# angeris/cfmm-routing-code

Measured on AMD Instinct MI355X. Metric: pool-subproblems/sec to 1e-6 rel-gap; 1e6 pools / 1k tokens; 1/2/4/8 GPU, higher is better.
Workload: dtype f64; 1 GPU; C3: 1000000 pools per GPU (cp2=700000, w2=200000, gn3-8=100000) / 1000 tokens, linear-utility arbitrage, cold-start solve to gap,infeas <= 1e-06; pools_per_gpu=1000000, pools_total=1000000, seed=0, parallelism=single GPU, rccl_ranks=1

## Files before the change

### cfmm-routing-code_amd/csrc/cfmm_hip.hip

```cpp
#include <hip/hip_runtime.h>
#include <dlfcn.h>
#include <algorithm>
#include <cmath>
#include <atomic>
#include <chrono>
#include <condition_variable>
#include <cstdarg>
#include <cstdio>
#include <cstdlib>
#include <cstring>
#include <map>
#include <memory>
#include <set>
#include <mutex>
#include <functional>
#include <limits>
#include <string>
#include <thread>
#include <type_traits>
#include <vector>

#include "../../include/cfmm.h"
#include "kernels.hpp"
#include "iterate.hpp"
// ... 96 lines not shown
    bool have_nu = false;
    bool hsol_valid = false;
    double mu_last = 0.0;
    bool slo_active = false;
    std::vector<double> tr_ovr;
    bool tr_ovr_valid = false;
};

struct cfmm_ctx {
    int device = 0, n = 0, ng = 0;
    int cus = 256;
    hipStream_t stream = nullptr;
    std::string err;
    std::string backend;

    std::shared_ptr<PoolStore> pools = std::make_shared<PoolStore>();
    int *flags2 = nullptr;
    bool is_clone = false;
    unsigned long long pool_gen = 0;
    hipEvent_t ev_pool = nullptr;
    char *upd_dev = nullptr; size_t upd_cap = 0;
    unsigned long long *upd_host = nullptr;
    int *flagsG[CFMM_MAX_POOL_SIZE + 1] = {};
    double *trade_buf = nullptr;
    size_t trade_cap = 0;

    double *c = nullptr, *h = nullptr, *off = nullptr, *glo = nullptr, *ghi = nullptr;
    int *ctype = nullptr, *grp = nullptr;
    int *gptr = nullptr, *gmem = nullptr;
    double *tie_tmp = nullptr;
    double *nu = nullptr, *nu_acc = nullptr, *psi_acc = nullptr, *psi_t = nullptr, *nu0 = nullptr;
    double *s = nullptr, *s_t = nullptr, *Gs = nullptr, *Gs_t = nullptr, *d = nullptr, *Ds = nullptr;
    double *S = nullptr, *Y = nullptr, *rho = nullptr;
    double *acc = nullptr;
    DevState *st = nullptr;
    long long *ts = nullptr;
    char *dev_arena = nullptr, *host_arena = nullptr;
    double *pin = nullptr; size_t pin_cap = 0;
    double *pin_dev = nullptr;
    unsigned long long io_seq = 0;
    bool h_clean = false;
    bool lean_io = true;
    char *util_h = nullptr;
    size_t util_span = 0;
    DevState *hst = nullptr;
    double *hsol = nullptr;
    double *hnu0 = nullptr;
    double *hnu0_d = nullptr, *hsol_d = nullptr;
    DevState *hst_d = nullptr;
    bool nu0_deferred = false;
    Point pt;
    hipEvent_t ev[2] = {nullptr, nullptr}, ev_t0 = nullptr, ev_t1 = nullptr;
    int walk_parity[2] = {0, 0};
    int nslices = 2;
    int eval_grid_mult = 1;
    int eval_blocks_per_cu = 1;
    int upd_grid = 1;
    bool no_graph = false;
    bool multi_graph = false;
    int upd_variant = 0;
    bool upd_generic = false;
    bool general_utility = false;
    bool have_utility = false;
    std::vector<double> hc, hh, hoff;
    std::vector<int> hctype, hgrp;

    bool fused = true;
    bool tile_dma = true;
    bool tiny_path = true;
    bool plain = false;
    bool det = false;
    unsigned long long *acc_l = nullptr;
    double max_reserve = 0.0, min_fee = 1.0;
    double g_max_reserve = 0.0;
    double nu_max = 1.0;
    double det_ref_reserve = 0.0, det_ref_fee = 0.0;
    double *acc3 = nullptr, *xs3 = nullptr;
    DevState *st3 = nullptr;
    DevState *hst3 = nullptr;
    int iter_blocks_per_cu = 1;
    volatile unsigned long long *hstat_h = nullptr;
    unsigned long long *hstat_d = nullptr;
    int run_ahead = 3;
    std::vector<char> listed;
    bool listed_valid = false;
    UpdArgs *upd_batch_d = nullptr, *upd_batch_h = nullptr;
    double *batch_ws[7] = {};
    long long batch_ws_m[7] = {};
    const double *batch_ws_of[7] = {};

    hipGraphExec_t gexec = nullptr;
    int g_iters = 0, g_memory = 0;
    cfmm_opts g_opts = {};
    bool g_valid = false;

    ncclComm_t comm = nullptr;
    int n_ranks = 1, rank = 0;
    int64_t g_total = 0, g_stable = 0, g_table = 0;
    bool g_counts_valid = false;

    unsigned long long *os_mail = nullptr;
    size_t os_cap = 0;
    unsigned long long *os_peers[ONESHOT_MAX_RANKS] = {};
    std::vector<void *> os_opened;
    bool os_ready = false;

    double *sm_out = nullptr, *sm_vec = nullptr, *H = nullptr, *Dinv = nullptr;
    double *Winv = nullptr, *Rinv = nullptr;
    double *chord_y = nullptr;
    bool chol_pairs = true;
    bool inverse_factor = true;
    double *sm_ws[CFMM_POOL_KINDS2] = {};
    long long sm_ws_m[CFMM_POOL_KINDS2] = {};
    double *sm_slo = nullptr;
    int *sm_mask = nullptr, *sm_info = nullptr;
    hipStream_t probe_stream = nullptr;
    long long *probe_ring = nullptr, *probe_ring_d = nullptr;
    bool probe_running = false;
};

namespace {

int fail(cfmm_ctx *ctx, int code, const char *fmt, ...);

int trade_scratch(cfmm_ctx *ctx, size_t count, double **delta, double **lambda)
{
    if (2 * count > ctx->trade_cap) {
        if (ctx->trade_buf) (void)hipFree(ctx->trade_buf);
        ctx->trade_buf = nullptr; ctx->trade_cap = 0;
        hipError_t e = hipMalloc((void **)&ctx->trade_buf, 2 * count * sizeof(double));
        if (e != hipSuccess) return fail(ctx, CFMM_E_HIP, "trade scratch: hipMalloc(%zu) -> %s", 2 * count * sizeof(double), hipGetErrorString(e));
        ctx->trade_cap = 2 * count;
    }
    *delta = ctx->trade_buf; *lambda = ctx->trade_buf + count;
    return CFMM_OK;
}

int fail(cfmm_ctx *ctx, int code, const char *fmt, ...)
{
    char buf[512];
    va_list ap; va_start(ap, fmt); vsnprintf(buf, sizeof buf, fmt, ap); va_end(ap);
    if (ctx) ctx->err = buf; else g_create_error = buf;
    return code;
}

#define HIP_TRY(ctx, call)                                                                        \
    do {                                                                                          \
        hipError_t e_ = (call);                                                                   \
        if (e_ != hipSuccess) return fail(ctx, CFMM_E_HIP, "%s -> %s (%s:%d)", #call, hipGetErrorString(e_), __FILE__, __LINE__); \
    } while (0)

inline bool sharded(const cfmm_ctx *ctx) { return ctx->comm != nullptr || ctx->os_ready; }
inline bool rccl_unfolded(const cfmm_ctx *ctx)
{
    static const bool off = getenv("CFMM_RCCL_FOLD") && atoi(getenv("CFMM_RCCL_FOLD")) != 0;
    return ctx->comm != nullptr && !ctx->det && !off && !(ctx->os_ready && (size_t)acc_arb(ctx->n) + 1 <= ctx->os_cap);
}

int all_reduce(cfmm_ctx *ctx, void *buf, size_t count, int dtype, int op, const DevState *stop = nullptr, int fold_slices = 1)
{
    if (fold_slices > 1 && !(ctx->os_ready && count <= ctx->os_cap))
        hipLaunchKernelGGL(fold_kernel, dim3(((int)count + 255) / 256), dim3(256), 0, ctx->stream, (double *)buf, ctx->n, fold_slices,
                           count > (size_t)acc_arb(ctx->n) + 1 ? 1 : 0, stop);
    if (ctx->os_ready && count <= ctx->os_cap) {
        OneShotArgs a = {};
        for (int r = 0; r < ctx->n_ranks; ++r) a.mail[r] = ctx->os_peers[r];
        a.buf = (unsigned long long *)buf;
        a.epoch_word = ctx->os_mail + oneshot_bytes(ctx->os_cap) / 8;
        a.stop = stop ? &stop->status : nullptr;
        a.nslices = fold_slices; a.stride = acc_stride(ctx->n);
        a.n_ranks = ctx->n_ranks; a.rank = ctx->rank; a.count = (int)count; a.cap = ctx->os_cap;
        a.op = dtype == NCCL_INT64 ? ONESHOT_SUM_I64 : (op == NCCL_MAX ? ONESHOT_MAX_F64 : ONESHOT_SUM_F64);
        hipLaunchKernelGGL(oneshot_allreduce_kernel, dim3(1), dim3(ONESHOT_THREADS), 0, ctx->stream, a);
        return CFMM_OK;
    }
    if (!ctx->comm) return fail(ctx, CFMM_E_UNSUPPORTED, "all-reduce of %zu elements: beyond the one-shot mailbox and no RCCL communicator", count);
    const int rc = g_rccl.AllReduce(buf, buf, count, dtype, op, ctx->comm, ctx->stream);
    if (rc != 0) return fail(ctx, CFMM_E_RCCL, "ncclAllReduce -> %s", g_rccl.GetErrorString ? g_rccl.GetErrorString(rc) : "error");
    return CFMM_OK;
}

template <class T>
int dev_upload(cfmm_ctx *ctx, T **dst, const T *src, size_t count, std::vector<void *> *track)
{
    T *p = nullptr;
    HIP_TRY(ctx, hipMalloc((void **)&p, count * sizeof(T) + 16));
    if (src) HIP_TRY(ctx, hipMemcpyAsync(p, src, count * sizeof(T), hipMemcpyHostToDevice, ctx->stream));
    else HIP_TRY(ctx, hipMemsetAsync(p, 0, count * sizeof(T), ctx->stream));
    if (track) track->push_back(p);
    *dst = p;
    return CFMM_OK;
}

constexpr size_t STAGE_BYTES = 4u << 20;
constexpr int STAGE_SLOTS = 4;
struct StageRing {
    std::mutex mu;
    char *buf = nullptr;
    hipEvent_t ev[STAGE_SLOTS] = {};
    bool used[STAGE_SLOTS] = {};
    hipStream_t last[STAGE_SLOTS] = {};
    int next = 0;
};
StageRing g_stage;
void stage_ring_drain(hipStream_t stream)
{
    std::lock_guard<std::mutex> lock(g_stage.mu);
    for (int q = 0; q < STAGE_SLOTS; ++q)
        if (g_stage.used[q] && g_stage.last[q] == stream) { (void)hipEventSynchronize(g_stage.ev[q]); g_stage.used[q] = false; }
}
hipError_t stage_slot_wait(int slot)
{
    hipError_t e = hipEventSynchronize(g_stage.ev[slot]);
    if (e != hipSuccess) { (void)hipGetLastError(); e = hipDeviceSynchronize(); }
    return e;
}
std::mutex g_stream_mu;
std::vector<hipStream_t> g_free_streams[64];

class HostPool {
public:
    static HostPool &get() { static HostPool *p = new HostPool(); return *p; }
    int threads() const { return nthreads_ + 1; }
    void run(int n, const std::function<void(int)> &f)
    {
        if (n <= 0) return;
        if (n == 1 || nthreads_ == 0) { for (int i = 0; i < n; ++i) f(i); return; }
        std::unique_lock<std::mutex> own(run_mu_);
        {
            std::lock_guard<std::mutex> g(mu_);
            job_ = &f; njobs_ = n; next_.store(0, std::memory_order_relaxed); left_.store(n, std::memory_order_relaxed);
            gen_.fetch_add(1, std::memory_order_release);
        }
// ... 1087 lines not shown
}
int listed_tokens(cfmm_ctx *ctx)
{
    if (ctx->listed_valid) return CFMM_OK;
    const int n = ctx->n;
    double *mark = ctx->sm_vec;
    HIP_TRY(ctx, hipMemsetAsync(mark, 0, (size_t)n * sizeof(double), ctx->stream));
    auto pass = [&](const int *ids, long long count) {
        if (!ids || count <= 0) return;
        const unsigned grid = (unsigned)std::min<long long>((count + 255) / 256, 4ll * ctx->cus);
        hipLaunchKernelGGL(mark_tokens_kernel, dim3(grid), dim3(256), 0, ctx->stream, ids, count, mark);
    };
    const PoolStore &ps = *ctx->pools;
    for (int k = 0; k < CFMM_POOL_KINDS2; ++k) { pass(ps.r2[k].b.ia, ps.r2[k].b.m); pass(ps.r2[k].b.ib, ps.r2[k].b.m); }
    for (int k = 3; k <= CFMM_MAX_POOL_SIZE; ++k) pass(ps.rn[k].b.idx, (long long)k * ps.rn[k].b.m);
    for (auto &row : ps.rg) for (int k = 2; k <= CFMM_MAX_POOL_SIZE; ++k) pass(row[k].b.idx, (long long)k * row[k].b.m);
    HIP_TRY(ctx, hipGetLastError());
    if (sharded(ctx)) { int rc = all_reduce(ctx, mark, (size_t)n, NCCL_FLOAT64, NCCL_SUM); if (rc) return rc; }
    std::vector<double> h(n);
    HIP_TRY(ctx, hipMemcpyAsync(h.data(), mark, (size_t)n * sizeof(double), hipMemcpyDeviceToHost, ctx->stream));
    HIP_TRY(ctx, hipStreamSynchronize(ctx->stream));
    ctx->listed.assign(n, 0);
    for (int j = 0; j < n; ++j) ctx->listed[j] = h[j] != 0.0;
    ctx->listed_valid = true;
    return CFMM_OK;
}

struct SmoothEval { std::vector<double> psi; double value = 0.0, trade = 0.0; };

int smooth_eval_host(cfmm_ctx *ctx, const std::vector<double> &nu, double mu, bool hess, SmoothEval &e, bool warm = true,
                     const std::vector<double> *slo = nullptr)
{
    const int n = ctx->n;
    int rc = smooth_buffers(ctx, hess); if (rc) return rc;
    double *pin = pin_scratch(ctx, 8 * (size_t)n + 64);
    if (!pin) return fail(ctx, CFMM_E_HIP, "pinned staging (%d tokens)", n);
    double *pin_nu = pin, *pin_slo = pin + n, *pin_out = pin + 2 * n;
    std::memcpy(pin_nu, nu.data(), n * sizeof(double));
    if (slo) std::memcpy(pin_slo, slo->data(), n * sizeof(double));
    if (ctx->lean_io) {
        IoList l;
        l.copy(ctx->nu, pin_device(ctx, pin_nu), n * sizeof(double));
        if (slo) l.copy(ctx->sm_slo, pin_device(ctx, pin_slo), n * sizeof(double));
        l.zero(ctx->sm_out, (size_t)(n + 2) * sizeof(double));
        if (hess && !ctx->h_clean) l.zero(ctx->H, (size_t)hess_ld(n) * hess_nr(n) * sizeof(double));
        if (hess) ctx->h_clean = false;
        if ((rc = launch_io(ctx, l, false))) return rc;
        if ((rc = launch_smooth(ctx, mu, hess, warm, slo != nullptr, true))) return rc;
        IoList p;
        p.copy(pin_device(ctx, pin_out), ctx->sm_out, (size_t)(n + 2) * sizeof(double));
        if ((rc = launch_io(ctx, p, true))) return rc;
        if ((rc = wait_io(ctx))) return rc;
    } else {
        HIP_TRY(ctx, hipMemcpyAsync(ctx->nu, pin_nu, n * sizeof(double), hipMemcpyHostToDevice, ctx->stream));
        if (slo) HIP_TRY(ctx, hipMemcpyAsync(ctx->sm_slo, pin_slo, n * sizeof(double), hipMemcpyHostToDevice, ctx->stream));
        if ((rc = launch_smooth(ctx, mu, hess, warm, slo != nullptr))) return rc;
        HIP_TRY(ctx, hipMemcpyAsync(pin_out, ctx->sm_out, (size_t)(n + 2) * sizeof(double), hipMemcpyDeviceToHost, ctx->stream));
        HIP_TRY(ctx, hipStreamSynchronize(ctx->stream));
    }
    e.psi.assign(pin_out, pin_out + n);
    e.value = pin_out[n]; e.trade = pin_out[n + 1];
    return CFMM_OK;
}

struct HostUtilityTerm { double pstar, ubar, uval, viol, d2; };
static HostUtilityTerm host_utility_term(int ctype, double c, double h, double nu, double psi)
{
    HostUtilityTerm t;
    if (ctype == CFMM_ULOG) {
        t.pstar = c / nu - h; t.ubar = c * std::log(c / nu) - c + nu * h;
        t.viol = std::max(-(psi + h), 0.0); t.uval = c * std::log(std::max(psi + h, 1e-300)); t.d2 = c;
    } else {
        t.pstar = h * (c - nu); t.ubar = 0.5 * h * (c - nu) * (c - nu);
        t.viol = 0.0; t.uval = c * psi - 0.5 * psi * psi / h; t.d2 = h * nu * nu;
    }
    return t;
}

int solve_newton(cfmm_ctx *ctx, const cfmm_opts &o, cfmm_stats *out, int evals_before, double warm_mu)
{
    const char *why = "";
    if (!newton_supported(ctx, &why)) return fail(ctx, CFMM_E_UNSUPPORTED, "solve: the second-order method cannot take this problem: %s", why);
    const int n = ctx->n;
    int rc = smooth_buffers(ctx, true); if (rc) return rc;
    const std::vector<double> &c = ctx->hc, &h = ctx->hh;
    const std::vector<int> &ct = ctx->hctype;

    HIP_TRY(ctx, hipStreamSynchronize(ctx->stream));
    const auto t0 = std::chrono::steady_clock::now();
    HIP_TRY(ctx, hipEventRecord(ctx->ev_t0, ctx->stream));

    std::vector<double> s(n), nu(n), d(n), G(n), Hd(n), rhs(n), s2(n), nu2(n), psi_x(n);
    std::vector<int> mask(n), pin(n);
    std::vector<double> lob(n);
    if (!pin_scratch(ctx, 8 * (size_t)n + 64 + n + (size_t)acc_stride(n))) return fail(ctx, CFMM_E_HIP, "pinned staging (%d tokens)", n);
    if (ctx->lean_io) {
        IoList z;
        for (int k = 0; k < CFMM_POOL_KINDS2; ++k) if (ctx->sm_ws[k]) z.zero(ctx->sm_ws[k], 2 * (size_t)ctx->pools->r2[k].b.m * sizeof(double));
        if (z.a.njobs && (rc = launch_io(ctx, z, false))) return rc;
        IoList p;
        p.copy(pin_device(ctx, ctx->pin), ctx->nu_acc, n * sizeof(double));
        if ((rc = launch_io(ctx, p, true)) || (rc = wait_io(ctx))) return rc;
        std::memcpy(nu.data(), ctx->pin, n * sizeof(double));
    } else {
        HIP_TRY(ctx, hipMemcpyAsync(nu.data(), ctx->nu_acc, n * sizeof(double), hipMemcpyDeviceToHost, ctx->stream));
        HIP_TRY(ctx, hipStreamSynchronize(ctx->stream));
    }
    if ((rc = listed_tokens(ctx))) return rc;
    std::vector<char> listed(n);
    for (int j = 0; j < n; ++j) listed[j] = !(ct[j] < CFMM_ULOG && !ctx->listed[j] && h[j] == 0.0);
    long long nbar = 0;
    for (int k = 0; k < CFMM_POOL_KINDS2; ++k) nbar += 2 * ctx->pools->r2[k].b.m;
    nbar += 2 * ctx->pools->r2[CFMM_POOL_SUM2].b.m;
    for (int k = 2; k <= CFMM_MAX_POOL_SIZE; ++k) nbar += 3LL * k * ctx->pools->rg[CFMM_POOLK_SUM][k].b.m;
    for (int j = 0; j < n; ++j) {
        mask[j] = ct[j] == CFMM_FREE || !listed[j];
        lob[j] = (ct[j] == CFMM_GE && c[j] > 0.0) ? std::log(c[j]) : -INFINITY;
        if (ct[j] == CFMM_GE && !(c[j] > 0.0) && listed[j]) nbar += 1;
        double sj = std::log(nu[j]);
        if (ct[j] == CFMM_FREE) {
            if (!(c[j] > 0.0)) return fail(ctx, CFMM_E_ARG, "solve: token %d is unconstrained (CFMM_FREE) with c = 0: unbounded", j);
            sj = std::log(c[j]);
        } else sj = std::max(sj, lob[j]);
        s[j] = sj; nu[j] = std::exp(sj);
    }
    if (sharded(ctx)) {
        long long ge = 0;
        for (int j = 0; j < n; ++j) ge += ct[j] == CFMM_GE && !(c[j] > 0.0) && listed[j];
        double cnt = (double)(nbar - ge);
        HIP_TRY(ctx, hipMemcpyAsync(ctx->sm_vec, &cnt, sizeof(double), hipMemcpyHostToDevice, ctx->stream));
        { int rc = all_reduce(ctx, ctx->sm_vec, 1, NCCL_FLOAT64, NCCL_SUM); if (rc) return rc; }
        HIP_TRY(ctx, hipMemcpyAsync(&cnt, ctx->sm_vec, sizeof(double), hipMemcpyDeviceToHost, ctx->stream));
        HIP_TRY(ctx, hipStreamSynchronize(ctx->stream));
        nbar = (long long)cnt + ge;
    }

    const std::vector<double> s_start = s;
    ctx->h_clean = false;
    int evals = evals_before, steps = 0, status = 0;
    double arb_x = 0.0;
    auto exact = [&](const std::vector<double> &p) { ++evals; return cfmm_eval_dual(ctx, p.data(), &arb_x, psi_x.data(), nullptr); };
    auto assemble = [&](const std::vector<double> &p, const SmoothEval &e, double mu, std::vector<double> *grad, std::vector<double> *hdiag) {
        double g = e.value;
        for (int j = 0; j < n; ++j) {
            double Gj, hj = 0.0;
            if (ct[j] >= CFMM_ULOG) {
                const HostUtilityTerm ut = host_utility_term(ct[j], c[j], h[j], p[j], e.psi[j]);
                g += ut.ubar;
                Gj = p[j] * (e.psi[j] - ut.pstar);
                hj = ut.d2;
            } else {
                g += (p[j] - c[j]) * h[j];
                Gj = p[j] * (e.psi[j] + h[j]);
            }
            const double Gj_lin = Gj;
            if (ct[j] == CFMM_GE && !(c[j] > 0.0) && listed[j]) {
                g -= mu * std::log(p[j]);
                Gj -= mu;
            }
            if (grad) (*grad)[j] = mask[j] ? 0.0 : Gj;
            if (hdiag) (*hdiag)[j] = std::max(Gj_lin, 0.0) + hj;
        }
        return g;
    };

    if (!ctx->lean_io)
        for (int k = 0; k < CFMM_POOL_KINDS2; ++k)
// ... 302 lines not shown
    static const bool trace_c = getenv("CFMM_UPLOAD_TRACE") != nullptr;
    const auto tc0 = std::chrono::steady_clock::now();
    auto lap = [&](const char *what) { if (trace_c) fprintf(stderr, "[cfmm create] %-28s %.3f ms\n", what, std::chrono::duration<double, std::milli>(std::chrono::steady_clock::now() - tc0).count()); };
    TRY_C(hipSetDevice(device));
    hipDeviceProp_t prop;
    TRY_C(hipGetDeviceProperties(&prop, device));
    lap("device properties");
    ctx->cus = prop.multiProcessorCount > 0 ? prop.multiProcessorCount : 256;
    ctx->backend = std::string("hip:") + prop.gcnArchName;
    if (ctx->backend.find("gfx950") == std::string::npos) {
        fail(ctx, CFMM_E_HIP, "cfmm_create: device is %s, this build is gfx950-only", prop.gcnArchName);
        return bail(CFMM_E_HIP);
    }
    if (eval_lds_bytes(n_tokens, true) > 160 * 1024) {
        fail(ctx, CFMM_E_LIMIT, "cfmm_create: %d tokens exceed the LDS-staged limit (%d)", n_tokens, (int)((160 * 1024 / 8 - 16) / 3));
        return bail(CFMM_E_LIMIT);
    }
    {
        const char *sp = getenv("CFMM_STREAM_POOL");
        std::lock_guard<std::mutex> g(g_stream_mu);
        auto &fl = g_free_streams[device & 63];
        if (!(sp && atoi(sp) == 0) && !fl.empty()) { ctx->stream = fl.back(); fl.pop_back(); }
    }
    if (!ctx->stream) TRY_C(hipStreamCreateWithFlags(&ctx->stream, hipStreamNonBlocking));
    lap("stream");
    if (const char *s = getenv("CFMM_SLICES")) ctx->nslices = std::min(64, std::max(1, atoi(s)));
    if (const char *s = getenv("CFMM_EVAL_GRID_MULT")) ctx->eval_grid_mult = std::max(1, atoi(s));
    if (const char *s = getenv("CFMM_UPDATE_GENERIC")) ctx->upd_generic = atoi(s) != 0;
    if (const char *s = getenv("CFMM_UPDATE_VARIANT")) ctx->upd_variant = atoi(s);
    if (const char *s = getenv("CFMM_UPD_GRID")) ctx->upd_grid = std::max(1, atoi(s));
    if (const char *s = getenv("CFMM_MULTI_GRAPH")) ctx->multi_graph = atoi(s) != 0;
    if (const char *s = getenv("CFMM_NO_GRAPH")) ctx->no_graph = atoi(s) != 0;
    if (const char *s = getenv("CFMM_FUSED")) ctx->fused = atoi(s) != 0;
    if (const char *s = getenv("CFMM_TILE_DMA")) ctx->tile_dma = atoi(s) != 0;
    if (const char *s = getenv("CFMM_BACKSUB")) ctx->inverse_factor = std::string(s) != "classic";
    if (const char *s = getenv("CFMM_CHOL")) ctx->chol_pairs = std::string(s) != "single";
    if (const char *s = getenv("CFMM_NEWTON_IO")) ctx->lean_io = std::string(s) != "blit";
    if (const char *s = getenv("CFMM_TINY")) ctx->tiny_path = atoi(s) != 0;
    if (const char *s = getenv("CFMM_RUN_AHEAD")) ctx->run_ahead = std::max(1, atoi(s));
    if (const char *s = getenv("CFMM_DETERMINISTIC")) ctx->det = atoi(s) != 0;
    const int n = n_tokens;
    int rc = 0;
    {
        struct Piece { void **dst; size_t bytes; };
        std::vector<Piece> pieces;
        auto want = [&](auto **pp, size_t count) { pieces.push_back({(void **)pp, count * sizeof(**pp)}); };
        want(&ctx->c, n + 4); want(&ctx->h, n + 4); want(&ctx->glo, n + 4); want(&ctx->ghi, n + 4); want(&ctx->ctype, n + 4);
        want(&ctx->off, n + 4); want(&ctx->grp, n + 4);
        want(&ctx->gptr, n + 5); want(&ctx->gmem, n + 4); want(&ctx->tie_tmp, 2 * (size_t)n + 4);
        double **vecs[] = {&ctx->nu, &ctx->nu_acc, &ctx->psi_acc, &ctx->psi_t, &ctx->nu0, &ctx->s, &ctx->s_t,
                           &ctx->Gs, &ctx->Gs_t, &ctx->d, &ctx->Ds};
        for (auto v : vecs) want(v, n + 4);
        want(&ctx->S, (size_t)MAX_MEMORY * hist_stride(n) + 4); want(&ctx->Y, (size_t)MAX_MEMORY * hist_stride(n) + 4);
        want(&ctx->rho, MAX_MEMORY);
        want(&ctx->acc, (size_t)ctx->nslices * acc_stride(n) + 4);
        want(&ctx->st, 1);
        want(&ctx->acc3, 3 * (size_t)ctx->nslices * acc_stride(n) + 4);
        want(&ctx->xs3, 3 * (size_t)XS_VECS * iter_xvs(n) + 4);
        want(&ctx->st3, 3);
        want(&ctx->acc_l, 6 * (size_t)n + 4);
        want(&ctx->ts, 64 + 8 * 4096 + 2048);
        size_t total = 0;
        for (auto &pc : pieces) total += (pc.bytes + 16 + 255) & ~(size_t)255;
        TRY_C(hipMalloc((void **)&ctx->dev_arena, total));
        TRY_C(hipMemsetAsync(ctx->dev_arena, 0, total, ctx->stream));
        size_t off = 0;
        for (auto &pc : pieces) { *pc.dst = ctx->dev_arena + off; off += (pc.bytes + 16 + 255) & ~(size_t)255; }
        ctx->util_span = (size_t)((char *)ctx->off - (char *)ctx->c);
        const size_t hb[5] = {2 * sizeof(DevState), 6 * sizeof(DevState), 2 * (size_t)n * sizeof(double), (size_t)n * sizeof(double), ctx->util_span};
        size_t ho[6] = {0, 0, 0, 0, 0, 0};
        for (int q = 0; q < 5; ++q) ho[q + 1] = ho[q] + ((hb[q] + 255) & ~(size_t)255);
        TRY_C(hipHostMalloc((void **)&ctx->host_arena, ho[5], hipHostMallocDefault));
        ctx->hst = (DevState *)(ctx->host_arena + ho[0]); ctx->hst3 = (DevState *)(ctx->host_arena + ho[1]);
        ctx->hsol = (double *)(ctx->host_arena + ho[2]); ctx->hnu0 = (double *)(ctx->host_arena + ho[3]);
        {
            char *base_d = nullptr;
            TRY_C(hipHostGetDevicePointer((void **)&base_d, ctx->host_arena, 0));
            ctx->hst_d = (DevState *)(base_d + ho[0]); ctx->hsol_d = (double *)(base_d + ho[2]); ctx->hnu0_d = (double *)(base_d + ho[3]);
        }
        ctx->util_h = ctx->host_arena + ho[4];
        std::memset(ctx->util_h, 0, ctx->util_span);
    }
    lap("device + pinned arenas");
    TRY_C(hipHostMalloc((void **)&ctx->hstat_h, 64 + ITER_HRING * sizeof(unsigned long long), hipHostMallocMapped));
    TRY_C(hipHostGetDevicePointer((void **)&ctx->hstat_d, (void *)ctx->hstat_h, 0));
    *ctx->hstat_h = 0;
    lap("mapped progress word");
    for (int i = 0; i < 2; ++i) TRY_C(hipEventCreateWithFlags(&ctx->ev[i], hipEventDisableTiming));
    TRY_C(hipEventCreate(&ctx->ev_t0));
    TRY_C(hipEventCreate(&ctx->ev_t1));
    TRY_C(hipEventCreateWithFlags(&ctx->ev_pool, hipEventDisableTiming));
    ctx->pools->sharers.push_back(ctx);
    if (ctx->det && eval_lds_bytes(n, true, true) > 160 * 1024) {
        fail(ctx, CFMM_E_LIMIT, "cfmm_create: CFMM_DETERMINISTIC=1 with %d tokens exceeds the LDS tile of the reproducible mode", n);
        return bail(CFMM_E_LIMIT);
    }
    lap("events");
    if ((rc = set_all_lds_attrs(ctx))) return bail(rc);
    lap("LDS attributes");
    {
        int nb = 0;
        TRY_C(hipOccupancyMaxActiveBlocksPerMultiprocessor(&nb, eval_kernel<false, false>, EVAL_THREADS, eval_lds_bytes(n, false)));
        ctx->eval_blocks_per_cu = nb < 1 ? 1 : nb;
        nb = 0;
        TRY_C(hipOccupancyMaxActiveBlocksPerMultiprocessor(&nb, iter_kernel<2, false, false>, EVAL_THREADS, iter_lds_bytes(n)));
        ctx->iter_blocks_per_cu = nb < 1 ? 1 : nb;
    }
    if (ctx->nslices > 64) ctx->nslices = 64;
    ctx->hc.assign(n, 0.0); ctx->hh.assign(n, 0.0); ctx->hoff.assign(n, 0.0);
    ctx->hctype.assign(n, CFMM_GE); ctx->hgrp.resize(n);
    for (int j = 0; j < n; ++j) ctx->hgrp[j] = j;
    lap("occupancy queries");
    TRY_C(hipMemcpyAsync(ctx->grp, ctx->hgrp.data(), n * sizeof(int), hipMemcpyHostToDevice, ctx->stream));
    TRY_C(hipStreamSynchronize(ctx->stream));
    lap("group ids + sync");
#undef TRY_C
    *out = ctx;
    return CFMM_OK;
}

int cfmm_clone(cfmm_ctx *src, cfmm_ctx **out)
{
    if (!src || !out) return CFMM_E_ARG;
    HIP_TRY(src, hipSetDevice(src->device));
    pools_ready(src);
    HIP_TRY(src, hipStreamSynchronize(src->stream));
    release_landed(src);
    cfmm_ctx *c = nullptr;
    int rc = cfmm_create(src->device, src->n, &c);
    if (rc) { src->err = g_create_error; return rc; }
    {
        std::lock_guard<std::mutex> g(src->pools->mu);
        c->pools = src->pools;
        c->pools->sharers.push_back(c);
    }
    c->is_clone = true;
    c->det = src->det;
    local_extrema(c);
    c->pool_gen = c->pools->gen.load(std::memory_order_acquire);
    c->nslices = src->nslices <= c->nslices ? src->nslices : c->nslices;
    *out = c;
    return CFMM_OK;
}

int cfmm_destroy(cfmm_ctx *ctx)
{
    if (!ctx) return CFMM_OK;
    (void)hipSetDevice(ctx->device);
    if (ctx->stream) (void)hipStreamSynchronize(ctx->stream);
    drop_graph(ctx);
    if (ctx->comm && g_rccl.CommDestroy) g_rccl.CommDestroy(ctx->comm);
    for (void *q : ctx->os_opened) (void)hipIpcCloseMemHandle(q);
    if (ctx->os_mail) (void)hipFree(ctx->os_mail);
    if (ctx->pools) {
        std::lock_guard<std::mutex> g(ctx->pools->mu);
        auto &sh = ctx->pools->sharers;
        sh.erase(std::remove(sh.begin(), sh.end(), ctx), sh.end());
    }
    ctx->pools.reset();
    if (ctx->ev_pool) (void)hipEventDestroy(ctx->ev_pool);
    if (ctx->upd_dev) (void)hipFree(ctx->upd_dev);
    if (ctx->upd_host) (void)hipHostFree(ctx->upd_host);
    if (ctx->flags2) (void)hipFree(ctx->flags2);
    for (int *q : ctx->flagsG) if (q) (void)hipFree(q);
    if (ctx->trade_buf) (void)hipFree(ctx->trade_buf);
    for (void *p : {(void *)ctx->sm_out, (void *)ctx->sm_vec, (void *)ctx->H, (void *)ctx->Dinv, (void *)ctx->Winv, (void *)ctx->Rinv, (void *)ctx->chord_y, (void *)ctx->sm_ws[0], (void *)ctx->sm_ws[1], (void *)ctx->sm_ws[3], (void *)ctx->sm_ws[4], (void *)ctx->sm_slo, (void *)ctx->sm_mask, (void *)ctx->sm_info}) if (p) (void)hipFree(p);
    if (ctx->dev_arena) (void)hipFree(ctx->dev_arena);
    if (ctx->host_arena) (void)hipHostFree(ctx->host_arena);
    if (ctx->pin) (void)hipHostFree(ctx->pin);
    if (ctx->hstat_h) (void)hipHostFree((void *)ctx->hstat_h);
    if (ctx->probe_ring) {
        __atomic_store_n(reinterpret_cast<volatile long long *>(ctx->probe_ring) + 2 * PROBE_CAP, 1ll, __ATOMIC_RELEASE);
        if (ctx->probe_stream) (void)hipStreamSynchronize(ctx->probe_stream);
        (void)hipHostFree(ctx->probe_ring);
    }
    if (ctx->probe_stream) (void)hipStreamDestroy(ctx->probe_stream);
    if (ctx->upd_batch_d) (void)hipFree(ctx->upd_batch_d);
    if (ctx->upd_batch_h) (void)hipHostFree(ctx->upd_batch_h);
    for (double *q : ctx->batch_ws) if (q) (void)hipFree(q);
    for (auto &e : ctx->ev) if (e) (void)hipEventDestroy(e);
    if (ctx->ev_t0) (void)hipEventDestroy(ctx->ev_t0);
    if (ctx->ev_t1) (void)hipEventDestroy(ctx->ev_t1);
    if (ctx->stream) {
        std::lock_guard<std::mutex> g(g_stream_mu);
        auto &fl = g_free_streams[ctx->device & 63];
        if (fl.size() < 16) fl.push_back(ctx->stream); else (void)hipStreamDestroy(ctx->stream);
    }
    sweep_release(ctx);
    delete ctx;
    return CFMM_OK;
}

int64_t cfmm_pool_count(cfmm_ctx *ctx)
{
    if (!ctx) return 0;
    int64_t m = 0;
    ctx->pools->each([&m](const auto &r) { m += r.b.m; });
    return m;
}

int64_t cfmm_eval_bytes(cfmm_ctx *ctx)
{
    if (!ctx) return 0;
    int64_t bytes = 0;
    for (int k = 0; k < CFMM_POOL_KINDS2; ++k) {
        const bool par = !(k == CFMM_POOL_CP2 || k == CFMM_POOL_SUM2);
        const bool mirror = ctx->pools->r2[k].cmem != nullptr && !ctx->det && !heavy_kind(k);
        bytes += ctx->pools->r2[k].b.m * ((mirror ? 21 : 32) + (par ? 8 : 0));
    }
    const bool lrw = !ctx->det && !CFMM_STAGED_WALK;
    for (int k = 3; k <= CFMM_MAX_POOL_SIZE; ++k) bytes += ctx->pools->rn[k].b.m * (20 + (lrw ? 28 : 20) * k);
    for (auto &row : ctx->pools->rg) {
        int k = 0;
        for (auto &r : row) { bytes += r.b.m * (12 * k + (r.b.param ? 40 : 16)); ++k; }
    }
    return bytes;
}

static bool reorder_applies(cfmm_ctx *ctx, int kind_or_k, int64_t m)
{
    static const bool off = getenv("CFMM_REORDER") && atoi(getenv("CFMM_REORDER")) == 0;
    return !off && m >= (kind_or_k >= 3 ? RO_MIN_POOLS_N : RO_MIN_POOLS) && ctx->n >= 2 * RO_NB && kind_or_k != CFMM_POOL_SUM2;
}
static char *reorder_arena(cfmm_ctx *ctx, size_t total, int64_t m, int **perm, unsigned **hist)
{
    char *na = nullptr;
    const size_t pbytes = ((size_t)m * 4 + 255) & ~(size_t)255;
    if (hipMalloc((void **)&na, total + 256 + pbytes + 4096) != hipSuccess) return nullptr;
    *perm = (int *)(na + total + 256);
    *hist = (unsigned *)(na + total + 256 + pbytes);
    (void)hipMemsetAsync(*hist, 0, RO_KEYS * sizeof(unsigned), ctx->stream);
    return na;
// ... 28 lines not shown
    const dim3 gh(std::min(grid, 2048)), gs(grid), blk(RO_THREADS);
    with_int<3, 8>(k, [&](auto K) {
        hipLaunchKernelGGL(ro_hist_kernel<K>, gh, blk, 0, ctx->stream, b.idx, (const int *)nullptr, (long long)b.m, bsz, hist);
        hipLaunchKernelGGL(ro_scan_kernel, dim3(1), dim3(64), 0, ctx->stream, hist);
        hipLaunchKernelGGL(ro_scatterN_kernel<K>, gs, blk, 0, ctx->stream, b, d, perm, bsz, hist);
    });
    b.idx = d.idx; b.R = d.R; b.w = d.w; b.fee = d.fee; b.lfee = d.lfee; b.lrw = d.lrw; b.perm = perm;
    r.mem = na;
    return true;
}

static void build_compact_mirrors(cfmm_ctx *ctx, PoolStore &ps)
{
    static const int mode = getenv("CFMM_COMPACT") ? atoi(getenv("CFMM_COMPACT")) : -1;
    if (mode == 0 || ctx->n > 65536) return;
    for (int k : {CFMM_POOL_CP2, CFMM_POOL_W2, CFMM_POOL_SUM2}) {
        Resident2 &r = ps.r2[k];
        Bucket2 &b = r.b;
        if (r.ctried || b.m == 0 || (mode < 0 && b.m < 1000000)) continue;
        r.ctried = true;
        const size_t m = (size_t)b.m, off_fee = (4 * m + 255) & ~(size_t)255, off_tab = (off_fee + m + 255) & ~(size_t)255;
        char *mem = nullptr;
        if (hipMalloc((void **)&mem, off_tab + 256 * 8 + 64) != hipSuccess) { (void)hipGetLastError(); continue; }
        (void)hipMemsetAsync(mem + off_tab, 0, 256 * 8 + 64, ctx->stream);
        int *flag = (int *)(mem + off_tab + 256 * 8);
        hipLaunchKernelGGL(compact_build_kernel, dim3((unsigned)std::min<size_t>((m + 255) / 256, 4096)), dim3(256), 0, ctx->stream, b,
                           (unsigned *)mem, (unsigned char *)(mem + off_fee), (unsigned long long *)(mem + off_tab), flag);
        int over = 1;
        if (hipMemcpyAsync(&over, flag, sizeof(int), hipMemcpyDeviceToHost, ctx->stream) != hipSuccess || hipStreamSynchronize(ctx->stream) != hipSuccess) over = 1;
        if (over) { (void)hipGetLastError(); (void)hipFree(mem); continue; }
        r.cmem = mem;
        b.cid = (const unsigned *)mem; b.cfee = (const unsigned char *)(mem + off_fee); b.ctab = (const double *)(mem + off_tab);
    }
}

static void pools_ready(cfmm_ctx *ctx)
{
    pools_seen(ctx);
    PoolStore &ps = *ctx->pools;
    std::lock_guard<std::mutex> guard(ps.mu);
    struct Mirrors { cfmm_ctx *c; PoolStore &p; ~Mirrors() { build_compact_mirrors(c, p); } } mirrors{ctx, ps};
    {
        bool pending = false;
        ps.each([&pending](const auto &r) { pending |= r.ro != 0; });
        if (!pending) return;
        double stray = 0.0;
        for (int k = 3; k <= CFMM_MAX_POOL_SIZE; ++k) stray += (double)ps.rn[k].b.m * (k - 2);
        if (stray / (double)ctx->cus >= 0.5 * ctx->n) {
            ps.each([](auto &r) { r.ro = 0; });
            return;
        }
    }
    for (auto &r : ps.r2) if (r.ro) {
        void *old = r.mem;
        if (reorder_bucket2(ctx, r)) ps.landed.emplace_back(old, ctx->stream);
        r.ro = 0;
    }
    for (int k = 3; k <= CFMM_MAX_POOL_SIZE; ++k) if (ps.rn[k].ro) {
        void *old = ps.rn[k].mem;
        if (reorder_bucketN(ctx, k, ps.rn[k])) ps.landed.emplace_back(old, ctx->stream);
        ps.rn[k].ro = 0;
    }
}
static void release_landed(cfmm_ctx *ctx)
{
    PoolStore &ps = *ctx->pools;
    std::vector<void *> mine;
    {
        std::lock_guard<std::mutex> guard(ps.mu);
        size_t keep = 0;
        for (auto &q : ps.landed) { if (q.second == ctx->stream) mine.push_back(q.first); else ps.landed[keep++] = q; }
        ps.landed.resize(keep);
    }
    if (mine.empty()) return;
    (void)hipStreamSynchronize(ctx->stream);
    for (void *q : mine) (void)hipFree(q);
}

struct PoolEntry {
    cfmm_ctx *ctx;
    PoolStore &ps;
    const bool reader;
    hipError_t device;
    explicit PoolEntry(cfmm_ctx *c, bool rd = true) : ctx(c), ps(*c->pools), reader(rd)
    {
        if (reader) { std::lock_guard<std::mutex> g(ps.mu); ++ps.readers; }
        if ((device = hipSetDevice(c->device)) == hipSuccess) pools_ready(c);
    }
    ~PoolEntry() { release_landed(ctx); if (reader) { std::lock_guard<std::mutex> g(ps.mu); --ps.readers; } }
};

struct Kind2Info { const char *name; bool needs_param; bool (*param_ok)(double); const char *param_rule; };
static const Kind2Info kKind2[CFMM_POOL_KINDS2] = {
    {"constant product", false, nullptr, ""},
    {"weighted geometric mean", true, [](double x) { return x > 0.0 && x < 1.0; }, "a weight in (0, 1)"},
    {"constant sum", false, nullptr, ""},
    {"stableswap", true, [](double x) { return x > 0.0 && x <= std::numeric_limits<double>::max(); }, "alpha > 0"},
    {"power sum", true, [](double x) { return x >= 1e-3 && x <= 0.999; }, "an exponent t in [0.001, 0.999]"},
};

extern "C++" {
static int upload_begin(cfmm_ctx *ctx, const char *who, const void *old_arena)
{
    HIP_TRY(ctx, hipSetDevice(ctx->device));
    if (ctx->pools.use_count() > 1) return fail(ctx, CFMM_E_STATE, "%s: the pools are shared with a clone (cfmm_clone); destroy the clones first", who);
    if (old_arena) HIP_TRY(ctx, hipStreamSynchronize(ctx->stream));
    return CFMM_OK;
}
template <class R, class B> static void upload_install(cfmm_ctx *ctx, R &r, const B &b, void *arena, const UploadScan &scan, size_t ro_total)
{
    r.release();
    r.b = b; r.mem = arena; r.ro = ro_total;
    r.mxr = scan.mxr; r.mnf = scan.mnf;
    pools_changed(ctx);
}
}

int cfmm_upload_pools2(cfmm_ctx *ctx, int kind, int64_t m, const double *Ra, const double *Rb, const double *fee,
                       const double *param, const int32_t *ia, const int32_t *ib)
{
    if (!ctx) return CFMM_E_ARG;
    if (kind < 0 || kind >= CFMM_POOL_KINDS2 || m < 0) return fail(ctx, CFMM_E_ARG, "upload_pools2: kind %d, m %lld", kind, (long long)m);
    if (m >= (1ll << 29)) return fail(ctx, CFMM_E_LIMIT, "upload_pools2: %lld pools in one bucket (the kernels address a column with 32-bit byte offsets: < 2^29)", (long long)m);
    if (m > 0 && (!Ra || !Rb || !fee || !ia || !ib)) return fail(ctx, CFMM_E_ARG, "upload_pools2: NULL column");
    if (m > 0 && kKind2[kind].needs_param && !param) return fail(ctx, CFMM_E_ARG, "upload_pools2: kind %d (%s) needs param", kind, kKind2[kind].name);
    Resident2 &r = ctx->pools->r2[kind];
    { int rc = upload_begin(ctx, "upload_pools2", r.mem); if (rc) return rc; }
    Bucket2 b = {};
    b.m = m;
    void *arena = nullptr;
    UploadScan scan;
    size_t ro_total = 0;
    if (m > 0) {
        const int ntok = ctx->n;
        std::vector<Col> cols;
        auto reserve_ok = [](double x) { return x > 0.0 && x <= std::numeric_limits<double>::max(); };
        cols.push_back(checked_col<double>(Ra, m, (void **)&b.Ra, &scan, 0, reserve_ok));
        cols.push_back(checked_col<double>(Rb, m, (void **)&b.Rb, &scan, 0, reserve_ok));
        cols.push_back(checked_col<double>(fee, m, (void **)&b.fee, &scan, 1, [](double x) { return x > 0.0 && x <= 1.0; }));
        if (param) {
            if (kKind2[kind].param_ok) cols.push_back(checked_col<double>(param, m, (void **)&b.param, &scan, 2, kKind2[kind].param_ok));
            else cols.push_back(plain_col(param, m * sizeof(double), (void **)&b.param));
        }
        cols.push_back(checked_col<int32_t>(ia, m, (void **)&b.ia, &scan, 2, [ntok](int32_t v) { return (uint32_t)v < (uint32_t)ntok; }));
        {
            Col c; c.bytes = m * sizeof(int32_t); c.dst = (void **)&b.ib; c.direct = ib;
            UploadScan *sp = &scan;
            c.fill = [ia, ib, ntok, sp](char *out, size_t off, size_t len) {
                const size_t i0 = off / sizeof(int32_t), cnt = len / sizeof(int32_t);
                std::memcpy(out, ib + i0, len);
                const int32_t *o = (const int32_t *)out, *a = ia + i0;
                bool ok = true;
                for (size_t i = 0; i < cnt; ++i) ok &= ((uint32_t)o[i] < (uint32_t)ntok) & (o[i] != a[i]);
                if (!ok) sp->bad.store(true, std::memory_order_relaxed);
            };
            cols.push_back(c);
        }
        size_t total = 0;
        const bool ro = reorder_applies(ctx, kind, m);
        int rc = upload_arena(ctx, cols, &arena, &scan, &total);
        if (rc == CFMM_E_ARG && scan.bad.load()) {
            for (int64_t i = 0; i < m; ++i) {
                const long long q = (long long)i;
                if (ia[i] < 0 || ia[i] >= ntok || ib[i] < 0 || ib[i] >= ntok || ia[i] == ib[i]) return fail(ctx, CFMM_E_ARG, "upload_pools2: pool %lld has token ids (%d, %d) outside [0,%d) or equal", q, ia[i], ib[i], ctx->n);
                if (!(Ra[i] > 0.0) || !(Rb[i] > 0.0) || !std::isfinite(Ra[i]) || !std::isfinite(Rb[i])) return fail(ctx, CFMM_E_ARG, "upload_pools2: pool %lld has a reserve that is not positive and finite", q);
                if (!(fee[i] > 0.0 && fee[i] <= 1.0)) return fail(ctx, CFMM_E_ARG, "upload_pools2: pool %lld has fee %g outside (0, 1]", q, fee[i]);
                if (kind == CFMM_POOL_W2 && !(param[i] > 0.0 && param[i] < 1.0)) return fail(ctx, CFMM_E_ARG, "upload_pools2: pool %lld has weight %g outside (0, 1)", q, param[i]);
                if (kind == CFMM_POOL_CURVE2 && !(param[i] > 0.0)) return fail(ctx, CFMM_E_ARG, "upload_pools2: pool %lld has alpha %g <= 0", q, param[i]);
                if (param && kKind2[kind].param_ok && !kKind2[kind].param_ok(param[i]))
                    return fail(ctx, CFMM_E_ARG, "upload_pools2: pool %lld (%s) has parameter %g: expected %s", q, kKind2[kind].name, param[i], kKind2[kind].param_rule);
            }
            return fail(ctx, CFMM_E_ARG, "upload_pools2: a column failed its checks");
        }
        if (rc) return rc;
        if (ro) ro_total = total;
    }
    if (kind == CFMM_POOL_SUM2) {
        ctx->pools->hs_ia.clear(); ctx->pools->hs_ib.clear(); ctx->pools->hs_fee.clear(); ctx->pools->hs_Ra.clear(); ctx->pools->hs_Rb.clear();
        if (m > 0 && m <= 65536) {
            ctx->pools->hs_ia.assign(ia, ia + m); ctx->pools->hs_ib.assign(ib, ib + m); ctx->pools->hs_fee.assign(fee, fee + m);
            ctx->pools->hs_Ra.assign(Ra, Ra + m); ctx->pools->hs_Rb.assign(Rb, Rb + m);
        }
        if (ctx->flags2) { (void)hipFree(ctx->flags2); ctx->flags2 = nullptr; }
    }
    upload_install(ctx, r, b, arena, scan, ro_total);
    return CFMM_OK;
}
// ... 297 lines not shown
    if (kind < 0 || kind >= CFMM_POOLK_KINDS || k < 2 || k > CFMM_MAX_POOL_SIZE || count < 0)
        return fail(ctx, CFMM_E_ARG, "%s: kind %d, %d assets, count %lld", who, kind, k, (long long)count);
    if (count > 0 && (!pos || !R)) return fail(ctx, CFMM_E_ARG, "%s: NULL column", who);
    if (param && kind != CFMM_POOLK_STABLE) return fail(ctx, CFMM_E_ARG, "%s: constant-sum pools have no parameter", who);
    UpdateFrame f(ctx, who, ctx->pools->rg[kind][k]);
    { int rc = f.open(count, pos, [&] { return fail(ctx, CFMM_E_STATE, "%s: no pools of kind %d with %d assets uploaded", who, kind, k); }); if (rc) return rc; }
    double mx_new = 0.0;
    { int rc = update_check_reserves(ctx, who, R, (int64_t)k * count, mx_new); if (rc) return rc; }
    if (param)
        for (int64_t i = 0; i < count; ++i)
            if (!(param[i] > 0.0 && param[i] <= std::numeric_limits<double>::max())) return fail(ctx, CFMM_E_ARG, "%s: entry %lld has alpha %g (need > 0)", who, (long long)i, param[i]);
    const BucketG b = f.r.b;
    const int64_t m = b.m;
    const double mx_old = f.r.mxr;
    std::vector<UpdPart> parts = {{pos, (size_t)count * 4}, {R, (size_t)count * k * 8}};
    if (param) parts.push_back({param, (size_t)count * 8});
    const int cnt = (int)count;
    return f.run(parts, nullptr, mx_new, count,
        [&](const char *d, const std::vector<size_t> &o, const int *, int *low) {
            hipLaunchKernelGGL(upd_scatterG_kernel, dim3(upd_grid(count)), dim3(UP_THREADS), 0, ctx->stream, b, k, cnt, (const int *)(d + o[0]),
                               (const double *)(d + o[1]), param ? (const double *)(d + o[2]) : nullptr, mx_old, low);
        },
        [&](unsigned long long *out) {
            hipLaunchKernelGGL(upd_max_kernel, dim3(max_grid((int64_t)k * m)), dim3(UP_THREADS), 0, ctx->stream, b.R, (long long)k * m, (const double *)nullptr, 0ll, out);
        });
}

int cfmm_get_tradesG(cfmm_ctx *ctx, int kind, int k, double *delta, double *lambda)
{
    if (!ctx || kind < 0 || kind >= CFMM_POOLK_KINDS || k < 2 || k > CFMM_MAX_POOL_SIZE) return CFMM_E_ARG;
    PoolEntry entry(ctx); HIP_TRY(ctx, entry.device);
    const BucketG &b = ctx->pools->rg[kind][k].b;
    if (b.m == 0) return CFMM_OK;
    const dim3 grid((unsigned)((b.m + GK_THREADS - 1) / GK_THREADS)), blk(GK_THREADS);
    const double *nu = ctx->nu_acc;
    const int *fl = kind == CFMM_POOLK_SUM ? ctx->flagsG[k] : nullptr;
    const double *slo = (ctx->pt.mu_last > 0.0 && ctx->pt.slo_active) ? ctx->sm_slo : nullptr;
    const double mu = ctx->pt.mu_last > 0.0 ? ctx->pt.mu_last : 0.0;
    return read_back(ctx, "get_tradesG", (size_t)k * b.m, delta, lambda, [&](double *dd, double *dl) {
        with_int<CFMM_POOLK_STABLE, CFMM_POOLK_SUM>(kind, [&](auto KIND) {
            with_int<2, 8>(k, [&](auto K) { hipLaunchKernelGGL((tradesg_kernel<KIND, K>), grid, blk, 0, ctx->stream, b, fl, nu, slo, mu, dd, dl); });
        });
    });
}

int cfmm_set_pool_flags(cfmm_ctx *ctx, int kind, const int32_t *flags)
{
    if (!ctx) return CFMM_E_ARG;
    if (kind != CFMM_POOL_SUM2) return fail(ctx, CFMM_E_ARG, "set_pool_flags: only CFMM_POOL_SUM2 pools can be tied");
    HIP_TRY(ctx, hipSetDevice(ctx->device));
    const Bucket2 &b = ctx->pools->r2[kind].b;
    HIP_TRY(ctx, hipStreamSynchronize(ctx->stream));
    if (ctx->flags2) { (void)hipFree(ctx->flags2); ctx->flags2 = nullptr; }
    ctx->g_valid = false;
    drop_tenders(ctx);
    if (!flags || b.m == 0) return CFMM_OK;
    int rc = dev_upload<int>(ctx, &ctx->flags2, flags, b.m, nullptr);
    if (rc) return rc;
    HIP_TRY(ctx, hipStreamSynchronize(ctx->stream));
    return CFMM_OK;
}

int cfmm_set_pool_flagsG(cfmm_ctx *ctx, int k, const int32_t *flags)
{
    if (!ctx || k < 2 || k > CFMM_MAX_POOL_SIZE) return ctx ? fail(ctx, CFMM_E_ARG, "set_pool_flagsG: %d assets", k) : CFMM_E_ARG;
    HIP_TRY(ctx, hipSetDevice(ctx->device));
    const BucketG &b = ctx->pools->rg[CFMM_POOLK_SUM][k].b;
    HIP_TRY(ctx, hipStreamSynchronize(ctx->stream));
    if (ctx->flagsG[k]) { (void)hipFree(ctx->flagsG[k]); ctx->flagsG[k] = nullptr; }
    ctx->g_valid = false;
    drop_tenders(ctx);
    if (!flags || b.m == 0) return CFMM_OK;
    std::vector<int> pm((size_t)k * b.m);
    for (int64_t i = 0; i < b.m; ++i) for (int j = 0; j < k; ++j) pm[(size_t)i * k + j] = flags[(size_t)j * b.m + i];
    HIP_TRY(ctx, hipMalloc((void **)&ctx->flagsG[k], pm.size() * sizeof(int) + 16));
    HIP_TRY(ctx, hipMemcpy(ctx->flagsG[k], pm.data(), pm.size() * sizeof(int), hipMemcpyHostToDevice));
    return CFMM_OK;
}

int cfmm_set_utility(cfmm_ctx *ctx, const double *c, const double *h, const int32_t *ctype)
{
    if (!ctx || !c) return ctx ? fail(ctx, CFMM_E_ARG, "set_utility: c is NULL") : CFMM_E_ARG;
    HIP_TRY(ctx, hipSetDevice(ctx->device));
    const int n = ctx->n;
    bool general = false;
    for (int j = 0; j < n; ++j) {
        if (!(c[j] >= 0.0) || !std::isfinite(c[j])) return fail(ctx, CFMM_E_ARG, "set_utility: c[%d] < 0 or not finite", j);
        if (ctype && (ctype[j] < 0 || ctype[j] > CFMM_UQUAD)) return fail(ctx, CFMM_E_ARG, "set_utility: ctype[%d] = %d", j, ctype[j]);
        if (ctype && ctype[j] >= CFMM_ULOG) {
            general = true;
            const double hj = h ? h[j] : 0.0;
            if (ctype[j] == CFMM_ULOG && !(c[j] > 0.0 && hj >= 0.0 && std::isfinite(hj)))
                return fail(ctx, CFMM_E_ARG, "set_utility: token %d, u = c log(Psi + h) needs c > 0 and h >= 0 (c %g, h %g)", j, c[j], hj);
            if (ctype[j] == CFMM_UQUAD && !(hj > 0.0 && std::isfinite(hj)))
                return fail(ctx, CFMM_E_ARG, "set_utility: token %d, u = c Psi - Psi^2 / (2 h) needs h > 0 (h %g)", j, hj);
        }
    }
    if (general && ctx->ng != ctx->n) return fail(ctx, CFMM_E_UNSUPPORTED, "set_utility: price ties are set; the utility table's entries take none");
    if (general != ctx->general_utility) ctx->g_valid = false;
    ctx->general_utility = general;
    ctx->hc.assign(c, c + n);
    if (h) ctx->hh.assign(h, h + n); else ctx->hh.assign(n, 0.0);
    if (ctype) ctx->hctype.assign(ctype, ctype + n); else ctx->hctype.assign(n, CFMM_GE);
    ctx->have_utility = true;
    bool plain = true;
    for (int j = 0; j < n; ++j) if (ctx->hh[j] != 0.0 || ctx->hctype[j] != CFMM_GE) { plain = false; break; }
    if (plain != ctx->plain) ctx->g_valid = false;
    ctx->plain = plain;
    HIP_TRY(ctx, hipStreamSynchronize(ctx->stream));
    std::memcpy(ctx->util_h, ctx->hc.data(), n * sizeof(double));
    std::memcpy(ctx->util_h + ((char *)ctx->h - (char *)ctx->c), ctx->hh.data(), n * sizeof(double));
    std::memcpy(ctx->util_h + ((char *)ctx->ctype - (char *)ctx->c), ctx->hctype.data(), n * sizeof(int));
    { int rc = bounds_into_mirror(ctx); if (rc) return rc; }
    HIP_TRY(ctx, hipMemcpyAsync(ctx->c, ctx->util_h, ctx->util_span, hipMemcpyHostToDevice, ctx->stream));
    HIP_TRY(ctx, hipStreamSynchronize(ctx->stream));
    return CFMM_OK;
}

int cfmm_set_ties(cfmm_ctx *ctx, int n_groups, const int32_t *grp, const double *off)
{
    if (!ctx) return CFMM_E_ARG;
    HIP_TRY(ctx, hipSetDevice(ctx->device));
    const int n = ctx->n;
    if (!grp) {
        ctx->ng = n;
        for (int j = 0; j < n; ++j) { ctx->hgrp[j] = j; ctx->hoff[j] = 0.0; }
    } else {
        if (n_groups < 1 || n_groups > n || !off) return fail(ctx, CFMM_E_ARG, "set_ties: n_groups %d", n_groups);
        if (ctx->general_utility) return fail(ctx, CFMM_E_UNSUPPORTED, "set_ties: the utility has entries beyond linear-plus-box, which take no price ties");
        for (int j = 0; j < n; ++j) if (grp[j] < 0 || grp[j] >= n_groups) return fail(ctx, CFMM_E_ARG, "set_ties: grp[%d] = %d", j, grp[j]);
        ctx->ng = n_groups;
        ctx->hgrp.assign(grp, grp + n); ctx->hoff.assign(off, off + n);
    }
    drop_tenders(ctx);
    HIP_TRY(ctx, hipMemcpyAsync(ctx->grp, ctx->hgrp.data(), n * sizeof(int), hipMemcpyHostToDevice, ctx->stream));
    HIP_TRY(ctx, hipMemcpyAsync(ctx->off, ctx->hoff.data(), n * sizeof(double), hipMemcpyHostToDevice, ctx->stream));
    if (ctx->ng != n) {
        std::vector<int> gp(ctx->ng + 1, 0), gm(n);
        for (int j = 0; j < n; ++j) ++gp[ctx->hgrp[j] + 1];
        for (int r = 0; r < ctx->ng; ++r) gp[r + 1] += gp[r];
        std::vector<int> fill(gp.begin(), gp.end() - 1);
        for (int j = 0; j < n; ++j) gm[fill[ctx->hgrp[j]]++] = j;
        HIP_TRY(ctx, hipMemcpyAsync(ctx->gptr, gp.data(), (ctx->ng + 1) * sizeof(int), hipMemcpyHostToDevice, ctx->stream));
        HIP_TRY(ctx, hipMemcpyAsync(ctx->gmem, gm.data(), n * sizeof(int), hipMemcpyHostToDevice, ctx->stream));
        HIP_TRY(ctx, hipStreamSynchronize(ctx->stream));
    }
    ctx->g_valid = false;
    return recompute_bounds(ctx);
}

static int check_prices(cfmm_ctx *ctx, const char *who, const double *nu)
{
    double mx = 0.0;
    for (int j = 0; j < ctx->n; ++j) {
        if (!(nu[j] > 0.0) || !std::isfinite(nu[j])) return fail(ctx, CFMM_E_ARG, "%s[%d] = %g is not a positive finite price", who, j, nu[j]);
        mx = std::max(mx, nu[j]);
    }
    ctx->nu_max = mx;
    return CFMM_OK;
}

int cfmm_set_nu(cfmm_ctx *ctx, const double *nu)
{
    if (!ctx || !nu) return CFMM_E_ARG;
    HIP_TRY(ctx, hipSetDevice(ctx->device));
    { int rc = check_prices(ctx, "set_nu: nu", nu); if (rc) return rc; }
    HIP_TRY(ctx, hipStreamSynchronize(ctx->stream));
    std::memcpy(ctx->hnu0, nu, ctx->n * sizeof(double));
    HIP_TRY(ctx, hipMemcpyAsync(ctx->nu_acc, ctx->hnu0, ctx->n * sizeof(double), hipMemcpyHostToDevice, ctx->stream));
    point_from_caller(ctx);
    return CFMM_OK;
}

int cfmm_get_nu(cfmm_ctx *ctx, double *nu)
{
    if (!ctx || !nu) return CFMM_E_ARG;
    HIP_TRY(ctx, hipSetDevice(ctx->device));
    HIP_TRY(ctx, hipMemcpyAsync(nu, ctx->nu_acc, ctx->n * sizeof(double), hipMemcpyDeviceToHost, ctx->stream));
    HIP_TRY(ctx, hipStreamSynchronize(ctx->stream));
    return CFMM_OK;
}

int cfmm_get_psi(cfmm_ctx *ctx, double *psi)
{
    if (!ctx || !psi) return CFMM_E_ARG;
    HIP_TRY(ctx, hipSetDevice(ctx->device));
    pools_seen(ctx);
    HIP_TRY(ctx, hipMemcpyAsync(psi, ctx->psi_acc, ctx->n * sizeof(double), hipMemcpyDeviceToHost, ctx->stream));
    HIP_TRY(ctx, hipStreamSynchronize(ctx->stream));
    return CFMM_OK;
}

int cfmm_get_solution(cfmm_ctx *ctx, double *nu, double *psi)
{
    if (!ctx || (!nu && !psi)) return CFMM_E_ARG;
    pools_seen(ctx);
    if (ctx->pt.hsol_valid) {
        if (nu) std::memcpy(nu, ctx->hsol, ctx->n * sizeof(double));
        if (psi) std::memcpy(psi, ctx->hsol + ctx->n, ctx->n * sizeof(double));
        return CFMM_OK;
    }
    HIP_TRY(ctx, hipSetDevice(ctx->device));
    if (nu) HIP_TRY(ctx, hipMemcpyAsync(nu, ctx->nu_acc, ctx->n * sizeof(double), hipMemcpyDeviceToHost, ctx->stream));
    if (psi) HIP_TRY(ctx, hipMemcpyAsync(psi, ctx->psi_acc, ctx->n * sizeof(double), hipMemcpyDeviceToHost, ctx->stream));
    HIP_TRY(ctx, hipStreamSynchronize(ctx->stream));
    return CFMM_OK;
}

int cfmm_eval_dual(cfmm_ctx *ctx, const double *nu, double *arb_sum, double *psi, double *diag)
{
    if (!ctx || !nu) return CFMM_E_ARG;
    PoolEntry entry(ctx); HIP_TRY(ctx, entry.device);
    const int n = ctx->n;
    for (int j = 0; j < n; ++j) if (!(nu[j] > 0.0) || !std::isfinite(nu[j])) return fail(ctx, CFMM_E_ARG, "eval_dual: nu[%d] = %g is not a positive finite price", j, nu[j]);
    const int len = acc_stride(n);
    double *pinb = pin_scratch(ctx, 8 * (size_t)n + 64 + n + (size_t)len);
    if (!pinb) return fail(ctx, CFMM_E_HIP, "pinned staging (%d tokens)", n);
    double *pin_nu = pinb + 8 * (size_t)n + 64, *pin_acc = pin_nu + n;
    std::memcpy(pin_nu, nu, n * sizeof(double));
    { double mx = 0.0; for (int j = 0; j < n; ++j) mx = std::max(mx, nu[j]); ctx->nu_max = mx; }
    if (ctx->det && sharded(ctx)) { int rc = refresh_global_counts(ctx); if (rc) return rc; }
    const bool lean = ctx->lean_io;
    if (lean) {
        IoList l;
        l.copy(ctx->nu, pin_device(ctx, pin_nu), n * sizeof(double));
        l.zero(ctx->nu + n, sizeof(double));
        l.zero(ctx->acc, (size_t)ctx->nslices * acc_stride(n) * sizeof(double));
        if (ctx->det) l.zero(ctx->acc_l, 6 * (size_t)n * sizeof(unsigned long long));
        int rc = launch_io(ctx, l, false); if (rc) return rc;
    } else {
        HIP_TRY(ctx, hipMemcpyAsync(ctx->nu, pin_nu, n * sizeof(double), hipMemcpyHostToDevice, ctx->stream));
        HIP_TRY(ctx, hipMemsetAsync(ctx->nu + n, 0, sizeof(double), ctx->stream));
        HIP_TRY(ctx, hipMemsetAsync(ctx->acc, 0, (size_t)ctx->nslices * acc_stride(n) * sizeof(double), ctx->stream));
        if (ctx->det) HIP_TRY(ctx, hipMemsetAsync(ctx->acc_l, 0, 6 * (size_t)n * sizeof(unsigned long long), ctx->stream));
    }
    if (diag) launch_all_evals<true>(ctx); else launch_all_evals<false>(ctx);
    if (ctx->det) { int rc = det_finish(ctx, ctx->acc, ctx->nu, diag != nullptr); if (rc) return rc; }
    else hipLaunchKernelGGL(fold_kernel, dim3((len + 255) / 256), dim3(256), 0, ctx->stream, ctx->acc, n, ctx->nslices, 1, (const DevState *)nullptr);
    HIP_TRY(ctx, hipGetLastError());
    if (sharded(ctx) && !ctx->det) {
        int rc = all_reduce(ctx, ctx->acc, (size_t)len, NCCL_FLOAT64, NCCL_SUM); if (rc) return rc;
    }
    if (lean) {
        IoList p;
        p.copy(pin_device(ctx, pin_acc), ctx->acc, len * sizeof(double));
        p.zero(ctx->acc, (size_t)len * sizeof(double));
        int rc = launch_io(ctx, p, true); if (rc) return rc;
        if ((rc = wait_io(ctx))) return rc;
    } else {
        HIP_TRY(ctx, hipMemcpyAsync(pin_acc, ctx->acc, len * sizeof(double), hipMemcpyDeviceToHost, ctx->stream));
        HIP_TRY(ctx, hipMemsetAsync(ctx->acc, 0, (size_t)len * sizeof(double), ctx->stream));
        HIP_TRY(ctx, hipStreamSynchronize(ctx->stream));
    }
    if (psi) std::memcpy(psi, pin_acc, n * sizeof(double));
    if (arb_sum) *arb_sum = pin_acc[acc_arb(n)];
    if (diag) std::memcpy(diag, pin_acc + acc_diag(n), n * sizeof(double));
    return CFMM_OK;
}

#ifdef CFMM_CH2_STAMPS
int cfmm_debug_ch2_stamps(cfmm_ctx *ctx, uint64_t *out64)
{
    HIP_TRY(ctx, hipStreamSynchronize(ctx->stream));
    HIP_TRY(ctx, hipMemcpyFromSymbol(out64, HIP_SYMBOL(cfmm::g_ch2_stamps), 64 * sizeof(uint64_t)));
    return CFMM_OK;
}
#endif
#ifdef CFMM_SMOOTH_HIST
int cfmm_debug_smooth_hist(cfmm_ctx *ctx, uint64_t *out128, int reset)
{
    HIP_TRY(ctx, hipStreamSynchronize(ctx->stream));
    HIP_TRY(ctx, hipMemcpyFromSymbol(out128, HIP_SYMBOL(cfmm::g_smooth_hist), 128 * sizeof(uint64_t)));
    { uint64_t e[4]; HIP_TRY(ctx, hipMemcpyFromSymbol(e, HIP_SYMBOL(cfmm::g_smooth_eff), sizeof e)); out128[126] = e[0]; out128[127] = e[1];
      if (reset) { uint64_t z4[4] = {}; HIP_TRY(ctx, hipMemcpyToSymbol(HIP_SYMBOL(cfmm::g_smooth_eff), z4, sizeof z4)); } }
    if (reset) { uint64_t z[128] = {}; HIP_TRY(ctx, hipMemcpyToSymbol(HIP_SYMBOL(cfmm::g_smooth_hist), z, sizeof z)); }
    return CFMM_OK;
}
int cfmm_debug_smooth_samples(cfmm_ctx *ctx, double *out768)
{
    HIP_TRY(ctx, hipStreamSynchronize(ctx->stream));
    HIP_TRY(ctx, hipMemcpyFromSymbol(out768, HIP_SYMBOL(cfmm::g_smooth_samples), 768 * sizeof(double)));
    return CFMM_OK;
}
#endif

int cfmm_debug_cholesky(cfmm_ctx *ctx, int n, const double *A, const double *b, double *x, int32_t *info)
{
    if (!ctx || !A || !b || !x || n != ctx->n) return ctx ? fail(ctx, CFMM_E_ARG, "debug_cholesky: n must equal the context's token count") : CFMM_E_ARG;
    HIP_TRY(ctx, hipSetDevice(ctx->device));
    int rc = smooth_buffers(ctx, true); if (rc) return rc;
    const int ld = hess_ld(n);
    std::vector<double> hd(n, 0.0);
    std::vector<int> mask(n, 0);
    HIP_TRY(ctx, hipMemsetAsync(ctx->H, 0, (size_t)ld * hess_nr(n) * sizeof(double), ctx->stream));
    HIP_TRY(ctx, hipMemcpy2DAsync(ctx->H, (size_t)ld * sizeof(double), A, (size_t)n * sizeof(double), (size_t)n * sizeof(double), n, hipMemcpyHostToDevice, ctx->stream));
    HIP_TRY(ctx, hipMemcpyAsync(ctx->sm_vec, hd.data(), n * sizeof(double), hipMemcpyHostToDevice, ctx->stream));
    HIP_TRY(ctx, hipMemcpyAsync(ctx->sm_vec + n, b, n * sizeof(double), hipMemcpyHostToDevice, ctx->stream));
    HIP_TRY(ctx, hipMemcpyAsync(ctx->sm_mask, mask.data(), n * sizeof(int), hipMemcpyHostToDevice, ctx->stream));
    hipLaunchKernelGGL(hess_finish_kernel, dim3(1024), dim3(256), 0, ctx->stream, ctx->H, n, hess_nr(n), ld, (const double *)ctx->sm_vec,
                       (const int *)ctx->sm_mask, (const double *)(ctx->sm_vec + n));
    if ((rc = launch_cholesky(ctx, n, ctx->sm_vec + n))) return rc;
    int inf = 0;
    HIP_TRY(ctx, hipMemcpyAsync(&inf, ctx->sm_info, sizeof(int), hipMemcpyDeviceToHost, ctx->stream));
    HIP_TRY(ctx, hipMemcpyAsync(x, ctx->sm_vec + n, n * sizeof(double), hipMemcpyDeviceToHost, ctx->stream));
    HIP_TRY(ctx, hipStreamSynchronize(ctx->stream));
    if (info) *info = inf;
    return CFMM_OK;
}

int cfmm_debug_cholesky_apply(cfmm_ctx *ctx, int n, const double *b, double *x)
{
    if (!ctx || !b || !x || n != ctx->n || !ctx->H) return ctx ? fail(ctx, CFMM_E_STATE, "debug_cholesky_apply: call cfmm_debug_cholesky first") : CFMM_E_ARG;
    HIP_TRY(ctx, hipSetDevice(ctx->device));
    HIP_TRY(ctx, hipMemcpyAsync(ctx->sm_vec + n, b, n * sizeof(double), hipMemcpyHostToDevice, ctx->stream));
    { int rc = launch_chord(ctx, n, ctx->sm_vec + n, ctx->sm_vec); if (rc) return rc; }
    HIP_TRY(ctx, hipMemcpyAsync(x, ctx->sm_vec, n * sizeof(double), hipMemcpyDeviceToHost, ctx->stream));
    HIP_TRY(ctx, hipStreamSynchronize(ctx->stream));
    return CFMM_OK;
}

int cfmm_eval_smooth(cfmm_ctx *ctx, const double *nu, double mu, double *value, double *trade, double *psi, double *H)
{
    if (!ctx || !nu || !(mu > 0.0)) return ctx ? fail(ctx, CFMM_E_ARG, "eval_smooth: nu is NULL or mu <= 0") : CFMM_E_ARG;
    PoolEntry entry(ctx); HIP_TRY(ctx, entry.device);
    const char *why = "";
    if (!newton_supported(ctx, &why)) return fail(ctx, CFMM_E_UNSUPPORTED, "eval_smooth: %s", why);
    const int n = ctx->n;
    for (int j = 0; j < n; ++j) if (!(nu[j] > 0.0) || !std::isfinite(nu[j])) return fail(ctx, CFMM_E_ARG, "eval_smooth: nu[%d] = %g is not a positive finite price", j, nu[j]);
    SmoothEval e;
    std::vector<double> p(nu, nu + n);
    int rc = smooth_eval_host(ctx, p, mu, H != nullptr, e, false); if (rc) return rc;
    if (value) *value = e.value;
    if (trade) *trade = e.trade;
    if (psi) std::memcpy(psi, e.psi.data(), n * sizeof(double));
    if (H) {
        HIP_TRY(ctx, hipMemcpy2DAsync(H, (size_t)n * sizeof(double), ctx->H, (size_t)hess_ld(n) * sizeof(double), (size_t)n * sizeof(double), n,
                                      hipMemcpyDeviceToHost, ctx->stream));
        HIP_TRY(ctx, hipStreamSynchronize(ctx->stream));
    }
    return CFMM_OK;
}

static int solve_lbfgs(cfmm_ctx *ctx, const cfmm_opts &o, cfmm_stats *out);

static int solve_tiny_kinks(cfmm_ctx *ctx, const cfmm_opts &o, cfmm_stats *out)
{
    const int n = ctx->n;
    const int64_t msum = ctx->pools->r2[CFMM_POOL_SUM2].b.m;
    if (msum == 0 || ctx->is_clone || (int64_t)ctx->pools->hs_ia.size() != msum || ctx->general_utility || ctx->ng != n || ctx->flags2 || sharded(ctx) || ctx->det || o.pg_rule) return 0;
    {
        const EvalArgs ea = make_eval_args(ctx, false, 0x7fffffff, false);
        if (!(ctx->tiny_path && extra_launch_pools(ctx) == 0 && ea.ntiles >= 1 && ea.ntiles <= TINY_MAX_TILES && n <= TINY_N)) return 0;
    }
    for (int j = 0; j < n; ++j) if (ctx->hctype[j] < CFMM_GE || ctx->hctype[j] > CFMM_FREE) return 0;
    std::vector<double> nu0(n);
    if (ctx->nu0_deferred) std::memcpy(nu0.data(), ctx->hnu0, n * sizeof(double));
    else if (ctx->pt.hsol_valid) std::memcpy(nu0.data(), ctx->hsol, n * sizeof(double));
    else {
        HIP_TRY(ctx, hipMemcpyAsync(nu0.data(), ctx->nu_acc, n * sizeof(double), hipMemcpyDeviceToHost, ctx->stream));
        HIP_TRY(ctx, hipStreamSynchronize(ctx->stream));
    }
    size_t tr_len = 0;
    for (int k = 0; k < CFMM_POOL_KINDS2; ++k) tr_len += 4 * (size_t)ctx->pools->r2[k].b.m;
    for (int k = 3; k <= CFMM_MAX_POOL_SIZE; ++k) tr_len += 2 * (size_t)k * ctx->pools->rn[k].b.m;
    std::vector<double> nu(n), psi(n), theta(msum), tr(tr_len);
    std::vector<int32_t> tsgn(msum), ct(ctx->hctype.begin(), ctx->hctype.begin() + n);
    cfmm_opts os = o;
    os.method = CFMM_METHOD_LBFGS;
    int32_t rounds = 0;
    cfmm_stats st;
    const bool deferred = ctx->nu0_deferred;
    ctx->nu0_deferred = false;
    int rc = cfmm_solve_sweep(ctx, 1, ctx->hc.data(), ctx->hh.data(), ct.data(), nu0.data(), msum, ctx->pools->hs_ia.data(), ctx->pools->hs_ib.data(), ctx->pools->hs_fee.data(),
                              ctx->pools->hs_Ra.data(), ctx->pools->hs_Rb.data(), &os, 0.0, 0, nu.data(), psi.data(), theta.data(), tsgn.data(), tr.data(), &st, &rounds);
    if (rc == CFMM_E_NUMERIC || rc == CFMM_E_UNSUPPORTED) { ctx->nu0_deferred = deferred; return 0; }
    if (rc) return rc;
    size_t off_sum = 0;
    for (int k = 0; k < CFMM_POOL_SUM2; ++k) off_sum += 4 * (size_t)ctx->pools->r2[k].b.m;
    double *dS = tr.data() + off_sum, *lS = dS + 2 * msum;
    for (int64_t i = 0; i < msum; ++i) {
        if (!std::isfinite(theta[i])) continue;
        const double ya = (tsgn[i] > 0 ? -ctx->pools->hs_Rb[i] / ctx->pools->hs_fee[i] : ctx->pools->hs_Ra[i]) * theta[i];
        const double yb = (tsgn[i] > 0 ? ctx->pools->hs_Rb[i] : -ctx->pools->hs_Ra[i] / ctx->pools->hs_fee[i]) * theta[i];
        psi[ctx->pools->hs_ia[i]] += ya; psi[ctx->pools->hs_ib[i]] += yb;
        dS[i] = std::max(-ya, 0.0); dS[msum + i] = std::max(-yb, 0.0);
        lS[i] = std::max(ya, 0.0); lS[msum + i] = std::max(yb, 0.0);
    }
    double value = 0.0, cs = 0.0, dual = 0.0, viol = 0.0, scale = 0.0;
    for (int j = 0; j < n; ++j) {
        const double c = ctx->hc[j], h = ctx->hh[j], r = psi[j] + h;
        value += c * psi[j]; cs += (nu[j] - c) * r; dual += (nu[j] - c) * h + nu[j] * psi[j];
        viol = std::max(viol, ct[j] == CFMM_GE ? std::max(-r, 0.0) : (ct[j] == CFMM_EQ ? std::fabs(r) : 0.0));
        scale = std::max(scale, std::max(std::fabs(psi[j]), std::fabs(h)));
    }
    const double gap = std::fabs(cs) / std::max(1.0, std::fabs(dual));
    const double infeas = viol / std::max(std::max(scale, 1e-12 * ctx->g_max_reserve), 1e-300);
    if (!(gap <= o.tol_gap * (1.0 + 1e-6) + 1e-15 && infeas <= o.tol_infeas * (1.0 + 1e-6) + 1e-15)) { ctx->nu0_deferred = deferred; return 0; }
    std::memcpy(ctx->hsol, nu.data(), n * sizeof(double));
    std::memcpy(ctx->hsol + n, psi.data(), n * sizeof(double));
    HIP_TRY(ctx, hipMemcpyAsync(ctx->nu_acc, ctx->hsol, n * sizeof(double), hipMemcpyHostToDevice, ctx->stream));
    HIP_TRY(ctx, hipMemcpyAsync(ctx->psi_acc, ctx->hsol + n, n * sizeof(double), hipMemcpyHostToDevice, ctx->stream));
    HIP_TRY(ctx, hipStreamSynchronize(ctx->stream));
    point_published(ctx, 0.0, false, &tr);
    *out = st;
    out->status = 1; out->primal_value = value; out->dual_value = dual; out->gap = gap; out->infeas = infeas;
    out->iters = st.iters; out->method = CFMM_METHOD_LBFGS;
    return 1;
}

int cfmm_solve(cfmm_ctx *ctx, const double *nu0, const cfmm_opts *opts_in, cfmm_stats *out)
{
    if (!ctx || !out) return CFMM_E_ARG;
    PoolEntry entry(ctx); HIP_TRY(ctx, entry.device);
    drop_tenders(ctx);
    cfmm_opts o;
    if (opts_in) o = *opts_in; else cfmm_default_opts(&o);
    if (o.memory == 0) o.memory = (ctx->n <= 32 || ctx->general_utility) ? 8 : 3;
    if (o.memory < 1 || o.memory > MAX_MEMORY || o.iters_per_graph < 1 || o.iters_per_graph > 256 || o.max_evals < 1)
        return fail(ctx, CFMM_E_ARG, "solve: memory %d, iters_per_graph %d, max_evals %d", o.memory, o.iters_per_graph, o.max_evals);
    if (o.method < CFMM_METHOD_AUTO || o.method > CFMM_METHOD_NEWTON) return fail(ctx, CFMM_E_ARG, "solve: method %d", o.method);
    if (!ctx->have_utility) return fail(ctx, CFMM_E_STATE, "solve: cfmm_set_utility has not been called");
    { int rc = refresh_global_counts(ctx); if (rc) return rc; }
    if (ctx->g_total == 0) return fail(ctx, CFMM_E_STATE, "solve: no pools uploaded");
    const double warm_mu = nu0 ? 0.0 : ctx->pt.mu_last;
    if (nu0) {
        { int rc = check_prices(ctx, "solve: nu0", nu0); if (rc) return rc; }
        std::memcpy(ctx->hnu0, nu0, ctx->n * sizeof(double));
        ctx->nu0_deferred = true;
        point_from_caller(ctx);
    }
    struct Flush {
        cfmm_ctx *c;
        ~Flush()
        {
            if (c->nu0_deferred) (void)hipMemcpyAsync(c->nu_acc, c->hnu0, c->n * sizeof(double), hipMemcpyHostToDevice, c->stream);
            c->nu0_deferred = false;
        }
    } flush_guard{ctx};
    auto send_nu0 = [&]() -> int {
        if (!ctx->nu0_deferred) return CFMM_OK;
        ctx->nu0_deferred = false;
        HIP_TRY(ctx, hipMemcpyAsync(ctx->nu_acc, ctx->hnu0, ctx->n * sizeof(double), hipMemcpyHostToDevice, ctx->stream));
        return CFMM_OK;
    };
    if (!ctx->pt.have_nu) return fail(ctx, CFMM_E_STATE, "solve: no start prices (pass nu0 or call cfmm_set_nu)");
    if (o.method == CFMM_METHOD_AUTO) {
        const int r = solve_tiny_kinks(ctx, o, out);
        if (r < 0) return r;
        if (r == 1) return CFMM_OK;
    }
    const char *why = "";
    const bool can_newton = newton_supported(ctx, &why);
    if (o.method == CFMM_METHOD_NEWTON || (o.method == CFMM_METHOD_AUTO && can_newton && near_linear_pools(ctx) && !o.pg_rule)) {
        static const int prelude = getenv("CFMM_NEWTON_PRELUDE") ? atoi(getenv("CFMM_NEWTON_PRELUDE")) : 12;
        int used = 0;
        double w0 = 0.0, d0 = 0.0;
        if (prelude > 0 && can_newton && warm_mu == 0.0 && ctx->g_total >= 50000 && !o.pg_rule) {
            cfmm_opts op = o;
            op.method = 0; op.max_newton = 0; op.barrier_shrink = 0.0; op.max_evals = prelude;
            int rc = solve_lbfgs(ctx, op, out);
            if (rc) return rc;
            if (out->status == 1) return CFMM_OK;
            used = out->evals; w0 = out->wall_seconds; d0 = out->device_seconds;
        }
        { int rc = send_nu0(); if (rc) return rc; }
        int rc = solve_newton(ctx, o, out, used, warm_mu);
        out->wall_seconds += w0; out->device_seconds += d0;
        if (!rc && (out->status == 2 || out->status == 3) && !o.pg_rule && o.method == CFMM_METHOD_NEWTON) {
            const cfmm_stats second = *out;
            const int n = ctx->n;
            const std::vector<double> keep(ctx->hsol, ctx->hsol + 2 * (size_t)n);
            const double keep_mu = ctx->pt.mu_last; const bool keep_slo = ctx->pt.slo_active;
            cfmm_opts ol = o;
            ol.method = 0; ol.max_newton = 0; ol.barrier_shrink = 0.0;
            rc = solve_lbfgs(ctx, ol, out);
            if (rc) return rc;
            const cfmm_stats fin = *out;
            auto worst = [&](const cfmm_stats &st) { return std::max(std::fabs(st.gap) / o.tol_gap, st.infeas / o.tol_infeas); };
            if (fin.status != 1 && !(worst(fin) < worst(second))) {
                *out = second;
                std::memcpy(ctx->hsol, keep.data(), keep.size() * sizeof(double));
                HIP_TRY(ctx, hipMemcpyAsync(ctx->nu_acc, ctx->hsol, n * sizeof(double), hipMemcpyHostToDevice, ctx->stream));
                HIP_TRY(ctx, hipMemcpyAsync(ctx->psi_acc, ctx->hsol + n, n * sizeof(double), hipMemcpyHostToDevice, ctx->stream));
                HIP_TRY(ctx, hipStreamSynchronize(ctx->stream));
                point_published(ctx, keep_mu, keep_slo);
            } else {
                out->newton_steps = second.newton_steps;
            }
            out->evals = second.evals + fin.evals; out->pool_subproblems = second.pool_subproblems + fin.pool_subproblems;
            out->wall_seconds = second.wall_seconds + fin.wall_seconds; out->device_seconds = second.device_seconds + fin.device_seconds;
        }
        return rc;
    }
    cfmm_opts ol = o;
    ol.method = 0; ol.max_newton = 0; ol.barrier_shrink = 0.0;
    int rc = solve_lbfgs(ctx, ol, out);
    if (rc || o.method == CFMM_METHOD_LBFGS || out->status == 1 || !can_newton || o.pg_rule) return rc;
    const cfmm_stats first = *out;
    cfmm_opts o2 = o;
    o2.max_evals = std::max(o.max_evals, 500);
    rc = solve_newton(ctx, o2, out, first.evals, warm_mu);
    out->wall_seconds += first.wall_seconds; out->device_seconds += first.device_seconds;
    return rc;
}

static int solve_lbfgs(cfmm_ctx *ctx, const cfmm_opts &o_in, cfmm_stats *out)
{
    const int n = ctx->n;
    drop_barrier(ctx);
    cfmm_opts o = o_in;
    const EvalArgs ea_tiny = make_eval_args(ctx, false, 0x7fffffff, false);
    const bool tiny = tiny_applies(ctx, ea_tiny, o);
    const bool fused = !tiny && fused_applies(ctx, o);
    if (fused) o.iters_per_graph = (o.iters_per_graph + 2) / 3 * 3;
    if (sharded(ctx) && ctx->n_ranks > 1 && !oneshot_runahead(ctx) && !ctx->multi_graph) o.iters_per_graph = 3;
    static const bool graph_forced = getenv("CFMM_FUSED_GRAPH") && atoi(getenv("CFMM_FUSED_GRAPH")) != 0;
    const bool shard = sharded(ctx);
    const bool use_graph_opt = fused && !shard && graph_forced;
    const bool use_graph = !tiny && (!shard || (ctx->multi_graph && !ctx->os_ready)) && !ctx->no_graph && (!fused || shard || graph_forced);
    if (use_graph && (!ctx->g_valid || !same_opts(o, ctx->g_opts))) { int rc = build_graph(ctx, o); if (rc) return rc; }
    UpdArgs ua = make_upd_args(ctx, o);
    IterArgs ia = make_iter_args(ctx, o);
    const size_t aset = acc_set_doubles(ctx);
    const double *nu_src = ctx->nu0_deferred ? ctx->hnu0_d : ctx->nu_acc;
    ctx->nu0_deferred = false;
    static const bool zc_off = getenv("CFMM_ZERO_COPY") && atoi(getenv("CFMM_ZERO_COPY")) == 0;
    const bool zero_copy = fused && !shard && !use_graph_opt && !ctx->det && !zc_off;
    if (zero_copy) { ia.h_nu_acc = ctx->hsol_d; ia.h_psi_acc = ctx->hsol_d + n; ia.h_final = ctx->hst_d; ctx->hst[0] = DevState{}; }

    HIP_TRY(ctx, hipStreamSynchronize(ctx->stream));
    const auto t0 = std::chrono::steady_clock::now();
    HIP_TRY(ctx, hipEventRecord(ctx->ev_t0, ctx->stream));
    *ctx->hstat_h = 0;
    if (ctx->det) HIP_TRY(ctx, hipMemsetAsync(ctx->acc_l, 0, 6 * (size_t)n * sizeof(unsigned long long), ctx->stream));
    if (fused) {
        double *x0 = ctx->xs3;
        ua.s = x0; ua.s_t = x0 + ia.xvs; ua.Gs = x0 + 2 * ia.xvs; ua.d = x0 + 3 * ia.xvs; ua.nu = x0 + 4 * ia.xvs; ua.st = ctx->st3;
        hipLaunchKernelGGL(start_kernel<false>, dim3(1), dim3(UPD_THREADS), upd_lds_bytes(ctx->ng), ctx->stream, ua, nu_src,
                           ctx->acc3, (long long)(3 * aset), ctx->st3 + 1, 2);
        for (int stable = 0; stable < 2; ++stable) {
            EvalArgs e0 = make_eval_args(ctx, stable != 0);
            e0.nu = ua.nu; e0.acc = ctx->acc3;
            if (stable) launch_eval<true, true>(ctx, e0); else launch_eval<true, false>(ctx, e0);
        }
        if (table_pools(ctx) > 0) launch_table_evals<true>(ctx, ua.nu, ctx->acc3);
        if (ctx->det) { int rc = det_finish(ctx, ctx->acc3, ua.nu, true); if (rc) return rc; }
        else if (shard && rccl_unfolded(ctx)) {
            int rc = all_reduce(ctx, ctx->acc3, (size_t)ctx->nslices * acc_stride(n), NCCL_FLOAT64, NCCL_SUM); if (rc) return rc;
        } else if (shard) {
            const int len = acc_stride(n);
            hipLaunchKernelGGL(fold_kernel, dim3((len + 255) / 256), dim3(256), 0, ctx->stream, ctx->acc3, n, ctx->nslices, 1, (const DevState *)nullptr);
            int rc = all_reduce(ctx, ctx->acc3, (size_t)len, NCCL_FLOAT64, NCCL_SUM); if (rc) return rc;
        }
    } else if (tiny) {
        hipLaunchKernelGGL(start_kernel<false>, dim3(1), dim3(UPD_THREADS), upd_lds_bytes(ctx->ng), ctx->stream, ua, nu_src,
                           ctx->acc, (long long)((size_t)ctx->nslices * acc_stride(n)), (DevState *)nullptr, 0);
        const int threads = 64 * std::min(TINY_THREADS / 64, std::max(1, ea_tiny.ntiles));
        hipLaunchKernelGGL(solve_tiny_kernel<false>, dim3(1), dim3(threads), (size_t)tiny_lds_doubles(n) * sizeof(double), ctx->stream, ea_tiny, ua, o.max_evals + 1);
    } else {
        hipLaunchKernelGGL(start_kernel<false>, dim3(1), dim3(UPD_THREADS), upd_lds_bytes(ctx->ng), ctx->stream, ua, nu_src,
                           ctx->acc, (long long)((size_t)ctx->nslices * acc_stride(n)), (DevState *)nullptr, 0);
        { int rc = enqueue_iteration<true>(ctx, ua); if (rc) return rc; }
    }
    HIP_TRY(ctx, hipGetLastError());
    const int max_chunks = (o.max_evals + o.iters_per_graph - 1) / o.iters_per_graph + 1;
    auto newest = [&](const DevState *h) -> const DevState & {
        int b = 0;
        if (fused) for (int q = 1; q < 3; ++q) if (h[q].evals > h[b].evals) b = q;
        return h[b];
    };
    const int nst = fused ? 3 : 1;
    DevState *hring = fused ? ctx->hst3 : ctx->hst;
    const DevState *dst = fused ? ctx->st3 : ctx->st;
    int status = 0, t = 1;
    if (tiny) {
    } else if (fused && (!shard || oneshot_runahead(ctx)) && !use_graph_opt) {
        const auto spin0 = std::chrono::steady_clock::now();
        long spins = 0;
        for (;;) {
            const unsigned long long w = *ctx->hstat_h;
            const int done = (int)(w & 0xffffffffu);
            status = (int)(w >> 32);
            if (status != 0) break;
            if (t > o.max_evals + 1) {
                HIP_TRY(ctx, hipStreamSynchronize(ctx->stream));
                break;
            }
            if (t - done <= ctx->run_ahead) {
                int rc = enqueue_fused_iteration(ctx, ia, t); if (rc) return rc;
                ++t; spins = 0;
                continue;
            }
            if ((++spins & 0xfffff) == 0) {
                if (hipGetLastError() != hipSuccess || std::chrono::duration<double>(std::chrono::steady_clock::now() - spin0).count() > 120.0)
                    return fail(ctx, CFMM_E_HIP, "solve: the device stopped reporting progress (launch %d, %d done)", t, done);
            }
        }
        HIP_TRY(ctx, hipGetLastError());
    } else if (fused && shard && !use_graph) {
        volatile unsigned long long *ring = ctx->hstat_h + 8;
        for (int q = 0; q < ITER_HRING; ++q) ring[q] = 0;
        ia.hring = ctx->hstat_d + 8;
        const auto spin0 = std::chrono::steady_clock::now();
        for (int cidx = 0; cidx < max_chunks; ++cidx) {
            for (int it = 0; it < o.iters_per_graph; ++it) { int rc = enqueue_fused_iteration(ctx, ia, t + it); if (rc) return rc; }
            HIP_TRY(ctx, hipGetLastError());
            t += o.iters_per_graph;
            if (cidx >= 1) {
                const int last = t - o.iters_per_graph - 1;
                unsigned long long w;
                long spins = 0;
                while ((int)((w = ring[last & (ITER_HRING - 1)]) >> 32) != last) {
                    if ((++spins & 0xfffff) == 0 && (hipGetLastError() != hipSuccess || std::chrono::duration<double>(std::chrono::steady_clock::now() - spin0).count() > 120.0))
                        return fail(ctx, CFMM_E_HIP, "solve: the device stopped reporting progress (launch %d)", last);
                }
                status = (int)((w >> 24) & 0xffu);
                if (status != 0) break;
            }
        }
    } else
    for (int cidx = 0; cidx < max_chunks; ++cidx) {
        if (use_graph) {
            HIP_TRY(ctx, hipGraphLaunch(ctx->gexec, ctx->stream));
        } else {
            for (int it = 0; it < o.iters_per_graph; ++it) {
                int rc = fused ? enqueue_fused_iteration(ctx, ia, t + it) : enqueue_iteration<false>(ctx, ua);
                if (rc) return rc;
            }
            HIP_TRY(ctx, hipGetLastError());
        }
        t += o.iters_per_graph;
        HIP_TRY(ctx, hipMemcpyAsync(hring + (cidx & 1) * nst, dst, nst * sizeof(DevState), hipMemcpyDeviceToHost, ctx->stream));
        HIP_TRY(ctx, hipEventRecord(ctx->ev[cidx & 1], ctx->stream));
        if (cidx >= 1) {
            HIP_TRY(ctx, hipEventSynchronize(ctx->ev[(cidx - 1) & 1]));
            status = newest(hring + ((cidx - 1) & 1) * nst).status;
            if (status != 0) break;
        }
    }
    HIP_TRY(ctx, hipEventRecord(ctx->ev_t1, ctx->stream));
    if (zero_copy) {
        HIP_TRY(ctx, hipStreamSynchronize(ctx->stream));
        hring[0] = ctx->hst[0];
        for (int q = 1; q < nst; ++q) hring[q] = DevState{};
        if (hring[0].status == 0) {
            HIP_TRY(ctx, hipMemcpy(hring, dst, nst * sizeof(DevState), hipMemcpyDeviceToHost));
            HIP_TRY(ctx, hipMemcpy(ctx->hsol, ctx->nu_acc, n * sizeof(double), hipMemcpyDeviceToHost));
            HIP_TRY(ctx, hipMemcpy(ctx->hsol + n, ctx->psi_acc, n * sizeof(double), hipMemcpyDeviceToHost));
        }
    } else {
    HIP_TRY(ctx, hipMemcpyAsync(hring, dst, nst * sizeof(DevState), hipMemcpyDeviceToHost, ctx->stream));
    HIP_TRY(ctx, hipMemcpyAsync(ctx->hsol, ctx->nu_acc, n * sizeof(double), hipMemcpyDeviceToHost, ctx->stream));
    HIP_TRY(ctx, hipMemcpyAsync(ctx->hsol + n, ctx->psi_acc, n * sizeof(double), hipMemcpyDeviceToHost, ctx->stream));
    HIP_TRY(ctx, hipStreamSynchronize(ctx->stream));
    }
    point_published(ctx, 0.0, false);
    { double mx = 0.0; for (int j = 0; j < n; ++j) mx = std::max(mx, ctx->hsol[j]); if (mx > 0.0 && std::isfinite(mx)) ctx->nu_max = mx; }
    const auto t1 = std::chrono::steady_clock::now();
    float ms = 0.f;
    HIP_TRY(ctx, hipEventElapsedTime(&ms, ctx->ev_t0, ctx->ev_t1));

    const DevState st = newest(hring);
    std::memset(out, 0, sizeof *out);
    out->evals = st.evals; out->iters = st.iters; out->status = st.status ? st.status : 3;
    out->n_ranks = ctx->n_ranks;
    out->dual_value = st.f; out->primal_value = st.primal; out->gap = st.gap; out->infeas = st.infeas;
    out->wall_seconds = std::chrono::duration<double>(t1 - t0).count();
    out->device_seconds = ms * 1e-3;
    out->pg = st.pg;
    out->pool_subproblems = (int64_t)st.evals * cfmm_pool_count(ctx);
    out->method = CFMM_METHOD_LBFGS;
    if (!std::isfinite(st.f)) { out->status = CFMM_E_NUMERIC; return fail(ctx, CFMM_E_NUMERIC, "solve: dual value is not finite"); }
    return CFMM_OK;
}

static int batch_member_check(cfmm_ctx *c0, cfmm_ctx *const *ctxs, int b, const char *who)
{
    cfmm_ctx *c = ctxs[b];
    if (!c) return fail(c0, CFMM_E_ARG, "%s: context %d is NULL", who, b);
    for (int q = 0; q < b; ++q) if (ctxs[q] == c) return fail(c0, CFMM_E_ARG, "%s: context %d appears twice", who, b);
    if (c->pools.get() != c0->pools.get() || c->n != c0->n || c->device != c0->device || c->nslices != c0->nslices)
        return fail(c0, CFMM_E_ARG, "%s: context %d does not share the lead context's pools (cfmm_clone)", who, b);
    bool tied = c->ng != c->n || c->flags2;
    for (const int *q : c->flagsG) tied = tied || q;
    if (tied) return fail(c0, CFMM_E_UNSUPPORTED, "%s: context %d has price ties set", who, b);
    if (sharded(c) || c->det) return fail(c0, CFMM_E_UNSUPPORTED, "%s: pool-sharded / reproducible contexts are solved one at a time", who);
    return CFMM_OK;
}

static int batch_slab(cfmm_ctx *c0, int nb, hipStream_t stream, TableBatchWs &tw)
{
    tw = TableBatchWs{};
    const int cap = batch_capacity(c0->n);
    for (int k = 2; k <= CFMM_MAX_POOL_SIZE; ++k) {
        const BucketG &b = c0->pools->rg[CFMM_POOLK_STABLE][k].b;
        const int q = k - 2;
        if (c0->batch_ws[q] && (c0->batch_ws_m[q] != b.m || c0->batch_ws_of[q] != b.ws)) {
            HIP_TRY(c0, hipStreamSynchronize(stream));
            (void)hipFree(c0->batch_ws[q]);
            c0->batch_ws[q] = nullptr;
        }
        if (b.m == 0) continue;
        if (!c0->batch_ws[q]) {
            HIP_TRY(c0, hipMalloc((void **)&c0->batch_ws[q], (size_t)cap * b.m * sizeof(double)));
            c0->batch_ws_m[q] = b.m; c0->batch_ws_of[q] = b.ws;
        }
        HIP_TRY(c0, hipMemsetAsync(c0->batch_ws[q], 0xff, (size_t)nb * b.m * sizeof(double), stream));
        tw.ws[q] = c0->batch_ws[q];
    }
    return CFMM_OK;
}

struct BatchEval {
    EvalArgs ea, eh;
    TableArgs ta;
    BatchArgs bt;
    TableBatchWs tw;
    int egrid, ethreads, hgrid, hthreads, tgrid, twaves;
    size_t elds, tlds;
};
static_assert((size_t)(GT_THREADS / 64) * GT_STRIP * sizeof(double2) <= (size_t)2 * 64 * (EVAL_THREADS / 64) * sizeof(double), "table_batch_eval_kernel's strips");
static int make_batch_eval(cfmm_ctx *const *ctxs, int nb, hipStream_t stream, BatchEval &e)
{
    cfmm_ctx *c0 = ctxs[0];
    const int n = c0->n;
    e.bt = BatchArgs{};
    e.bt.nb = nb;
    for (int b = 0; b < nb; ++b) { e.bt.nu[b] = ctxs[b]->nu; e.bt.acc[b] = ctxs[b]->acc; }
    e.ea = make_eval_args(c0, false, 0x7fffffff, false);
    e.eh = make_eval_args(c0, true, 0x7fffffff, false);
    eval_geometry(c0, e.ea.ntiles, e.egrid, e.ethreads);
    eval_geometry(c0, e.eh.ntiles, e.hgrid, e.hthreads);
    e.elds = batch_lds_bytes(n, nb);
    e.ta = make_table_args(c0, nullptr, nullptr);
    static const bool warm_off = getenv("CFMM_BATCH_WARM") && atoi(getenv("CFMM_BATCH_WARM")) == 0;
    if (warm_off) e.ta.warm = 0;
    e.twaves = std::max(1, std::min(GT_THREADS / 64, e.ta.ntiles));
    e.tgrid = std::min((e.ta.ntiles + e.twaves - 1) / e.twaves, c0->cus);
    e.tlds = table_batch_lds_bytes(n, nb, e.twaves);
    e.tw = TableBatchWs{};
    if (e.ta.ntiles > 0 && e.ta.tile_end[6] > 0 && e.ta.warm) return batch_slab(c0, nb, stream, e.tw);
    e.ta.warm = 0;
    return CFMM_OK;
}
static void launch_batch_eval(cfmm_ctx *c0, const BatchEval &e, hipStream_t stream, int t)
{
    const int rev = pingpong_on(c0) ? (t & 1) : 0;
    if (e.ea.ntiles > 0) {
        EvalArgs eb = e.ea;
        eb.rev = rev;
        hipLaunchKernelGGL(eval_batch_kernel, dim3(e.egrid), dim3(e.ethreads), e.elds, stream, eb, e.bt);
    }
    if (e.eh.ntiles > 0) {
        EvalArgs eb = e.eh;
        eb.rev = rev;
        hipLaunchKernelGGL(eval_batch_heavy_kernel, dim3(e.hgrid), dim3(e.hthreads), e.elds, stream, eb, e.bt);
    }
    if (e.ta.ntiles > 0) hipLaunchKernelGGL(table_batch_eval_kernel, dim3(e.tgrid), dim3(64 * e.twaves), e.tlds, stream, e.ta, e.bt, e.tw);
}

int cfmm_solve_batch(cfmm_ctx *const *ctxs, int nb, const double *const *nu0, const cfmm_opts *opts_in, cfmm_stats *out)
{
    if (!ctxs || nb < 1 || !ctxs[0] || !out) return CFMM_E_ARG;
    cfmm_ctx *c0 = ctxs[0];
    PoolEntry entry(c0); HIP_TRY(c0, entry.device);
    for (int b = 1; b < nb; ++b) if (ctxs[b]) pools_seen(ctxs[b]);
    const int n = c0->n;
    if (nb > batch_capacity(n)) return fail(c0, CFMM_E_LIMIT, "solve_batch: %d solves, at most %d fit the LDS tile at %d tokens", nb, batch_capacity(n), n);
    cfmm_opts o;
    if (opts_in) o = *opts_in; else cfmm_default_opts(&o);
    if (o.memory == 0) o.memory = n <= 32 ? 8 : 3;
    if (o.memory < 1 || o.memory > MAX_MEMORY || o.max_evals < 1) return fail(c0, CFMM_E_ARG, "solve_batch: memory %d, max_evals %d", o.memory, o.max_evals);
    if (o.method == CFMM_METHOD_NEWTON) return fail(c0, CFMM_E_UNSUPPORTED, "solve_batch: first-order method only");
    for (int b = 0; b < nb; ++b) {
        { int rc = batch_member_check(c0, ctxs, b, "solve_batch"); if (rc) return rc; }
        cfmm_ctx *c = ctxs[b];
        if (!c->have_utility) return fail(c0, CFMM_E_STATE, "solve_batch: context %d has no utility", b);
        if (c->general_utility) return fail(c0, CFMM_E_UNSUPPORTED, "solve_batch: context %d has a utility beyond linear-plus-box (CFMM_ULOG / CFMM_UQUAD): solved one at a time", b);
        if (nu0 && nu0[b]) { int rc = cfmm_set_nu(c, nu0[b]); if (rc) { c0->err = c->err; return rc; } }
        if (!c->pt.have_nu) return fail(c0, CFMM_E_STATE, "solve_batch: context %d has no start prices", b);
        point_from_caller(c);
        HIP_TRY(c0, hipStreamSynchronize(c->stream));
    }
    if (cfmm_pool_count(c0) == 0) return fail(c0, CFMM_E_STATE, "solve_batch: no pools uploaded");
    if (!c0->upd_batch_d) {
        HIP_TRY(c0, hipMalloc((void **)&c0->upd_batch_d, BATCH_MAX * sizeof(UpdArgs)));
        HIP_TRY(c0, hipHostMalloc((void **)&c0->upd_batch_h, BATCH_MAX * sizeof(UpdArgs), hipHostMallocDefault));
    }
    hipStream_t stream = c0->stream;
    for (int b = 0; b < nb; ++b) {
        UpdArgs ua = make_upd_args(ctxs[b], o);
        ua.hstat = c0->hstat_d + b;
        c0->upd_batch_h[b] = ua;
        c0->hstat_h[b] = 0;
    }
    UpdArgs lead = c0->upd_batch_h[0];
    lead.batch = c0->upd_batch_d;
    BatchEval be;
    { int rc = make_batch_eval(ctxs, nb, stream, be); if (rc) return rc; }
    const size_t ulds = upd_lds_bytes(n);
    auto launch_update_batch = [&]() {
        const int M = o.memory;
        auto thr = [n](int E) { return 64 * ((n + 64 * E - 1) / (64 * E)); };
        if (c0->upd_generic || n > 2048 || (n > 1024 && M > 4))
            hipLaunchKernelGGL(update_kernel<true>, dim3(nb), dim3(UPD_THREADS), ulds, stream, lead);
        else if (n <= 1024 && M <= GRAM_MM)
            hipLaunchKernelGGL((update_gram_kernel<512, 2, true>), dim3(nb), dim3(thr(2)), ulds, stream, lead);
        else if (n <= 1024)
            hipLaunchKernelGGL((update_reg_kernel<512, 8, 2, true>), dim3(nb), dim3(thr(2)), ulds, stream, lead);
        else
            hipLaunchKernelGGL((update_reg_kernel<512, 4, 4, true>), dim3(nb), dim3(thr(4)), ulds, stream, lead);
    };

    HIP_TRY(c0, hipStreamSynchronize(stream));
    const auto t0 = std::chrono::steady_clock::now();
    HIP_TRY(c0, hipEventRecord(c0->ev_t0, stream));
    HIP_TRY(c0, hipMemcpyAsync(c0->upd_batch_d, c0->upd_batch_h, nb * sizeof(UpdArgs), hipMemcpyHostToDevice, stream));
    hipLaunchKernelGGL(start_kernel<true>, dim3(nb), dim3(UPD_THREADS), ulds, stream, lead, (const double *)nullptr, (double *)nullptr,
                       (long long)((size_t)c0->nslices * acc_stride(n)), (DevState *)nullptr, 0);
    for (int b = 0; b < nb; ++b) {
        launch_eval<true, false>(ctxs[b], make_eval_args(ctxs[b], false), stream);
        if (be.eh.ntiles > 0) launch_eval<true, true>(ctxs[b], make_eval_args(ctxs[b], true), stream);
        if (be.ta.ntiles > 0) {
            double *row[7];
            for (int q = 0; q < 7; ++q) row[q] = be.tw.ws[q] ? be.tw.ws[q] + (size_t)b * be.ta.bs[q].m : nullptr;
            launch_table_evals<true>(ctxs[b], ctxs[b]->nu, ctxs[b]->acc, stream, row);
        }
    }
    launch_update_batch();
    HIP_TRY(c0, hipGetLastError());
    int t = 1;
    {
        const auto spin0 = std::chrono::steady_clock::now();
        long spins = 0;
        for (;;) {
            int done = 0, running = 0;
            for (int b = 0; b < nb; ++b) {
                const unsigned long long w = c0->hstat_h[b];
                done = std::max(done, (int)(w & 0xffffffffu));
                if ((w >> 32) == 0) ++running;
            }
            if (!running) break;
            if (t > o.max_evals + 1) { HIP_TRY(c0, hipStreamSynchronize(stream)); break; }
            if (t - done <= c0->run_ahead) {
                launch_batch_eval(c0, be, stream, t);
                launch_update_batch();
                ++t; spins = 0;
                continue;
            }
            if ((++spins & 0xfffff) == 0) {
                if (hipGetLastError() != hipSuccess || std::chrono::duration<double>(std::chrono::steady_clock::now() - spin0).count() > 120.0)
                    return fail(c0, CFMM_E_HIP, "solve_batch: the device stopped reporting progress (launch %d, %d done)", t, done);
            }
        }
        HIP_TRY(c0, hipGetLastError());
    }
    HIP_TRY(c0, hipEventRecord(c0->ev_t1, stream));
    for (int b = 0; b < nb; ++b) {
        cfmm_ctx *c = ctxs[b];
        HIP_TRY(c0, hipMemcpyAsync(c->hst, c->st, sizeof(DevState), hipMemcpyDeviceToHost, stream));
        HIP_TRY(c0, hipMemcpyAsync(c->hsol, c->nu_acc, n * sizeof(double), hipMemcpyDeviceToHost, stream));
        HIP_TRY(c0, hipMemcpyAsync(c->hsol + n, c->psi_acc, n * sizeof(double), hipMemcpyDeviceToHost, stream));
    }
    HIP_TRY(c0, hipStreamSynchronize(stream));
    const auto t1 = std::chrono::steady_clock::now();
    float ms = 0.f;
    HIP_TRY(c0, hipEventElapsedTime(&ms, c0->ev_t0, c0->ev_t1));
    int rc_all = CFMM_OK;
    for (int b = 0; b < nb; ++b) {
        cfmm_ctx *c = ctxs[b];
        point_published(c, 0.0, false);
        { double mx = 0.0; for (int j = 0; j < n; ++j) mx = std::max(mx, c->hsol[j]); if (mx > 0.0 && std::isfinite(mx)) c->nu_max = mx; }
        const DevState st = c->hst[0];
        cfmm_stats *s = out + b;
        std::memset(s, 0, sizeof *s);
        s->evals = st.evals; s->iters = st.iters; s->status = st.status ? st.status : 3;
        s->n_ranks = 1;
        s->dual_value = st.f; s->primal_value = st.primal; s->gap = st.gap; s->infeas = st.infeas;
        s->wall_seconds = std::chrono::duration<double>(t1 - t0).count();
        s->device_seconds = ms * 1e-3;
        s->pg = st.pg;
        s->pool_subproblems = (int64_t)st.evals * cfmm_pool_count(c0);
        s->method = CFMM_METHOD_LBFGS;
        if (!std::isfinite(st.f)) { s->status = CFMM_E_NUMERIC; rc_all = fail(c0, CFMM_E_NUMERIC, "solve_batch: dual value of solve %d is not finite", b); }
    }
    return rc_all;
}

int cfmm_eval_dual_batch(cfmm_ctx *const *ctxs, int nb, const double *const *nu, double *arb_sum, double *const *psi)
{
    if (!ctxs || nb < 1 || !ctxs[0] || !nu) return CFMM_E_ARG;
    cfmm_ctx *c0 = ctxs[0];
    PoolEntry entry(c0); HIP_TRY(c0, entry.device);
    for (int b = 1; b < nb; ++b) if (ctxs[b]) pools_seen(ctxs[b]);
    const int n = c0->n;
    if (nb > batch_capacity(n)) return fail(c0, CFMM_E_LIMIT, "eval_dual_batch: %d price vectors, at most %d fit the LDS tile at %d tokens", nb, batch_capacity(n), n);
    for (int b = 0; b < nb; ++b) {
        { int rc = batch_member_check(c0, ctxs, b, "eval_dual_batch"); if (rc) return rc; }
        if (!nu[b]) return fail(c0, CFMM_E_ARG, "eval_dual_batch: nu[%d] is NULL", b);
        { int rc = check_prices(ctxs[b], "eval_dual_batch: nu", nu[b]); if (rc) { c0->err = ctxs[b]->err; return rc; } }
    }
    if (cfmm_pool_count(c0) == 0) return fail(c0, CFMM_E_STATE, "eval_dual_batch: no pools uploaded");
    hipStream_t stream = c0->stream;
    const int len = acc_arb(n) + 1;
    for (int b = 0; b < nb; ++b) {
        cfmm_ctx *c = ctxs[b];
        HIP_TRY(c0, hipStreamSynchronize(c->stream));
        std::memcpy(c->hnu0, nu[b], n * sizeof(double));
        HIP_TRY(c0, hipMemcpyAsync(c->nu_acc, c->hnu0, n * sizeof(double), hipMemcpyHostToDevice, stream));
        HIP_TRY(c0, hipMemcpyAsync(c->nu, c->hnu0, n * sizeof(double), hipMemcpyHostToDevice, stream));
        HIP_TRY(c0, hipMemsetAsync(c->nu + n, 0, sizeof(double), stream));
        HIP_TRY(c0, hipMemsetAsync(c->acc, 0, (size_t)c->nslices * acc_stride(n) * sizeof(double), stream));
        point_from_caller(c);
    }
    BatchEval be;
    { int rc = make_batch_eval(ctxs, nb, stream, be); if (rc) return rc; }
    launch_batch_eval(c0, be, stream, 0);
    for (int b = 0; b < nb; ++b) {
        cfmm_ctx *c = ctxs[b];
        hipLaunchKernelGGL(fold_kernel, dim3((len + 255) / 256), dim3(256), 0, stream, c->acc, n, c->nslices, 0, (const DevState *)nullptr);
        double *pin = pin_scratch(c, (size_t)len);
        if (!pin) return fail(c0, CFMM_E_HIP, "pinned staging (%d tokens)", n);
        HIP_TRY(c0, hipMemcpyAsync(pin, c->acc, len * sizeof(double), hipMemcpyDeviceToHost, stream));
        HIP_TRY(c0, hipMemsetAsync(c->acc, 0, (size_t)len * sizeof(double), stream));
    }
    HIP_TRY(c0, hipGetLastError());
    HIP_TRY(c0, hipStreamSynchronize(stream));
    for (int b = 0; b < nb; ++b) {
        const double *h = ctxs[b]->pin;
        if (psi && psi[b]) std::memcpy(psi[b], h, n * sizeof(double));
        if (arb_sum) arb_sum[b] = h[acc_arb(n)];
    }
    return CFMM_OK;
}

int cfmm_batch_capacity(int n_tokens) { return n_tokens < 1 ? 0 : batch_capacity(n_tokens); }

namespace {

struct SweepTies {
    int parent[TINY_N]; double off[TINY_N]; int n;
    void init(int n_) { n = n_; for (int j = 0; j < n; ++j) { parent[j] = j; off[j] = 0.0; } }
    int find(int j)
    {
        int path[TINY_N], np = 0;
        while (parent[j] != j) { path[np++] = j; j = parent[j]; }
        const int root = j;
        for (int q = np - 1; q >= 0; --q) {
            const int node = path[q], p = parent[node];
            if (p != root) off[node] += off[p];
            parent[node] = root;
        }
        return root;
    }
    bool tie(int a, int b, double delta)
    {
        const int ra = find(a), rb = find(b);
        if (ra == rb) return std::fabs((off[a] - off[b]) - delta) < 1e-12;
        off[ra] = delta + off[b] - off[a];
        parent[ra] = rb;
        return true;
    }
    int groups(int *grp)
    {
        int root[TINY_N]; bool is_root[TINY_N] = {};
        for (int j = 0; j < n; ++j) { root[j] = find(j); is_root[root[j]] = true; }
        int id[TINY_N], ng = 0;
        for (int j = 0; j < n; ++j) if (is_root[j]) id[j] = ng++;
        for (int j = 0; j < n; ++j) grp[j] = id[root[j]];
        return ng;
    }
};

struct SweepTie { int sgn; bool loose; };
struct SumCols { int64_t m; const int32_t *ia, *ib; const double *fee, *Ra, *Rb; };

bool small_lsq(const std::vector<double> &A, const std::vector<double> &b, int R, int K, const std::vector<int> &freev, const std::vector<double> &fixed,
               std::vector<double> &th)
{
    const int F = (int)freev.size();
    th = fixed;
    if (F == 0) return true;
    std::vector<double> N((size_t)F * F, 0.0), g(F, 0.0), rb(b);
    for (int r = 0; r < R; ++r) for (int k = 0; k < K; ++k) rb[r] -= A[(size_t)r * K + k] * fixed[k];
    double tr = 0.0;
    for (int i = 0; i < F; ++i) {
        for (int j = 0; j <= i; ++j) {
            double v = 0.0;
            for (int r = 0; r < R; ++r) v += A[(size_t)r * K + freev[i]] * A[(size_t)r * K + freev[j]];
            N[(size_t)i * F + j] = N[(size_t)j * F + i] = v;
// ... 386 lines not shown
    const auto t1 = std::chrono::steady_clock::now();
    float ms = 0.f;
    HIP_TRY(ctx, hipEventElapsedTime(&ms, ctx->ev_t0, ctx->ev_t1));
    int rc_all = CFMM_OK;
    for (int p = 0; p < B; ++p) {
        const SweepPointState &S = ps[p];
        std::memcpy(nu_out + (size_t)p * n, L.O(host, p), n * sizeof(double));
        std::memcpy(psi_out + (size_t)p * n, L.O(host, p) + n, n * sizeof(double));
        for (int i = 0; i < msum; ++i) { theta_out[(size_t)p * msum + i] = std::numeric_limits<double>::quiet_NaN(); tsgn_out[(size_t)p * msum + i] = 0; }
        if (S.fills_ok) { int k = 0; for (auto &kv : S.tied) { theta_out[(size_t)p * msum + kv.first] = S.theta[k++]; tsgn_out[(size_t)p * msum + kv.first] = kv.second.sgn; } }
        cfmm_stats *s = out + p;
        std::memset(s, 0, sizeof *s);
        s->evals = S.evals; s->iters = S.iters; s->status = S.st.status ? S.st.status : 3;
        s->n_ranks = 1;
        s->dual_value = S.st.f; s->primal_value = S.st.primal; s->gap = S.st.gap; s->infeas = S.st.infeas;
        s->wall_seconds = std::chrono::duration<double>(t1 - t0).count();
        s->device_seconds = ms * 1e-3;
        s->pg = S.st.pg;
        s->pool_subproblems = (int64_t)S.evals * pools;
        s->method = CFMM_METHOD_LBFGS;
        if (rounds_out) rounds_out[p] = S.rounds;
        if (S.st.status == CFMM_E_NUMERIC) rc_all = fail(ctx, CFMM_E_NUMERIC, "solve_sweep: dual value of point %d is not finite", p);
    }
    return rc_all;
}


int cfmm_get_trades2(cfmm_ctx *ctx, int kind, double *delta, double *lambda)
{
    if (!ctx || kind < 0 || kind >= CFMM_POOL_KINDS2) return CFMM_E_ARG;
    PoolEntry entry(ctx); HIP_TRY(ctx, entry.device);
    Bucket2 b = ctx->pools->r2[kind].b;
    if (kind == CFMM_POOL_SUM2) b.flags = ctx->flags2;
    if (b.m == 0) return CFMM_OK;
    if (ctx->pt.tr_ovr_valid) {
        size_t off = 0;
        for (int k = 0; k < kind; ++k) off += 4 * (size_t)ctx->pools->r2[k].b.m;
        if (delta) std::memcpy(delta, ctx->pt.tr_ovr.data() + off, 2 * (size_t)b.m * sizeof(double));
        if (lambda) std::memcpy(lambda, ctx->pt.tr_ovr.data() + off + 2 * (size_t)b.m, 2 * (size_t)b.m * sizeof(double));
        return CFMM_OK;
    }
    const dim3 grid((unsigned)((b.m + 255) / 256)), blk(256);
    const double *nu = ctx->nu_acc;
    return read_back(ctx, "get_trades2", 2 * (size_t)b.m, delta, lambda, [&](double *dd, double *dl) {
        with_int<0, 4>(kind, [&](auto K) {
            if (ctx->pt.mu_last > 0.0) {
                const double *slo = ctx->pt.slo_active ? ctx->sm_slo : nullptr;
                hipLaunchKernelGGL(smooth_trades_kernel<K>, grid, blk, 0, ctx->stream, b, nu, slo, ctx->pt.mu_last, dd, dl);
            } else hipLaunchKernelGGL(trades2_kernel<K>, grid, blk, 0, ctx->stream, b, nu, dd, dl);
        });
    });
}

int cfmm_get_tradesN(cfmm_ctx *ctx, int k, double *delta, double *lambda)
{
    if (!ctx || k < 3 || k > CFMM_MAX_POOL_SIZE) return CFMM_E_ARG;
    PoolEntry entry(ctx); HIP_TRY(ctx, entry.device);
    const BucketN &b = ctx->pools->rn[k].b;
    if (b.m == 0) return CFMM_OK;
    const dim3 grid((unsigned)((b.m + 255) / 256)), blk(256);
    const double *nu = ctx->nu_acc;
    const double *slo = (ctx->pt.mu_last > 0.0 && ctx->pt.slo_active) ? ctx->sm_slo : nullptr;
    return read_back(ctx, "get_tradesN", (size_t)k * b.m, delta, lambda, [&](double *dd, double *dl) {
        with_int<3, 8>(k, [&](auto K) { hipLaunchKernelGGL(tradesn_kernel<K>, grid, blk, 0, ctx->stream, b, nu, slo, dd, dl); });
    });
}

int cfmm_comm_unique_id(void *uid128)
{
    if (!uid128) return CFMM_E_ARG;
    std::string err;
    if (!g_rccl.load(err)) return fail(nullptr, CFMM_E_RCCL, "%s", err.c_str());
    ncclUniqueId id;
    int rc = g_rccl.GetUniqueId(&id);
    if (rc != 0) return fail(nullptr, CFMM_E_RCCL, "ncclGetUniqueId failed (%d)", rc);
    std::memcpy(uid128, &id, sizeof id);
    return CFMM_OK;
}

int cfmm_comm_init(cfmm_ctx *ctx, int n_ranks, int rank, const void *uid128)
{
    if (!ctx || n_ranks < 1 || rank < 0 || rank >= n_ranks || !uid128) return ctx ? fail(ctx, CFMM_E_ARG, "comm_init: bad arguments") : CFMM_E_ARG;
    HIP_TRY(ctx, hipSetDevice(ctx->device));
    std::string err;
    if (!g_rccl.load(err)) return fail(ctx, CFMM_E_RCCL, "%s", err.c_str());
    ncclUniqueId id;
    std::memcpy(&id, uid128, sizeof id);
    int rc = g_rccl.CommInitRank(&ctx->comm, n_ranks, id, rank);
    if (rc != 0) return fail(ctx, CFMM_E_RCCL, "ncclCommInitRank -> %s", g_rccl.GetErrorString ? g_rccl.GetErrorString(rc) : "error");
    ctx->n_ranks = n_ranks; ctx->rank = rank;
    ctx->g_valid = false; ctx->g_counts_valid = false;
    rc = g_rccl.AllReduce(ctx->acc, ctx->acc, (size_t)acc_stride(ctx->n), NCCL_FLOAT64, NCCL_SUM, ctx->comm, ctx->stream);
    if (rc != 0) return fail(ctx, CFMM_E_RCCL, "warm-up ncclAllReduce -> %s", g_rccl.GetErrorString ? g_rccl.GetErrorString(rc) : "error");
    HIP_TRY(ctx, hipStreamSynchronize(ctx->stream));
    return CFMM_OK;
}

int cfmm_set_deterministic(cfmm_ctx *ctx, int on)
{
    if (!ctx) return CFMM_E_ARG;
    if (on && eval_lds_bytes(ctx->n, true, true) > 160 * 1024)
        return fail(ctx, CFMM_E_LIMIT, "set_deterministic: %d tokens exceed the LDS tile of the reproducible mode (7 n doubles)", ctx->n);
    if ((on != 0) != ctx->det) { ctx->g_valid = false; ctx->g_counts_valid = false; }
    ctx->det = on != 0;
    return CFMM_OK;
}

int cfmm_debug_eval_limbs(cfmm_ctx *ctx, const double *nu, double ref_reserve, double ref_fee, uint64_t *limbs)
{
    if (!ctx || !nu || !limbs) return CFMM_E_ARG;
    PoolEntry entry(ctx); HIP_TRY(ctx, entry.device);
    const int n = ctx->n;
    if (eval_lds_bytes(n, true, true) > 160 * 1024) return fail(ctx, CFMM_E_LIMIT, "debug_eval_limbs: too many tokens for the reproducible mode");
    for (int j = 0; j < n; ++j) if (!(nu[j] > 0.0) || !std::isfinite(nu[j])) return fail(ctx, CFMM_E_ARG, "debug_eval_limbs: nu[%d] is not a positive finite price", j);
    { int rc = refresh_global_counts(ctx); if (rc) return rc; }
    const bool was = ctx->det;
    ctx->det = true; ctx->det_ref_reserve = ref_reserve; ctx->det_ref_fee = ref_fee;
    hipError_t e = hipMemcpyAsync(ctx->nu, nu, n * sizeof(double), hipMemcpyHostToDevice, ctx->stream);
    if (e == hipSuccess) e = hipMemsetAsync(ctx->nu + n, 0, sizeof(double), ctx->stream);
    if (e == hipSuccess) e = hipMemsetAsync(ctx->acc_l, 0, 6 * (size_t)n * sizeof(unsigned long long), ctx->stream);
    if (e == hipSuccess) { launch_all_evals<false>(ctx); e = hipGetLastError(); }
    if (e == hipSuccess) e = hipMemcpyAsync(limbs, ctx->acc_l, 3 * (size_t)n * sizeof(uint64_t), hipMemcpyDeviceToHost, ctx->stream);
    if (e == hipSuccess) e = hipMemsetAsync(ctx->acc_l, 0, 6 * (size_t)n * sizeof(unsigned long long), ctx->stream);
    if (e == hipSuccess) e = hipStreamSynchronize(ctx->stream);
    ctx->det = was; ctx->det_ref_reserve = 0.0; ctx->det_ref_fee = 0.0;
    if (e != hipSuccess) return fail(ctx, CFMM_E_HIP, "debug_eval_limbs -> %s", hipGetErrorString(e));
    return CFMM_OK;
}

static int oneshot_alloc(cfmm_ctx *ctx)
{
    if (ctx->os_mail) return CFMM_OK;
    ctx->os_cap = (size_t)std::max(acc_stride(ctx->n), 6 * ctx->n) + 8;
    HIP_TRY(ctx, hipMalloc((void **)&ctx->os_mail, oneshot_alloc_bytes(ctx->os_cap)));
    HIP_TRY(ctx, hipMemsetAsync(ctx->os_mail, 0, oneshot_alloc_bytes(ctx->os_cap), ctx->stream));
    HIP_TRY(ctx, hipStreamSynchronize(ctx->stream));
    return CFMM_OK;
}

void *cfmm_oneshot_mailbox(cfmm_ctx *ctx)
{
    if (!ctx || hipSetDevice(ctx->device) != hipSuccess || oneshot_alloc(ctx) != CFMM_OK) return nullptr;
    return ctx->os_mail;
}

int cfmm_oneshot_export(cfmm_ctx *ctx, void *handle64)
{
    if (!ctx || !handle64) return CFMM_E_ARG;
    HIP_TRY(ctx, hipSetDevice(ctx->device));
    { int rc = oneshot_alloc(ctx); if (rc) return rc; }
    hipIpcMemHandle_t h;
    static_assert(sizeof(hipIpcMemHandle_t) == 64, "IPC handle size");
    HIP_TRY(ctx, hipIpcGetMemHandle(&h, ctx->os_mail));
    std::memcpy(handle64, &h, sizeof h);
    return CFMM_OK;
}

int cfmm_oneshot_attach(cfmm_ctx *ctx, int n_ranks, int rank, void *const *mailboxes)
{
    if (!ctx || !mailboxes || n_ranks < 1 || n_ranks > ONESHOT_MAX_RANKS || rank < 0 || rank >= n_ranks)
        return ctx ? fail(ctx, CFMM_E_ARG, "oneshot_attach: %d ranks (at most %d), rank %d", n_ranks, ONESHOT_MAX_RANKS, rank) : CFMM_E_ARG;
    HIP_TRY(ctx, hipSetDevice(ctx->device));
    { int rc = oneshot_alloc(ctx); if (rc) return rc; }
    if (ctx->comm && ctx->n_ranks != n_ranks) return fail(ctx, CFMM_E_STATE, "oneshot_attach: the RCCL communicator has %d ranks", ctx->n_ranks);
    for (int r = 0; r < n_ranks; ++r) {
        ctx->os_peers[r] = r == rank ? ctx->os_mail : (unsigned long long *)mailboxes[r];
        if (!ctx->os_peers[r]) return fail(ctx, CFMM_E_ARG, "oneshot_attach: mailbox of rank %d is NULL", r);
    }
    ctx->n_ranks = n_ranks; ctx->rank = rank;
    HIP_TRY(ctx, hipMemsetAsync(ctx->os_mail, 0, oneshot_alloc_bytes(ctx->os_cap), ctx->stream));
    HIP_TRY(ctx, hipStreamSynchronize(ctx->stream));
    ctx->os_ready = true; ctx->g_valid = false; ctx->g_counts_valid = false;
    return CFMM_OK;
}

int cfmm_oneshot_import(cfmm_ctx *ctx, int n_ranks, int rank, const void *handles)
{
    if (!ctx || !handles || n_ranks < 1 || n_ranks > ONESHOT_MAX_RANKS || rank < 0 || rank >= n_ranks) return ctx ? fail(ctx, CFMM_E_ARG, "oneshot_import: bad arguments") : CFMM_E_ARG;
    HIP_TRY(ctx, hipSetDevice(ctx->device));
    void *ptrs[ONESHOT_MAX_RANKS] = {};
    for (int r = 0; r < n_ranks; ++r) {
        if (r == rank) continue;
        hipIpcMemHandle_t h;
        std::memcpy(&h, (const char *)handles + 64 * (size_t)r, sizeof h);
        void *p = nullptr;
        hipError_t e = hipIpcOpenMemHandle(&p, h, hipIpcMemLazyEnablePeerAccess);
        if (e != hipSuccess) return fail(ctx, CFMM_E_HIP, "oneshot_import: hipIpcOpenMemHandle(rank %d) -> %s", r, hipGetErrorString(e));
        ctx->os_opened.push_back(p);
        ptrs[r] = p;
    }
    return cfmm_oneshot_attach(ctx, n_ranks, rank, ptrs);
}

int cfmm_oneshot_enable(cfmm_ctx *ctx, int on)
{
    if (!ctx) return CFMM_E_ARG;
    if (on && !ctx->os_peers[ctx->rank]) return fail(ctx, CFMM_E_STATE, "oneshot_enable: no mailboxes attached (cfmm_oneshot_import / _attach first)");
    if (!on && !ctx->comm && ctx->os_ready) return fail(ctx, CFMM_E_STATE, "oneshot_enable(0): no RCCL communicator to fall back on");
    HIP_TRY(ctx, hipSetDevice(ctx->device));
    HIP_TRY(ctx, hipStreamSynchronize(ctx->stream));
    if ((on != 0) != ctx->os_ready) drop_graph(ctx);
    ctx->os_ready = on != 0; ctx->g_counts_valid = false;
    return CFMM_OK;
}

int cfmm_selftest(cfmm_ctx *ctx)
{
    if (!ctx) return CFMM_E_ARG;
    HIP_TRY(ctx, hipSetDevice(ctx->device));
    int *d = nullptr, h = -1;
    HIP_TRY(ctx, hipMalloc((void **)&d, sizeof(int)));
    HIP_TRY(ctx, hipMemsetAsync(d, 0, sizeof(int), ctx->stream));
    hipLaunchKernelGGL(selftest_kernel, dim3(1), dim3(64), 0, ctx->stream, d);
    hipLaunchKernelGGL(selftest_gram_kernel, dim3(1), dim3(64), 0, ctx->stream, d);
    hipLaunchKernelGGL(selftest_log_kernel, dim3(1), dim3(64), 0, ctx->stream, d);
    hipLaunchKernelGGL(selftest_generic_kernel, dim3(1), dim3(64), 0, ctx->stream, d);
    hipLaunchKernelGGL(selftest_table_kernel, dim3(1), dim3(64), 0, ctx->stream, d);
    hipError_t e = hipMemcpyAsync(&h, d, sizeof(int), hipMemcpyDeviceToHost, ctx->stream);
    if (e == hipSuccess) e = hipStreamSynchronize(ctx->stream);
    (void)hipFree(d);
    if (e != hipSuccess) return fail(ctx, CFMM_E_HIP, "selftest -> %s", hipGetErrorString(e));
    if (h != 0) return fail(ctx, CFMM_E_NUMERIC, "selftest: %d results of the cross-lane reductions / the fast logarithm / the generic pool solver are wrong on this device / ROCm", h);
    return CFMM_OK;
}

int cfmm_debug_timers(cfmm_ctx *ctx, int64_t *out64)
{
    if (!ctx || !out64) return CFMM_E_ARG;
    HIP_TRY(ctx, hipSetDevice(ctx->device));
    HIP_TRY(ctx, hipStreamSynchronize(ctx->stream));
    HIP_TRY(ctx, hipMemcpy(out64, ctx->ts, (64 + 8 * 4096 + 2048) * sizeof(int64_t), hipMemcpyDeviceToHost));
    HIP_TRY(ctx, hipMemset(ctx->ts, 0, (64 + 8 * 4096 + 2048) * sizeof(int64_t)));
    return CFMM_OK;
}


int cfmm_clock_probe_start(cfmm_ctx *ctx, double period_us, double max_ms)
{
    if (!ctx || !(period_us >= 1.0) || !(max_ms > 0.0) || max_ms > 60000.0) return CFMM_E_ARG;
    HIP_TRY(ctx, hipSetDevice(ctx->device));
    if (ctx->probe_running) return fail(ctx, CFMM_E_STATE, "clock probe: already running (cfmm_clock_probe_stop first)");
    if (!ctx->probe_stream) HIP_TRY(ctx, hipStreamCreateWithFlags(&ctx->probe_stream, hipStreamNonBlocking));
    if (!ctx->probe_ring) {
        HIP_TRY(ctx, hipHostMalloc((void **)&ctx->probe_ring, (2 * PROBE_CAP + 8) * sizeof(long long), hipHostMallocMapped));
        HIP_TRY(ctx, hipHostGetDevicePointer((void **)&ctx->probe_ring_d, ctx->probe_ring, 0));
    }
    std::memset(ctx->probe_ring, 0, (2 * PROBE_CAP + 8) * sizeof(long long));
    hipLaunchKernelGGL(clock_probe_kernel, dim3(1), dim3(64), 0, ctx->probe_stream, ctx->probe_ring_d, PROBE_CAP,
                       (long long)(period_us * 100.0), (long long)(max_ms * 1e5));
    HIP_TRY(ctx, hipGetLastError());
    ctx->probe_running = true;
    return CFMM_OK;
}
int cfmm_clock_probe_read(cfmm_ctx *ctx, int64_t *out, int cap, int *count)
{
    if (!ctx || !count || (cap > 0 && !out)) return CFMM_E_ARG;
    *count = 0;
    if (!ctx->probe_ring) return CFMM_OK;
    const long long head = __atomic_load_n(reinterpret_cast<volatile long long *>(ctx->probe_ring) + 2 * PROBE_CAP + 1, __ATOMIC_ACQUIRE);
    const int k = (int)std::min<long long>(std::min<long long>(head, PROBE_CAP), cap);
    for (int i = 0; i < 2 * k; ++i) out[i] = reinterpret_cast<volatile long long *>(ctx->probe_ring)[i];
    *count = k;
    return CFMM_OK;
}
int cfmm_clock_probe_chain(cfmm_ctx *ctx, int64_t *out3)
{
    if (!ctx || !out3) return CFMM_E_ARG;
    for (int i = 0; i < 3; ++i) out3[i] = ctx->probe_ring ? reinterpret_cast<volatile long long *>(ctx->probe_ring)[2 * PROBE_CAP + 2 + i] : 0;
    return CFMM_OK;
}
int cfmm_clock_probe_stop(cfmm_ctx *ctx, int64_t *out, int cap, int *count)
{
    if (!ctx) return CFMM_E_ARG;
    if (ctx->probe_running) {
        HIP_TRY(ctx, hipSetDevice(ctx->device));
        __atomic_store_n(reinterpret_cast<volatile long long *>(ctx->probe_ring) + 2 * PROBE_CAP, 1ll, __ATOMIC_RELEASE);
        HIP_TRY(ctx, hipStreamSynchronize(ctx->probe_stream));
        ctx->probe_running = false;
    }
    int dummy = 0;
    return cfmm_clock_probe_read(ctx, out, cap, count ? count : &dummy);
}

int cfmm_time_xcd_handoff(cfmm_ctx *ctx, int np, int reps, double *out7)
{
    double *out6 = out7;
    if (!ctx || !out6 || np < 1 || np > 8192 || reps < 1) return CFMM_E_ARG;
    HIP_TRY(ctx, hipSetDevice(ctx->device));
    const int grid = ctx->cus;
    double *pub = nullptr; unsigned long long *flag = nullptr; long long *stamps = nullptr;
    HIP_TRY(ctx, hipMalloc(&pub, (size_t)16 * np * sizeof(double)));
    HIP_TRY(ctx, hipMalloc(&flag, 16 * 16 * sizeof(unsigned long long)));
    HIP_TRY(ctx, hipMalloc(&stamps, (size_t)4 * grid * sizeof(long long)));
    HIP_TRY(ctx, hipMemset(flag, 0, 16 * 16 * sizeof(unsigned long long)));
    (void)hipFuncSetAttribute((const void *)xcd_handoff_kernel, hipFuncAttributeMaxDynamicSharedMemorySize, 128 * 1024);
    std::vector<long long> h((size_t)4 * grid);
    std::vector<double> full, seen;
    int wrong_xcc = 0, failed = 0, orphan = 0;
    for (int r = 0; r < reps; ++r) {
        hipLaunchKernelGGL(xcd_handoff_kernel, dim3(grid), dim3(1024), (size_t)96 * 1024, ctx->stream, pub, flag, (unsigned long long)(r + 1), np, 500ll, stamps);
        HIP_TRY(ctx, hipGetLastError());
        HIP_TRY(ctx, hipMemcpyAsync(h.data(), stamps, h.size() * sizeof(long long), hipMemcpyDeviceToHost, ctx->stream));
        HIP_TRY(ctx, hipStreamSynchronize(ctx->stream));
        long long ready[16]; bool have[16] = {};
        for (int b = 0; b < 8 && b < grid; ++b) { const int x = (int)h[4 * b] & 15; ready[x] = h[4 * b + 1]; have[x] = true; }
        long long worst = 0, worst_seen = 0;
        wrong_xcc = 0; orphan = 0;
        for (int x = 0; x < 8; ++x) orphan += !have[x];
        for (int b = 0; b < grid; ++b) {
            const int x = (int)h[4 * b] & 15;
            wrong_xcc += x != b % 8;
            if (b < 8) continue;
            if (h[4 * b + 3] != 0 || !have[x]) { ++failed; continue; }
            worst = std::max(worst, h[4 * b + 2] - ready[x]);
            worst_seen = std::max(worst_seen, h[4 * b + 1] - ready[x]);
        }
        full.push_back(worst * 0.01); seen.push_back(worst_seen * 0.01);
    }
    std::sort(full.begin(), full.end()); std::sort(seen.begin(), seen.end());
    out6[0] = full[full.size() / 2]; out6[1] = full.back(); out6[2] = seen[seen.size() / 2];
    out6[3] = wrong_xcc; out6[4] = failed; out6[5] = orphan;
    out7[6] = 0.0;
    for (int b = 0; b < 8 && b < grid; ++b) out7[6] = 10.0 * out7[6] + (double)((int)h[4 * b] & 15 ? ((int)h[4 * b] & 15) % 10 : 0);
    (void)hipFree(pub); (void)hipFree(flag); (void)hipFree(stamps);
    return CFMM_OK;
}

int cfmm_time_eval_kernel(cfmm_ctx *ctx, int kind, int reps, double *sec_per_launch)
{
    if (!ctx || reps < 1 || !sec_per_launch) return CFMM_E_ARG;
    PoolEntry entry(ctx); HIP_TRY(ctx, entry.device);
    if (!ctx->pt.have_nu) return fail(ctx, CFMM_E_STATE, "time_eval_kernel: no prices set");
    HIP_TRY(ctx, hipMemcpyAsync(ctx->nu, ctx->nu_acc, ctx->n * sizeof(double), hipMemcpyDeviceToDevice, ctx->stream));
    HIP_TRY(ctx, hipMemsetAsync(ctx->nu + ctx->n, 0, sizeof(double), ctx->stream));
    const int only = kind == CFMM_TIME_ALL ? 0x7fffffff : kind;
    const bool table_only = kind == CFMM_TIME_TABLE;
    const EvalArgs ea = make_eval_args(ctx, false, only), es = make_eval_args(ctx, true, only);
    if (table_only ? table_pools(ctx) == 0 : ea.ntiles + es.ntiles == 0) return fail(ctx, CFMM_E_ARG, "time_eval_kernel: bucket %d is empty", kind);
    auto launch = [&]() {
        if (table_only) { launch_table_evals<false>(ctx, ctx->nu, ctx->acc); return; }
        launch_eval<false, false>(ctx, ea); launch_eval<false, true>(ctx, es);
        if (kind == CFMM_TIME_ALL && table_pools(ctx) > 0) launch_table_evals<false>(ctx, ctx->nu, ctx->acc);
    };
    for (int i = 0; i < 3; ++i) launch();
    HIP_TRY(ctx, hipEventRecord(ctx->ev_t0, ctx->stream));
    for (int i = 0; i < reps; ++i) launch();
    HIP_TRY(ctx, hipEventRecord(ctx->ev_t1, ctx->stream));
    HIP_TRY(ctx, hipMemsetAsync(ctx->acc, 0, (size_t)ctx->nslices * acc_stride(ctx->n) * sizeof(double), ctx->stream));
    if (ctx->det) HIP_TRY(ctx, hipMemsetAsync(ctx->acc_l, 0, 6 * (size_t)ctx->n * sizeof(unsigned long long), ctx->stream));
    HIP_TRY(ctx, hipStreamSynchronize(ctx->stream));
    HIP_TRY(ctx, hipGetLastError());
    float ms = 0.f;
    HIP_TRY(ctx, hipEventElapsedTime(&ms, ctx->ev_t0, ctx->ev_t1));
    *sec_per_launch = ms * 1e-3 / reps;
    return CFMM_OK;
}

int cfmm_time_newton_kernels(cfmm_ctx *ctx, double mu, int reps, double *out4)
{
    if (!ctx || reps < 1 || !out4 || !(mu > 0.0)) return CFMM_E_ARG;
    PoolEntry entry(ctx); HIP_TRY(ctx, entry.device);
    const char *why = "";
    if (!newton_supported(ctx, &why)) return fail(ctx, CFMM_E_UNSUPPORTED, "time_newton_kernels: %s", why);
    const int n = ctx->n, nr = hess_nr(n), ld = hess_ld(n);
    int rc = smooth_buffers(ctx, true); if (rc) return rc;
    if (!ctx->pt.have_nu) return fail(ctx, CFMM_E_STATE, "time_newton_kernels: no prices (cfmm_set_nu or a solve first)");
    HIP_TRY(ctx, hipMemcpyAsync(ctx->nu, ctx->nu_acc, n * sizeof(double), hipMemcpyDeviceToDevice, ctx->stream));
    HIP_TRY(ctx, hipMemsetAsync(ctx->sm_mask, 0, n * sizeof(int), ctx->stream));
    for (int k = 0; k < CFMM_POOL_KINDS2; ++k)
        if (ctx->sm_ws[k]) HIP_TRY(ctx, hipMemsetAsync(ctx->sm_ws[k], 0, 2 * (size_t)ctx->pools->r2[k].b.m * sizeof(double), ctx->stream));
    float ms = 0.f;
    for (int which = 0; which < 2; ++which) {
        if ((rc = launch_smooth(ctx, mu, which == 0, true, false))) return rc;
        HIP_TRY(ctx, hipEventRecord(ctx->ev_t0, ctx->stream));
        for (int i = 0; i < reps; ++i) if ((rc = launch_smooth(ctx, mu, which == 0, true, false))) return rc;
        HIP_TRY(ctx, hipEventRecord(ctx->ev_t1, ctx->stream));
        HIP_TRY(ctx, hipStreamSynchronize(ctx->stream));
        HIP_TRY(ctx, hipEventElapsedTime(&ms, ctx->ev_t0, ctx->ev_t1));
        out4[which] = ms * 1e-3 / reps;
    }
    if ((rc = launch_smooth(ctx, mu, true, true, false))) return rc;
    std::vector<double> hd(n, 0.0), rhs(n, 1.0);
    {
        std::vector<double> col(n);
        double mx = 0.0;
        for (int j = 0; j < n; j += std::max(1, n / 64)) {
            HIP_TRY(ctx, hipMemcpy(&col[j], ctx->H + (size_t)j * ld + j, sizeof(double), hipMemcpyDeviceToHost));
            mx = std::max(mx, std::fabs(col[j]));
        }
        for (int j = 0; j < n; ++j) hd[j] = 1e-3 * std::max(mx, 1e-300);
    }
    HIP_TRY(ctx, hipMemcpyAsync(ctx->sm_vec, hd.data(), n * sizeof(double), hipMemcpyHostToDevice, ctx->stream));
    HIP_TRY(ctx, hipMemcpyAsync(ctx->sm_vec + n, rhs.data(), n * sizeof(double), hipMemcpyHostToDevice, ctx->stream));
    hipLaunchKernelGGL(hess_finish_kernel, dim3(1024), dim3(256), 0, ctx->stream, ctx->H, n, nr, ld, (const double *)ctx->sm_vec,
                       (const int *)ctx->sm_mask, (const double *)(ctx->sm_vec + n));
    struct Scratch {
        double *keep = nullptr; hipEvent_t ev_end = nullptr;
        ~Scratch() { if (ev_end) (void)hipEventDestroy(ev_end); if (keep) (void)hipFree(keep); }
    } sc;
    HIP_TRY(ctx, hipMalloc((void **)&sc.keep, (size_t)ld * nr * sizeof(double)));
    double *const keep = sc.keep;
    HIP_TRY(ctx, hipMemcpyAsync(keep, ctx->H, (size_t)ld * nr * sizeof(double), hipMemcpyDeviceToDevice, ctx->stream));
    double fac = 0.0, back = 0.0;
    HIP_TRY(ctx, hipEventCreate(&sc.ev_end));
    const hipEvent_t ev_end = sc.ev_end;
    for (int i = 0; i < reps && rc == CFMM_OK; ++i) {
        if (hipMemcpyAsync(ctx->H, keep, (size_t)ld * nr * sizeof(double), hipMemcpyDeviceToDevice, ctx->stream) != hipSuccess) { rc = CFMM_E_HIP; break; }
        (void)hipEventRecord(ctx->ev_t0, ctx->stream);
        rc = launch_factor(ctx, n);
        (void)hipEventRecord(ctx->ev_t1, ctx->stream);
        if (rc == CFMM_OK) rc = launch_backsolve(ctx, n, ctx->sm_vec + n);
        (void)hipEventRecord(ev_end, ctx->stream);
        if (hipStreamSynchronize(ctx->stream) != hipSuccess) { rc = CFMM_E_HIP; break; }
        (void)hipEventElapsedTime(&ms, ctx->ev_t0, ctx->ev_t1); fac += ms * 1e-3;
        (void)hipEventElapsedTime(&ms, ctx->ev_t1, ev_end); back += ms * 1e-3;
    }
    drop_barrier(ctx);
    if (rc) { const std::string prev = ctx->err; return fail(ctx, rc, "time_newton_kernels: the factorisation launches failed (%s; %s)", prev.c_str(), hipGetErrorString(hipGetLastError())); }
    out4[2] = fac / reps; out4[3] = back / reps;
    return CFMM_OK;
}

int cfmm_time_collective(cfmm_ctx *ctx, int reps, double *fold_sec, double *allreduce_sec)
{
    if (!ctx || reps < 1) return CFMM_E_ARG;
    HIP_TRY(ctx, hipSetDevice(ctx->device));
    const int n = ctx->n, len = acc_arb(n) + 1;
    float ms = 0.f;
    HIP_TRY(ctx, hipMemsetAsync(ctx->acc, 0, (size_t)ctx->nslices * acc_stride(n) * sizeof(double), ctx->stream));
    const bool folded_inside = ctx->os_ready && (size_t)len <= ctx->os_cap && !ctx->det;
    cfmm_opts od; cfmm_default_opts(&od); od.memory = 3;
    const bool unfolded = rccl_unfolded(ctx) && fused_applies(ctx, od);
    if (fold_sec) *fold_sec = 0.0;
    if (!folded_inside && !unfolded) {
        HIP_TRY(ctx, hipEventRecord(ctx->ev_t0, ctx->stream));
        for (int i = 0; i < reps; ++i)
            hipLaunchKernelGGL(fold_kernel, dim3((len + 255) / 256), dim3(256), 0, ctx->stream, ctx->acc, n, ctx->nslices, 0, (const DevState *)nullptr);
        HIP_TRY(ctx, hipEventRecord(ctx->ev_t1, ctx->stream));
        HIP_TRY(ctx, hipStreamSynchronize(ctx->stream));
        HIP_TRY(ctx, hipEventElapsedTime(&ms, ctx->ev_t0, ctx->ev_t1));
        if (fold_sec) *fold_sec = ms * 1e-3 / reps;
    }
    if (allreduce_sec) *allreduce_sec = 0.0;
    if (sharded(ctx) && allreduce_sec) {
        const int fs = folded_inside ? ctx->nslices : 1;
        const size_t cnt = unfolded ? (size_t)(ctx->nslices - 1) * acc_stride(n) + len : (size_t)len;
        for (int i = 0; i < 3; ++i) { int rc = all_reduce(ctx, ctx->acc, cnt, NCCL_FLOAT64, NCCL_SUM, nullptr, fs); if (rc) return rc; }
        HIP_TRY(ctx, hipEventRecord(ctx->ev_t0, ctx->stream));
        for (int i = 0; i < reps; ++i) { int rc = all_reduce(ctx, ctx->acc, cnt, NCCL_FLOAT64, NCCL_SUM, nullptr, fs); if (rc) return rc; }
        HIP_TRY(ctx, hipEventRecord(ctx->ev_t1, ctx->stream));
        HIP_TRY(ctx, hipStreamSynchronize(ctx->stream));
        HIP_TRY(ctx, hipEventElapsedTime(&ms, ctx->ev_t0, ctx->ev_t1));
        *allreduce_sec = ms * 1e-3 / reps;
    }
    return CFMM_OK;
}

}
```

### cfmm-routing-code_amd/csrc/iterate.hpp

```cpp
#pragma once
#include <utility>
#include "kernels.hpp"

namespace cfmm {

#ifndef ITER_E_SMALL_DEF
#define ITER_E_SMALL_DEF 2
#endif
constexpr int ITER_E_SMALL = ITER_E_SMALL_DEF;
constexpr int ITER_MM = 3;
constexpr int ITER_P = ITER_MM + 1;
constexpr int GI_U = 8, GI_V = GI_U + ITER_P, GI_SY = GI_V + ITER_P, GI_YHY = GI_SY + ITER_P * (ITER_P - 1) / 2,
              GI_END = GI_YHY + ITER_P * (ITER_P + 1) / 2;
static_assert(GI_END <= 32, "the batch must fit one 32-value reduce-scatter");
constexpr int XS_HIST = 5;
constexpr int XS_VECS = XS_HIST + 2 * ITER_MM;
__host__ __device__ inline int iter_xvs(int n) { return (n + 3) & ~1; }

constexpr int ITER_HRING = 1024;
__host__ __device__ inline unsigned long long iter_hring_word(int evals, int status, int launch)
{
    return (unsigned long long)((unsigned)evals & 0xffffffu) | ((unsigned long long)((unsigned)status & 0xffu) << 24) | ((unsigned long long)(unsigned)launch << 32);
}
struct IterArgs {
    EvalArgs ev;
    int n, M, nread, phase;
    int xvs, max_evals, pg_rule;
    int plain;
    double *acc3; long long acc_set;
    double *xs; long long xs_set;
    DevState *st3;
    const double *c, *h, *glo, *ghi;
    const int *ctype;
    double *Ds;
    double *nu, *nu_acc, *psi_acc;
    double tol_gap, tol_infeas, armijo, max_step;
    unsigned long long *hstat;
    unsigned long long *hring;
    int launch;
    double *h_nu_acc, *h_psi_acc;
    DevState *h_final;
};

template <int E> __device__ __forceinline__ void ldE(const double *p, int first, double (&v)[E]);
template <> __device__ __forceinline__ void ldE<1>(const double *p, int first, double (&v)[1]) { v[0] = p[first]; }
template <> __device__ __forceinline__ void ldE<2>(const double *p, int first, double (&v)[2])
{
    const double2 t = *reinterpret_cast<const double2 *>(p + first);
    v[0] = t.x; v[1] = t.y;
}
template <int E> __device__ __forceinline__ void ldEi(const int *p, int first, int (&v)[E]);
template <> __device__ __forceinline__ void ldEi<1>(const int *p, int first, int (&v)[1]) { v[0] = p[first]; }
template <> __device__ __forceinline__ void ldEi<2>(const int *p, int first, int (&v)[2])
{
    const int2 t = *reinterpret_cast<const int2 *>(p + first);
    v[0] = t.x; v[1] = t.y;
}
template <int E> __device__ __forceinline__ void stE(double *p, int first, int len, const double (&v)[E])
{
    if (E == 2 && first + 1 < len) { *reinterpret_cast<double2 *>(p + first) = make_double2(v[0], v[E - 1]); return; }
    if (first < len) p[first] = v[0];
}

template <int E> __device__ __forceinline__ void stX(double *p, int first, const double (&v)[E])
{
    if (E == 2) *reinterpret_cast<double2 *>(p + first) = make_double2(v[0], v[E - 1]);
    else p[first] = v[0];
}

template <int E>
struct GramIn {
    double g1[8];
    double S[ITER_P][E], Y[ITER_P][E], q0[E], H0[E], hq[E];
};
__host__ __device__ constexpr int sy_row(int c) { int k = 1; while (k * (k + 1) / 2 <= c) ++k; return k; }
__host__ __device__ constexpr int yhy_row(int c) { int k = 0; while ((k + 1) * (k + 2) / 2 <= c) ++k; return k; }
template <int I, int E>
__device__ __forceinline__ double gram_val(const GramIn<E> &in)
{
    double r = 0.0;
    if constexpr (I < GI_U) r = in.g1[I];
    else if constexpr (I < GI_V) {
#pragma unroll
        for (int e = 0; e < E; ++e) r = fma(in.S[I - GI_U][e], in.q0[e], r);
    } else if constexpr (I < GI_SY) {
#pragma unroll
        for (int e = 0; e < E; ++e) r = fma(in.Y[I - GI_V][e], in.hq[e], r);
    } else if constexpr (I < GI_YHY) {
        constexpr int c = I - GI_SY, k = sy_row(c), j = c - k * (k - 1) / 2;
        static_assert(j >= 0 && j < k && k < ITER_P, "SY index");
#pragma unroll
        for (int e = 0; e < E; ++e) r = fma(in.S[k][e], in.Y[j][e], r);
    } else if constexpr (I < GI_END) {
        constexpr int c = I - GI_YHY, k = yhy_row(c), j = c - k * (k + 1) / 2;
        static_assert(j >= 0 && j <= k && k < ITER_P, "YHY index");
#pragma unroll
        for (int e = 0; e < E; ++e) r = fma(in.H0[e] * in.Y[k][e], in.Y[j][e], r);
    }
    return r;
}

template <int I, int E>
__device__ __forceinline__ double gram_pair16(const GramIn<E> &in)
{
    const double a = gram_val<I, E>(in), b = gram_val<I + 16, E>(in);
    const int l0 = __double2loint(a), h0 = __double2hiint(a);
    const int l1 = __double2loint(b), h1 = __double2hiint(b);
    const auto lo = __builtin_amdgcn_permlane16_swap(l0, l1, false, false);
    const auto hi = __builtin_amdgcn_permlane16_swap(h0, h1, false, false);
    return __hiloint2double(hi[0], lo[0]) + __hiloint2double(hi[1], lo[1]);
}
template <int E, int... I>
__device__ __forceinline__ void gram_pairs16(const GramIn<E> &in, double (&v)[16], std::integer_sequence<int, I...>)
{
    ((v[I] = gram_pair16<I, E>(in)), ...);
}
__device__ __forceinline__ double row_halve4(double (&v)[8], int lane)
{
    const bool b4 = lane & 4, b2 = lane & 2, b1 = lane & 1;
#pragma unroll
    for (int i = 0; i < 4; ++i) {
        const double keep = b4 ? v[i + 4] : v[i], send = b4 ? v[i] : v[i + 4];
        v[i] = keep + swz_xor4(send);
    }
// ... 69 lines not shown
{
    extern __shared__ __attribute__((aligned(16))) double lds_raw[];
    constexpr int SLOT = STAGE_BYTES / 8, NSLOT = EVAL_THREADS / 64;
    double *const stage0 = lds_raw;
    double *const lds = lds_raw + (DMA ? NSLOT * SLOT : 0);
    constexpr int MM = ITER_MM, P = ITER_P;
    static_assert(MM == 3, "DevState::rhow0..2 hold a window of 3");
    const int n = a.n, M = a.M;
    const int tid = threadIdx.x, lane = tid & 63, wave = uni((int)(threadIdx.x >> 6)), nw = blockDim.x >> 6;
    const int tile = eval_tile_doubles(n, DET);
    double *psi_s = lds;
    double *nu_s = lds + tile;
    double *fpart = nu_s + n + 2;
    int *next_tile = reinterpret_cast<int *>(fpart + 16);
    double *strips = lds + eval_lds_doubles(n, false, DET);
    constexpr bool LNU = eval_has_lnu(false, DET) && !DMA;
    double *lnu_s = lds + eval_lnu_offset(n, false, DET);
    double *xw = strips;
    double *xm = xw + 16 * 32;
    BlockRed red(xm + 32);
    double *ctl = xm + 32 + 2 * BlockRed::NRED * 16;
    int *ctli = reinterpret_cast<int *>(ctl + 2 * ITER_P + 2);
    double *gst_s = psi_s;
    double *sts_s = nu_s;
    double *glo_s = strips + 2 * 64 * (EVAL_THREADS / 64);
    double *ghi_s = glo_s + a.xvs;
    double *psi_k = DMA ? stage0 + NSLOT * SLOT - 2 * a.xvs : ghi_s + a.xvs, *nu_k = psi_k + a.xvs;
    double *fsafe = (DMA ? ghi_s : ghi_s + 2 * a.xvs) + a.xvs;
    const int first_late = (NSLOT * SLOT - 2 * a.xvs) / SLOT;

#ifdef CFMM_PHASE_TIMERS
    const long long ts_c16 = clock64(), ts_w16 = wall_clock64();
#endif
    const int p = a.phase, pr = (p + 2) % 3, pz = (p + 1) % 3;
    const int stride = acc_stride(n), xvs = a.xvs;
    const double *Xr = a.xs + (size_t)pr * a.xs_set;
    double *Xw = a.xs + (size_t)p * a.xs_set;
    const double *Ar = a.acc3 + (size_t)pr * a.acc_set;
    enum { R_STATE = 0, R_S = 0, R_ST = 1, R_GS = 2, R_D = 3, R_NU = 4, R_SW = 5, R_YW = 5 + ITER_MM, R_PSI_ACC = 5 + 2 * ITER_MM, R_NU_ACC, R_DS };
    const bool wide = gridDim.x > R_DS;
    const bool has_role = !wide || blockIdx.x <= R_DS;
    auto mine = [&](int role) { return wide ? blockIdx.x == (unsigned)role : blockIdx.x == (unsigned)role % gridDim.x; };
    const bool wr = mine(R_STATE);
    const int r0 = tid * E;
    const int ld0 = (r0 < n) ? r0 : 0;
    bool tin[E];
#pragma unroll
    for (int e = 0; e < E; ++e) tin[e] = r0 + e < n;
    const bool wave_active = wave * 64 * E < n;
    const int nwa = (n + 64 * E - 1) / (64 * E);
    red.nw = nwa;
    GramIn<E> in;
    double s[E], s_t[E], Gs[E], nuj[E], Ds[E], glo[E], ghi[E], hj[E], cj[E], psi[E];
    int ct[E];
#pragma unroll
    for (int e = 0; e < E; ++e) {
        s[e] = s_t[e] = Gs[e] = nuj[e] = Ds[e] = glo[e] = cj[e] = 0.0; psi[e] = 0.0; ghi[e] = __builtin_inf(); hj[e] = 0.0; ct[e] = 0;
        in.q0[e] = in.H0[e] = in.hq[e] = 0.0;
#pragma unroll
        for (int k = 0; k < P; ++k) { in.S[k][e] = 0.0; in.Y[k][e] = 0.0; }
    }
    if (wave_active) {
        ldE<E>(Xr, ld0, s); ldE<E>(Xr + xvs, ld0, s_t); ldE<E>(Xr + 2 * xvs, ld0, Gs); ldE<E>(Xr + 4 * xvs, ld0, nuj);
        ldE<E>(a.Ds, ld0, Ds); ldE<E>(a.glo, ld0, glo); ldE<E>(a.c, ld0, cj);
        if (!PLAIN) { ldE<E>(a.ghi, ld0, ghi); ldE<E>(a.h, ld0, hj); ldEi<E>(a.ctype, ld0, ct); }
        for (int sl = 0; sl < a.nread; ++sl) {
            double t1[E];
            ldE<E>(Ar + (size_t)sl * stride, ld0, t1);
#pragma unroll
            for (int e = 0; e < E; ++e) psi[e] += t1[e];
        }
#pragma unroll
        for (int k = 0; k < MM; ++k) {
            ldE<E>(Xr + (size_t)(XS_HIST + k) * xvs, ld0, in.S[k + 1]);
            ldE<E>(Xr + (size_t)(XS_HIST + MM + k) * xvs, ld0, in.Y[k + 1]);
        }
    }
    if (DET) for (int j = n + tid; j < tile; j += blockDim.x) psi_s[j] = 0.0;
    DevState st = a.st3[pr];
    if (st.status != 0) {
        if (blockIdx.x == 0 && tid == 0) {
            a.st3[p] = st;
            if (a.hring) __hip_atomic_store(a.hring + (a.launch & (ITER_HRING - 1)), iter_hring_word(st.evals, st.status, a.launch), __ATOMIC_RELAXED, __HIP_MEMORY_SCOPE_SYSTEM);
        }
        return;
    }
    st.evals = uni(st.evals); st.iters = uni(st.iters); st.first = uni(st.first); st.hist = uni(st.hist);
    st.nrej = uni(st.nrej); st.f = uni(st.f); st.t_step = uni(st.t_step);
    long long *const tsb = (st.evals + 1 < a.max_evals) ? a.ev.ts : nullptr;
    (void)tsb;
    PHASE_STAMP(tsb, 17);

    if (blockIdx.x == gridDim.x - 1) {
        double *Z = a.acc3 + (size_t)pz * a.acc_set;
        const int len = a.ev.nslices * stride;
        for (int j = tid; j < len; j += blockDim.x) Z[j] = 0.0;
    }

    bool act[E];
#pragma unroll
    for (int e = 0; e < E; ++e) act[e] = true;
    const bool keeps_acc = has_role && (mine(R_PSI_ACC) || mine(R_NU_ACC));
    if (wave_active) {
        double mx[2] = {0.0, 0.0};
        if (st.first) {
            double dg[E];
#pragma unroll
            for (int e = 0; e < E; ++e) dg[e] = 0.0;
            for (int sl = 0; sl < a.nread; ++sl) {
                double t2[E];
                ldE<E>(Ar + (size_t)sl * stride + acc_diag(n), ld0, t2);
#pragma unroll
                for (int e = 0; e < E; ++e) dg[e] += t2[e];
            }
#pragma unroll
            for (int e = 0; e < E; ++e) Ds[e] = dg[e];
            if (has_role && r0 < n && mine(R_DS)) stE<E>(a.Ds, r0, n, Ds);
        }
#pragma unroll
        for (int k = 0; k < MM; ++k) {
            const bool have = k < st.hist;
#pragma unroll
            for (int e = 0; e < E; ++e) if (!have || !tin[e]) { in.S[k + 1][e] = 0.0; in.Y[k + 1][e] = 0.0; }
        }
        double fpools = 0.0;
        if (tid < a.nread) fpools = Ar[(size_t)tid * stride + acc_arb(n)];
#pragma unroll
        for (int i = 0; i < 8; ++i) in.g1[i] = 0.0;
        in.g1[0] = fpools;
        double Gs_t[E];
#pragma unroll
        for (int e = 0; e < E; ++e) {
            Gs_t[e] = 0.0;
            if (tin[e]) {
                const double rj = PLAIN ? psi[e] : psi[e] + hj[e];
                Gs_t[e] = nuj[e] * rj;
                if (!PLAIN) in.g1[0] += (nuj[e] - cj[e]) * hj[e];
                in.g1[1] += (nuj[e] - cj[e]) * rj;
                mx[0] = fmax(mx[0], (PLAIN || ct[e] == 0) ? fmax(-rj, 0.0) : (ct[e] == 1 ? fabs(rj) : 0.0));
                mx[1] = fmax(mx[1], PLAIN ? fabs(psi[e]) : fmax(fabs(psi[e]), fabs(hj[e])));
                const double sv = s_t[e] - s[e], yv = Gs_t[e] - Gs[e];
                if (!st.first) {
                    in.S[0][e] = sv; in.Y[0][e] = yv;
                    in.g1[2] += Gs[e] * sv; in.g1[3] += Gs_t[e] * sv;
                    in.g1[4] += sv * yv; in.g1[5] += sv * sv; in.g1[6] += yv * yv;
                }
                const double G = Gs_t[e], sr = s_t[e];
                double v = G;
                if (!PLAIN && glo[e] == ghi[e]) v = 0.0;
                else if (sr <= glo[e] + 1e-14) v = fmin(G, 0.0);
                else if (!PLAIN && sr >= ghi[e] - 1e-14) v = fmax(G, 0.0);
                in.g1[7] += fabs(v);
                act[e] = PLAIN ? (sr <= glo[e] + 1e-14 && G > 0.0) : is_active(sr, glo[e], ghi[e], G);
                in.q0[e] = act[e] ? 0.0 : G;
                const double H = Ds[e] + fmax(G, 0.0);
                in.H0[e] = H > 0.0 ? rcp_nr(H) : 0.0;
                in.hq[e] = in.H0[e] * in.q0[e];
                gst_s[r0 + e] = Gs_t[e];
                sts_s[r0 + e] = s_t[e]; glo_s[r0 + e] = glo[e];
                if (!PLAIN) ghi_s[r0 + e] = ghi[e];
                if (keeps_acc) { psi_k[r0 + e] = psi[e]; nu_k[r0 + e] = nuj[e]; }
            }
        }
        PHASE_STAMP(tsb, 18);
        const double qa = gram_reduce32<E>(in, lane);
        PHASE_STAMP(tsb, 19);
// ... 115 lines not shown
#pragma unroll
        for (int e = 0; e < E; ++e) if (tin[e]) psi_s[r0 + e] = 0.0;
        if (keeps_acc && accept && r0 < n) {
            double pk[E], nk[E];
#pragma unroll
            for (int e = 0; e < E; ++e) { pk[e] = tin[e] ? psi_k[r0 + e] : 0.0; nk[e] = tin[e] ? nu_k[r0 + e] : 0.0; }
            if (mine(R_PSI_ACC)) { stE<E>(a.psi_acc, r0, n, pk); if (a.h_psi_acc) stE<E>(a.h_psi_acc, r0, n, pk); }
            if (mine(R_NU_ACC)) { stE<E>(a.nu_acc, r0, n, nk); if (a.h_nu_acc) stE<E>(a.h_nu_acc, r0, n, nk); }
        }
    }

    auto trial = [&](double step) {
#pragma unroll
        for (int e = 0; e < E; ++e) {
            v[e] = fmax(s[e] + step * d[e], glo[e]);
            if (!PLAIN) v[e] = fmin(v[e], ghi[e]);
            nn[e] = tin[e] ? exp(v[e]) : 0.0;
        }
    };
    double F[2] = {0.0, 0.0};
    bool F_pending = false;
    auto safeguard = [&](double (&F)[2]) {
        bool redo = false;
        if (!(F[0] < 0.0) && gp_sq > 0.0) {
            st.hist = 0;
            double m1[1] = {0.0};
#pragma unroll
            for (int e = 0; e < E; ++e) {
                d[e] = (!tin[e] || act[e]) ? 0.0 : -Gs[e] * in.H0[e];
                m1[0] = fmax(m1[0], fabs(d[e]));
            }
            red.put<0, 1>(m1, wave_active);
            red.template get<0, 1, DMA>(m1);
            F[1] = m1[0];
            redo = true;
        }
        st.t_step = lbfgs::step_cap(F[1], a.max_step);
        const bool again = redo || st.t_step != 1.0;
        if (again && wave_active) trial(st.t_step);
        return again;
    };
    if (new_dir) {
        if (wave_active) {
#pragma unroll
            for (int e = 0; e < E; ++e) {
                double qm = in.q0[e], rs = 0.0;
#pragma unroll
                for (int k = 0; k < P; ++k) { qm -= al[k] * in.Y[k][e]; rs += ga[k] * in.S[k][e]; }
                d[e] = (tin[e] && !act[e]) ? -(in.H0[e] * qm + rs) : 0.0;
                F[0] += d[e] * Gs[e]; F[1] = fmax(F[1], fabs(d[e]));
            }
        }
#ifndef CFMM_EAGER_SAFEGUARD
        F_pending = st.evals < a.max_evals;
#endif
        if (F_pending) {
            if (wave_active) {
                F[0] = wave_allsum(F[0]); F[1] = wave_allmax(F[1]);
                if (lane == 0) { fsafe[wave] = F[0]; fsafe[16 + wave] = F[1]; }
                trial(1.0);
            }
        } else {
            red.put<1, 1>(F, wave_active);
            if (wave_active) trial(1.0);
            red.template get<1, 1, DMA>(F);
            (void)safeguard(F);
        }
    } else if (st.status == 0 && wave_active) trial(st.t_step);

    if (st.status == 0 && st.evals >= a.max_evals) st.status = 3;
    auto store_state = [&]() {
        if (has_role && wave_active && r0 < n) {
            if (mine(R_S)) stX<E>(Xw, r0, s);
            if (mine(R_ST)) stX<E>(Xw + xvs, r0, v);
            if (mine(R_GS)) stX<E>(Xw + 2 * xvs, r0, Gs);
            if (mine(R_D)) stX<E>(Xw + 3 * xvs, r0, d);
            if (mine(R_NU)) stX<E>(Xw + 4 * xvs, r0, nn);
            if (wr) stE<E>(a.nu, r0, n, nn);
        }
        if (wr) {
            if (tid == 0) {
                a.st3[p] = st; a.nu[n] = st.status != 0 ? 1.0 : 0.0;
                if (st.status != 0 && a.h_final) *a.h_final = st;
                if (a.hstat) __hip_atomic_store(a.hstat, (unsigned long long)(unsigned)st.evals | ((unsigned long long)(unsigned)st.status << 32),
                                                __ATOMIC_RELAXED, __HIP_MEMORY_SCOPE_SYSTEM);
                if (a.hring) __hip_atomic_store(a.hring + (a.launch & (ITER_HRING - 1)), iter_hring_word(st.evals, st.status, a.launch), __ATOMIC_RELAXED, __HIP_MEMORY_SCOPE_SYSTEM);
            }
        }
    };
    if (st.status != 0) {
        store_state();
        if constexpr (DMA) dma_wait();
        return;
    }
    PHASE_STAMP(a.ev.ts, 22);
    auto publish = [&]() {
#pragma unroll
        for (int e = 0; e < E; ++e) if (tin[e]) { nu_s[r0 + e] = nn[e]; if constexpr (LNU) lnu_s[r0 + e] = v[e]; }
    };
    publish();
    if constexpr (DMA) {
        if (helper_mode && !wave_active) dma_wait();
        lds_barrier();
    } else
    __syncthreads();
    PHASE_STAMP(a.ev.ts, 23);
    if (F_pending) {
        F[0] = 0.0; F[1] = 0.0;
        for (int w = 0; w < nwa; ++w) { F[0] += fsafe[w]; F[1] = fmax(F[1], fsafe[16 + w]); }
        if (safeguard(F)) {
            publish();
            if constexpr (DMA) lds_barrier(); else __syncthreads();
        }
    }
    store_state();
#ifdef CFMM_PHASE_TIMERS
    if (a.ev.ts && tid == 0) {
        if (blockIdx.x == 0) { a.ev.ts[2 * 16] = ts_c16; a.ev.ts[2 * 16 + 1] = ts_w16; }
        if (blockIdx.x < 256) { long long *tb = a.ev.ts + 64 + 8 * 4096; tb[2 * blockIdx.x] = ts_w16; tb[2 * (blockIdx.x + 256)] = wall_clock64(); }
    }
#endif
    double2 *xs = reinterpret_cast<double2 *>(strips) + 64 * wave;
    if constexpr (DMA)
        eval_tiles_and_flush<false, false, DET, false, true, true>(a.ev, a.acc3 + (size_t)p * a.acc_set, nu_s, psi_s, nullptr, fpart, next_tile, xs,
                                                                   BatchCtl{1u, 0, 0}, nullptr, stage0 + SLOT * wave, !dma_late);
    else
    eval_tiles_and_flush<false, false, DET, false, true, false, NT, LNU>(a.ev, a.acc3 + (size_t)p * a.acc_set, nu_s, psi_s, nullptr, fpart, next_tile, xs,
                                                                         BatchCtl{1u, 0, 0}, nullptr, nullptr, false, lnu_s);
#ifdef CFMM_PHASE_TIMERS
    __syncthreads();
    if (a.ev.ts && tid == 0 && blockIdx.x < 256) a.ev.ts[64 + 8 * 4096 + 2 * blockIdx.x + 1] = wall_clock64();
#endif
}

}
```

### cfmm-routing-code_amd/csrc/kernels.hpp

```cpp
#pragma once
#include "pool_math.hpp"
#include "phi2.hpp"
#include "lbfgs_rules.hpp"

namespace cfmm {

#ifdef CFMM_PHASE_TIMERS
#define PHASE_STAMP(buf, i) do { if ((buf) && blockIdx.x == 0 && threadIdx.x == 0) { (buf)[2 * (i)] = clock64(); (buf)[2 * (i) + 1] = wall_clock64(); } } while (0)
#else
#define PHASE_STAMP(buf, i) do { } while (0)
#endif

#ifndef EVAL_THREADS_DEF
#define EVAL_THREADS_DEF 1024
#endif
constexpr int EVAL_THREADS = EVAL_THREADS_DEF;
#ifndef EVAL_WAVES_PER_SIMD
#define EVAL_WAVES_PER_SIMD 4
#endif
constexpr int UPD_THREADS = 1024;
constexpr int MAX_MEMORY = 8;

#ifndef WT_LIGHT_DEF
#define WT_LIGHT_DEF 128
// ... 1944 lines not shown
selftest_kernel(int *out)
{
    const int lane = threadIdx.x;
    int bad = 0;
    const double x = (double)((lane * 37 + 11) % 101) - 50.0;
    double ts = 0.0, tm = -1e300;
    for (int l = 0; l < 64; ++l) { const double v = (double)((l * 37 + 11) % 101) - 50.0; ts += v; tm = fmax(tm, v); }
    if (wave_allsum(x) != ts) ++bad;
    if (wave_allmax(x) != tm) ++bad;
    double V[64];
#pragma unroll
    for (int i = 0; i < 64; ++i) V[i] = (double)(((lane + 3) * (i + 5)) % 23) - 7.0;
    double want = 0.0;
    for (int l = 0; l < 64; ++l) want += (double)(((l + 3) * (lane + 5)) % 23) - 7.0;
    if (wave_reduce_scatter64(V, lane) != want) ++bad;
    atomicAdd(out, bad);
}

__global__ void __launch_bounds__(64)
selftest_generic_kernel(int *out)
{
    int bad = 0;
    unsigned long long st = 0x9E3779B97F4A7C15ull * (threadIdx.x + 1);
    auto rnd = [&]() { st ^= st << 13; st ^= st >> 7; st ^= st << 17; return (double)(st >> 11) * (1.0 / 9007199254740992.0); };
    for (int k = 0; k < 48; ++k) {
        const double Ra = exp(10.0 * rnd() - 2.0), Rb = exp(10.0 * rnd() - 2.0);
        const double g = 1.0 - 0.01 * rnd();
        const double pa = exp(0.6 * rnd() - 0.3), wa = 0.1 + 0.8 * rnd(), t = 0.05 + 0.9 * rnd();
        auto cmp = [&](const Y2 &a, const Y2 &b) {
            if (!(fabs(a.ya - b.ya) <= 1e-11 * Ra && fabs(a.yb - b.yb) <= 1e-11 * Rb)) ++bad;
        };
        {
            const double pb = pa * Ra / Rb * exp(0.6 * rnd() - 0.3);
            cmp(pool_generic2<0>(Ra, Rb, g, 0.0, pa, pb), pool_cp2(Ra, Rb, g, pa, pb));
        }
        {
            const double pb = pa * (1.0 - wa) / wa * Ra / Rb * exp(0.6 * rnd() - 0.3);
            cmp(pool_generic2<1>(Ra, Rb, g, wa, pa, pb), pool_w2(Ra, Rb, g, wa, pa, pb));
        }
        {
            const double Rb2 = Ra * exp(0.4 * rnd() - 0.2), al = Ra * Ra * Rb2 * (0.05 + rnd());
            const double pb = pa * exp(0.02 * rnd() - 0.01);
            const Y2 a = pool_generic2<3>(Ra, Rb2, g, al, pa, pb), b = pool_curve2(Ra, Rb2, g, al, pa, pb);
            if (!(fabs(a.ya - b.ya) <= 1e-10 * Ra && fabs(a.yb - b.yb) <= 1e-10 * Rb2)) ++bad;
        }
        {
            const double pb = pa * exp(t * log(Ra / Rb)) * exp(0.6 * rnd() - 0.3);
            const Y2 a = pool_generic2<4>(Ra, Rb, g, t, pa, pb);
            Y2 b; b.ya = 0.0; b.yb = 0.0;
            const double q = 1.0 - t, K = exp(q * log(Ra)) + exp(q * log(Rb));
            auto dir = [&](double Rin, double Rout, double ni, double no, double &yin, double &yout) {
                if (!(no * g * exp(t * log(Rout / Rin)) > ni)) return false;
                const double rho = ni / (g * no);
                const double x = exp(log(K / (1.0 + exp((q / t) * log(rho)))) / q), y = x * exp(log(rho) / t);
                yin = -(x - Rin) / g; yout = Rout - y;
                return true;
            };
            if (!dir(Ra, Rb, pa, pb, b.ya, b.yb)) dir(Rb, Ra, pb, pa, b.yb, b.ya);
            if (!(fabs(a.ya - b.ya) <= 1e-10 * Ra && fabs(a.yb - b.yb) <= 1e-10 * Rb)) ++bad;
        }
    }
    atomicAdd(out, bad);
}

__global__ void __launch_bounds__(64)
selftest_log_kernel(int *out)
{
    int bad = 0;
    for (int k = 0; k < 256; ++k) {
        const int i = k * 64 + threadIdx.x;
        double x;
        if (i < 8192) x = exp((i - 4096) * (690.0 / 4096.0));
        else x = 1.0 + (i - 12288) * (1.0 / 8192.0) * ((i & 1) ? 1.0 : 1e-6);
        if (!(x > 0.0)) continue;
        const double a = log_pos(x), b = log(x);
        const double ulp = fmax(fabs(b), 1e-300) * 2.220446049250313e-16;
        if (!(fabs(a - b) <= 2.0 * ulp + 1e-320)) ++bad;
    }
    if (bad) atomicAdd(out, bad);
}

template <bool BATCH = false>
__global__ void __launch_bounds__(UPD_THREADS)
start_kernel(UpdArgs a0, const double *nu0_, double *zero, long long nzero, DevState *st_clear, int n_clear)
{
    const UpdArgs &a = upd_args<BATCH>(a0);
    const double *nu0 = BATCH ? a.nu_acc : nu0_;
    if (BATCH) { zero = a.acc; }
    for (long long j = threadIdx.x; j < nzero; j += blockDim.x) zero[j] = 0.0;
    if ((int)threadIdx.x < n_clear) { DevState z = {}; st_clear[threadIdx.x] = z; }
    extern __shared__ __attribute__((aligned(16))) double lds[];
    double *sum = lds, *cnt = lds + a.ng;
    const int tid = threadIdx.x, nt = blockDim.x;
    const int n = a.n, ng = a.ng;
    for (int r = tid; r < ng; r += nt) { sum[r] = 0.0; cnt[r] = 0.0; }
    __syncthreads();
    if (a.gptr && ng != n) {
        for (int r = tid; r < ng; r += nt) {
            double v = 0.0;
            const int m1 = a.gptr[r + 1];
            for (int m = a.gptr[r]; m < m1; ++m) { const int t = a.gmem[m]; v += log(nu0[t]) - a.off[t]; }
            sum[r] = v; cnt[r] = (double)(m1 - a.gptr[r]);
        }
    } else
    for (int j = tid; j < n; j += nt) {
        unsafeAtomicAdd(&sum[a.grp[j]], log(nu0[j]) - a.off[j]);
        unsafeAtomicAdd(&cnt[a.grp[j]], 1.0);
    }
    __syncthreads();
    for (int r = tid; r < ng; r += nt) {
        double v = sum[r] / fmax(cnt[r], 1.0);
        v = fmax(v, a.glo[r]);
        v = fmin(v, a.ghi[r]);
        sum[r] = v;
        a.s_t[r] = v; a.s[r] = v; a.d[r] = 0.0;
    }
    __syncthreads();
    for (int j = tid; j < n; j += nt) { const double v = exp(sum[a.grp[j]] + a.off[j]); a.nu[j] = v; a.nu_acc[j] = v; }
    if (tid == 0) {
        DevState st = {};
        st.status = 0; st.evals = 0; st.iters = 0; st.first = 1; st.hist = 0; st.head = 0; st.nrej = 0; st.pad = 0;
        st.f = 0.0; st.t_step = 1.0; st.gap = 0.0; st.infeas = 0.0; st.primal = 0.0; st.pg = 0.0;
        *a.st = st;
        a.nu[n] = 0.0;
        report_progress(a, st);
    }
}

}
```

Measured before the change: 47.15 billion pool-subproblems/s.

## Seal zero-copy solve with device epoch record instead of stream synchronize

On the zero-copy fused path, the host stops synchronizing the stream before and after each solve. Completion is detected by spinning on a mapped epoch-tagged seal word that the kernel writes, and device time comes from wall_clock64 stamps in place of hip events. The leftover stream tail is drained lazily by a settle() call in every other API entry point. This removes the synchronize and event overhead around each solve, but adds the risk of missing a settle call somewhere and an extra enqueued iteration after convergence.

Measured after the change: 48.67 billion pool-subproblems/s (median of 6 runs). 3.2% higher.

```diff
diff --git a/cfmm-routing-code_amd/csrc/cfmm_hip.hip b/cfmm-routing-code_amd/csrc/cfmm_hip.hip
--- a/cfmm-routing-code_amd/csrc/cfmm_hip.hip
+++ b/cfmm-routing-code_amd/csrc/cfmm_hip.hip
@@ -202,6 +202,11 @@
     volatile unsigned long long *hstat_h = nullptr;
     unsigned long long *hstat_d = nullptr;
     int run_ahead = 3;
+    volatile EnvRec *env_h = nullptr;
+    EnvRec *env_d = nullptr;
+    unsigned epoch = 0;
+    bool tail = false;
+    double wall_clock_hz = 1e8;
     std::vector<char> listed;
     bool listed_valid = false;
     UpdArgs *upd_batch_d = nullptr, *upd_batch_h = nullptr;
@@ -269,6 +274,14 @@
         hipError_t e_ = (call);                                                                   \
         if (e_ != hipSuccess) return fail(ctx, CFMM_E_HIP, "%s -> %s (%s:%d)", #call, hipGetErrorString(e_), __FILE__, __LINE__); \
     } while (0)
+
+inline int settle(cfmm_ctx *ctx)
+{
+    if (!ctx->tail) return CFMM_OK;
+    ctx->tail = false;
+    HIP_TRY(ctx, hipStreamSynchronize(ctx->stream));
+    return CFMM_OK;
+}
 
 inline bool sharded(const cfmm_ctx *ctx) { return ctx->comm != nullptr || ctx->os_ready; }
 inline bool rccl_unfolded(const cfmm_ctx *ctx)
@@ -1522,7 +1535,8 @@
     const char *why = "";
     if (!newton_supported(ctx, &why)) return fail(ctx, CFMM_E_UNSUPPORTED, "solve: the second-order method cannot take this problem: %s", why);
     const int n = ctx->n;
-    int rc = smooth_buffers(ctx, true); if (rc) return rc;
+    int rc = settle(ctx); if (rc) return rc;
+    rc = smooth_buffers(ctx, true); if (rc) return rc;
     const std::vector<double> &c = ctx->hc, &h = ctx->hh;
     const std::vector<int> &ct = ctx->hctype;
 
@@ -1991,9 +2005,18 @@
         std::memset(ctx->util_h, 0, ctx->util_span);
     }
     lap("device + pinned arenas");
-    TRY_C(hipHostMalloc((void **)&ctx->hstat_h, 64 + ITER_HRING * sizeof(unsigned long long), hipHostMallocMapped));
+    TRY_C(hipHostMalloc((void **)&ctx->hstat_h, 64 + ITER_HRING * sizeof(unsigned long long) + 64, hipHostMallocMapped));
     TRY_C(hipHostGetDevicePointer((void **)&ctx->hstat_d, (void *)ctx->hstat_h, 0));
     *ctx->hstat_h = 0;
+    static_assert(sizeof(EnvRec) <= 64, "the envelope record has 64 bytes behind the ring");
+    ctx->env_h = reinterpret_cast<volatile EnvRec *>(ctx->hstat_h + 8 + ITER_HRING);
+    ctx->env_d = reinterpret_cast<EnvRec *>(ctx->hstat_d + 8 + ITER_HRING);
+    ctx->env_h->prog = 0; ctx->env_h->seal = 0; ctx->env_h->t0 = 0; ctx->env_h->t1 = 0;
+    {
+        int khz = 0;
+        if (hipDeviceGetAttribute(&khz, hipDeviceAttributeWallClockRate, device) == hipSuccess && khz > 0) ctx->wall_clock_hz = 1e3 * khz;
+        else (void)hipGetLastError();
+    }
     lap("mapped progress word");
     for (int i = 0; i < 2; ++i) TRY_C(hipEventCreateWithFlags(&ctx->ev[i], hipEventDisableTiming));
     TRY_C(hipEventCreate(&ctx->ev_t0));
@@ -2032,6 +2055,7 @@
 {
     if (!src || !out) return CFMM_E_ARG;
     HIP_TRY(src, hipSetDevice(src->device));
+    { int rc_ = settle(src); if (rc_) return rc_; }
     pools_ready(src);
     HIP_TRY(src, hipStreamSynchronize(src->stream));
     release_landed(src);
@@ -2057,6 +2081,7 @@
     if (!ctx) return CFMM_OK;
     (void)hipSetDevice(ctx->device);
     if (ctx->stream) (void)hipStreamSynchronize(ctx->stream);
+    ctx->tail = false;
     drop_graph(ctx);
     if (ctx->comm && g_rccl.CommDestroy) g_rccl.CommDestroy(ctx->comm);
     for (void *q : ctx->os_opened) (void)hipIpcCloseMemHandle(q);
@@ -2251,10 +2276,13 @@
     PoolStore &ps;
     const bool reader;
     hipError_t device;
-    explicit PoolEntry(cfmm_ctx *c, bool rd = true) : ctx(c), ps(*c->pools), reader(rd)
+    explicit PoolEntry(cfmm_ctx *c, bool rd = true, bool keep_tail = false) : ctx(c), ps(*c->pools), reader(rd)
     {
         if (reader) { std::lock_guard<std::mutex> g(ps.mu); ++ps.readers; }
-        if ((device = hipSetDevice(c->device)) == hipSuccess) pools_ready(c);
+        if ((device = hipSetDevice(c->device)) == hipSuccess) {
+            if (!keep_tail && c->tail) { c->tail = false; device = hipStreamSynchronize(c->stream); }
+            if (device == hipSuccess) pools_ready(c);
+        }
     }
     ~PoolEntry() { release_landed(ctx); if (reader) { std::lock_guard<std::mutex> g(ps.mu); --ps.readers; } }
 };
@@ -2272,6 +2300,7 @@
 static int upload_begin(cfmm_ctx *ctx, const char *who, const void *old_arena)
 {
     HIP_TRY(ctx, hipSetDevice(ctx->device));
+    { int rc_ = settle(ctx); if (rc_) return rc_; }
     if (ctx->pools.use_count() > 1) return fail(ctx, CFMM_E_STATE, "%s: the pools are shared with a clone (cfmm_clone); destroy the clones first", who);
     if (old_arena) HIP_TRY(ctx, hipStreamSynchronize(ctx->stream));
     return CFMM_OK;
@@ -2735,6 +2764,7 @@
 {
     if (!ctx || !c) return ctx ? fail(ctx, CFMM_E_ARG, "set_utility: c is NULL") : CFMM_E_ARG;
     HIP_TRY(ctx, hipSetDevice(ctx->device));
+    { int rc_ = settle(ctx); if (rc_) return rc_; }
     const int n = ctx->n;
     bool general = false;
     for (int j = 0; j < n; ++j) {
@@ -2774,6 +2804,7 @@
 {
     if (!ctx) return CFMM_E_ARG;
     HIP_TRY(ctx, hipSetDevice(ctx->device));
+    { int rc_ = settle(ctx); if (rc_) return rc_; }
     const int n = ctx->n;
     if (!grp) {
         ctx->ng = n;
@@ -2817,6 +2848,7 @@
 {
     if (!ctx || !nu) return CFMM_E_ARG;
     HIP_TRY(ctx, hipSetDevice(ctx->device));
+    { int rc_ = settle(ctx); if (rc_) return rc_; }
     { int rc = check_prices(ctx, "set_nu: nu", nu); if (rc) return rc; }
     HIP_TRY(ctx, hipStreamSynchronize(ctx->stream));
     std::memcpy(ctx->hnu0, nu, ctx->n * sizeof(double));
@@ -2829,6 +2861,7 @@
 {
     if (!ctx || !nu) return CFMM_E_ARG;
     HIP_TRY(ctx, hipSetDevice(ctx->device));
+    { int rc_ = settle(ctx); if (rc_) return rc_; }
     HIP_TRY(ctx, hipMemcpyAsync(nu, ctx->nu_acc, ctx->n * sizeof(double), hipMemcpyDeviceToHost, ctx->stream));
     HIP_TRY(ctx, hipStreamSynchronize(ctx->stream));
     return CFMM_OK;
@@ -2838,6 +2871,7 @@
 {
     if (!ctx || !psi) return CFMM_E_ARG;
     HIP_TRY(ctx, hipSetDevice(ctx->device));
+    { int rc_ = settle(ctx); if (rc_) return rc_; }
     pools_seen(ctx);
     HIP_TRY(ctx, hipMemcpyAsync(psi, ctx->psi_acc, ctx->n * sizeof(double), hipMemcpyDeviceToHost, ctx->stream));
     HIP_TRY(ctx, hipStreamSynchronize(ctx->stream));
@@ -2854,6 +2888,7 @@
         return CFMM_OK;
     }
     HIP_TRY(ctx, hipSetDevice(ctx->device));
+    { int rc_ = settle(ctx); if (rc_) return rc_; }
     if (nu) HIP_TRY(ctx, hipMemcpyAsync(nu, ctx->nu_acc, ctx->n * sizeof(double), hipMemcpyDeviceToHost, ctx->stream));
     if (psi) HIP_TRY(ctx, hipMemcpyAsync(psi, ctx->psi_acc, ctx->n * sizeof(double), hipMemcpyDeviceToHost, ctx->stream));
     HIP_TRY(ctx, hipStreamSynchronize(ctx->stream));
@@ -2941,6 +2976,7 @@
 {
     if (!ctx || !A || !b || !x || n != ctx->n) return ctx ? fail(ctx, CFMM_E_ARG, "debug_cholesky: n must equal the context's token count") : CFMM_E_ARG;
     HIP_TRY(ctx, hipSetDevice(ctx->device));
+    { int rc_ = settle(ctx); if (rc_) return rc_; }
     int rc = smooth_buffers(ctx, true); if (rc) return rc;
     const int ld = hess_ld(n);
     std::vector<double> hd(n, 0.0);
@@ -2965,6 +3001,7 @@
 {
     if (!ctx || !b || !x || n != ctx->n || !ctx->H) return ctx ? fail(ctx, CFMM_E_STATE, "debug_cholesky_apply: call cfmm_debug_cholesky first") : CFMM_E_ARG;
     HIP_TRY(ctx, hipSetDevice(ctx->device));
+    { int rc_ = settle(ctx); if (rc_) return rc_; }
     HIP_TRY(ctx, hipMemcpyAsync(ctx->sm_vec + n, b, n * sizeof(double), hipMemcpyHostToDevice, ctx->stream));
     { int rc = launch_chord(ctx, n, ctx->sm_vec + n, ctx->sm_vec); if (rc) return rc; }
     HIP_TRY(ctx, hipMemcpyAsync(x, ctx->sm_vec, n * sizeof(double), hipMemcpyDeviceToHost, ctx->stream));
@@ -3064,7 +3101,7 @@
 int cfmm_solve(cfmm_ctx *ctx, const double *nu0, const cfmm_opts *opts_in, cfmm_stats *out)
 {
     if (!ctx || !out) return CFMM_E_ARG;
-    PoolEntry entry(ctx); HIP_TRY(ctx, entry.device);
+    PoolEntry entry(ctx, true, true); HIP_TRY(ctx, entry.device);
     drop_tenders(ctx);
     cfmm_opts o;
     if (opts_in) o = *opts_in; else cfmm_default_opts(&o);
@@ -3179,18 +3216,30 @@
     ctx->nu0_deferred = false;
     static const bool zc_off = getenv("CFMM_ZERO_COPY") && atoi(getenv("CFMM_ZERO_COPY")) == 0;
     const bool zero_copy = fused && !shard && !use_graph_opt && !ctx->det && !zc_off;
+    static const bool env_classic = getenv("CFMM_ENVELOPE") && !strcmp(getenv("CFMM_ENVELOPE"), "classic");
+    const bool sealed = zero_copy && !env_classic && o.max_evals < 0xffffff;
+    unsigned epoch = 0;
+    if (sealed) {
+        if (++ctx->epoch == 0) ++ctx->epoch;
+        epoch = ctx->epoch;
+        ia.env = ctx->env_d; ia.epoch = epoch; ia.hstat = nullptr;
+    } else {
+        HIP_TRY(ctx, hipStreamSynchronize(ctx->stream));
+        ctx->tail = false;
+    }
     if (zero_copy) { ia.h_nu_acc = ctx->hsol_d; ia.h_psi_acc = ctx->hsol_d + n; ia.h_final = ctx->hst_d; ctx->hst[0] = DevState{}; }
 
-    HIP_TRY(ctx, hipStreamSynchronize(ctx->stream));
     const auto t0 = std::chrono::steady_clock::now();
-    HIP_TRY(ctx, hipEventRecord(ctx->ev_t0, ctx->stream));
-    *ctx->hstat_h = 0;
+    if (!sealed) {
+        HIP_TRY(ctx, hipEventRecord(ctx->ev_t0, ctx->stream));
+        *ctx->hstat_h = 0;
+    }
     if (ctx->det) HIP_TRY(ctx, hipMemsetAsync(ctx->acc_l, 0, 6 * (size_t)n * sizeof(unsigned long long), ctx->stream));
     if (fused) {
         double *x0 = ctx->xs3;
         ua.s = x0; ua.s_t = x0 + ia.xvs; ua.Gs = x0 + 2 * ia.xvs; ua.d = x0 + 3 * ia.xvs; ua.nu = x0 + 4 * ia.xvs; ua.st = ctx->st3;
         hipLaunchKernelGGL(start_kernel<false>, dim3(1), dim3(UPD_THREADS), upd_lds_bytes(ctx->ng), ctx->stream, ua, nu_src,
-                           ctx->acc3, (long long)(3 * aset), ctx->st3 + 1, 2);
+                           ctx->acc3, (long long)(3 * aset), ctx->st3 + 1, 2, sealed ? (long long *)&ctx->env_d->t0 : (long long *)nullptr);
         for (int stable = 0; stable < 2; ++stable) {
             EvalArgs e0 = make_eval_args(ctx, stable != 0);
             e0.nu = ua.nu; e0.acc = ctx->acc3;
@@ -3230,15 +3279,25 @@
     } else if (fused && (!shard || oneshot_runahead(ctx)) && !use_graph_opt) {
         const auto spin0 = std::chrono::steady_clock::now();
         long spins = 0;
+        int done = 0;
         for (;;) {
-            const unsigned long long w = *ctx->hstat_h;
-            const int done = (int)(w & 0xffffffffu);
-            status = (int)(w >> 32);
+            if (sealed) {
+                const unsigned long long w = ctx->env_h->prog;
+                const bool cur = (unsigned)(w >> 32) == epoch;
+                done = cur ? (int)(w & 0xffffffu) : 0;
+                status = cur ? (int)((w >> 24) & 0xffu) : 0;
+            } else {
+                const unsigned long long w = *ctx->hstat_h;
+                done = (int)(w & 0xffffffffu);
+                status = (int)(w >> 32);
+            }
             if (status != 0) break;
             if (t > o.max_evals + 1) {
-                HIP_TRY(ctx, hipStreamSynchronize(ctx->stream));
-                break;
-            }
+                if (!sealed) {
+                    HIP_TRY(ctx, hipStreamSynchronize(ctx->stream));
+                    break;
+                }
+            } else
             if (t - done <= ctx->run_ahead) {
                 int rc = enqueue_fused_iteration(ctx, ia, t); if (rc) return rc;
                 ++t; spins = 0;
@@ -3250,6 +3309,7 @@
             }
         }
         HIP_TRY(ctx, hipGetLastError());
+        if (sealed && t < done + 2) { int rc = enqueue_fused_iteration(ctx, ia, t); if (rc) return rc; ++t; HIP_TRY(ctx, hipGetLastError()); }
     } else if (fused && shard && !use_graph) {
         volatile unsigned long long *ring = ctx->hstat_h + 8;
         for (int q = 0; q < ITER_HRING; ++q) ring[q] = 0;
@@ -3291,12 +3351,23 @@
             if (status != 0) break;
         }
     }
-    HIP_TRY(ctx, hipEventRecord(ctx->ev_t1, ctx->stream));
+    if (!sealed) HIP_TRY(ctx, hipEventRecord(ctx->ev_t1, ctx->stream));
     if (zero_copy) {
-        HIP_TRY(ctx, hipStreamSynchronize(ctx->stream));
+        bool drained = !sealed;
+        if (sealed) {
+            const auto spin0 = std::chrono::steady_clock::now();
+            long spins = 0;
+            while ((unsigned)(ctx->env_h->seal >> 32) != epoch) {
+                if ((++spins & 0xfffff) == 0 && (hipGetLastError() != hipSuccess || std::chrono::duration<double>(std::chrono::steady_clock::now() - spin0).count() > 120.0)) { drained = true; break; }
+            }
+            std::atomic_thread_fence(std::memory_order_acquire);
+            ctx->tail = !drained;
+        }
+        if (drained) HIP_TRY(ctx, hipStreamSynchronize(ctx->stream));
         hring[0] = ctx->hst[0];
         for (int q = 1; q < nst; ++q) hring[q] = DevState{};
         if (hring[0].status == 0) {
+            { int rc = settle(ctx); if (rc) return rc; }
             HIP_TRY(ctx, hipMemcpy(hring, dst, nst * sizeof(DevState), hipMemcpyDeviceToHost));
             HIP_TRY(ctx, hipMemcpy(ctx->hsol, ctx->nu_acc, n * sizeof(double), hipMemcpyDeviceToHost));
             HIP_TRY(ctx, hipMemcpy(ctx->hsol + n, ctx->psi_acc, n * sizeof(double), hipMemcpyDeviceToHost));
@@ -3311,7 +3382,14 @@
     { double mx = 0.0; for (int j = 0; j < n; ++j) mx = std::max(mx, ctx->hsol[j]); if (mx > 0.0 && std::isfinite(mx)) ctx->nu_max = mx; }
     const auto t1 = std::chrono::steady_clock::now();
     float ms = 0.f;
-    HIP_TRY(ctx, hipEventElapsedTime(&ms, ctx->ev_t0, ctx->ev_t1));
+    double dev_s = 0.0;
+    if (sealed) {
+        const long long c0 = ctx->env_h->t0, c1 = ctx->env_h->t1;
+        if (c1 > c0) dev_s = (double)(c1 - c0) / ctx->wall_clock_hz;
+    } else {
+        HIP_TRY(ctx, hipEventElapsedTime(&ms, ctx->ev_t0, ctx->ev_t1));
+        dev_s = ms * 1e-3;
+    }
 
     const DevState st = newest(hring);
     std::memset(out, 0, sizeof *out);
@@ -3319,7 +3397,7 @@
     out->n_ranks = ctx->n_ranks;
     out->dual_value = st.f; out->primal_value = st.primal; out->gap = st.gap; out->infeas = st.infeas;
     out->wall_seconds = std::chrono::duration<double>(t1 - t0).count();
-    out->device_seconds = ms * 1e-3;
+    out->device_seconds = dev_s;
     out->pg = st.pg;
     out->pool_subproblems = (int64_t)st.evals * cfmm_pool_count(ctx);
     out->method = CFMM_METHOD_LBFGS;
@@ -3433,7 +3511,7 @@
         if (nu0 && nu0[b]) { int rc = cfmm_set_nu(c, nu0[b]); if (rc) { c0->err = c->err; return rc; } }
         if (!c->pt.have_nu) return fail(c0, CFMM_E_STATE, "solve_batch: context %d has no start prices", b);
         point_from_caller(c);
-        HIP_TRY(c0, hipStreamSynchronize(c->stream));
+        HIP_TRY(c0, hipStreamSynchronize(c->stream)); c->tail = false;
     }
     if (cfmm_pool_count(c0) == 0) return fail(c0, CFMM_E_STATE, "solve_batch: no pools uploaded");
     if (!c0->upd_batch_d) {
@@ -3558,7 +3636,7 @@
     const int len = acc_arb(n) + 1;
     for (int b = 0; b < nb; ++b) {
         cfmm_ctx *c = ctxs[b];
-        HIP_TRY(c0, hipStreamSynchronize(c->stream));
+        HIP_TRY(c0, hipStreamSynchronize(c->stream)); c->tail = false;
         std::memcpy(c->hnu0, nu[b], n * sizeof(double));
         HIP_TRY(c0, hipMemcpyAsync(c->nu_acc, c->hnu0, n * sizeof(double), hipMemcpyHostToDevice, stream));
         HIP_TRY(c0, hipMemcpyAsync(c->nu, c->hnu0, n * sizeof(double), hipMemcpyHostToDevice, stream));
@@ -4111,6 +4189,7 @@
 {
     if (!ctx || n_ranks < 1 || rank < 0 || rank >= n_ranks || !uid128) return ctx ? fail(ctx, CFMM_E_ARG, "comm_init: bad arguments") : CFMM_E_ARG;
     HIP_TRY(ctx, hipSetDevice(ctx->device));
+    { int rc_ = settle(ctx); if (rc_) return rc_; }
     std::string err;
     if (!g_rccl.load(err)) return fail(ctx, CFMM_E_RCCL, "%s", err.c_str());
     ncclUniqueId id;
@@ -4177,6 +4256,7 @@
 {
     if (!ctx || !handle64) return CFMM_E_ARG;
     HIP_TRY(ctx, hipSetDevice(ctx->device));
+    { int rc_ = settle(ctx); if (rc_) return rc_; }
     { int rc = oneshot_alloc(ctx); if (rc) return rc; }
     hipIpcMemHandle_t h;
     static_assert(sizeof(hipIpcMemHandle_t) == 64, "IPC handle size");
@@ -4190,6 +4270,7 @@
     if (!ctx || !mailboxes || n_ranks < 1 || n_ranks > ONESHOT_MAX_RANKS || rank < 0 || rank >= n_ranks)
         return ctx ? fail(ctx, CFMM_E_ARG, "oneshot_attach: %d ranks (at most %d), rank %d", n_ranks, ONESHOT_MAX_RANKS, rank) : CFMM_E_ARG;
     HIP_TRY(ctx, hipSetDevice(ctx->device));
+    { int rc_ = settle(ctx); if (rc_) return rc_; }
     { int rc = oneshot_alloc(ctx); if (rc) return rc; }
     if (ctx->comm && ctx->n_ranks != n_ranks) return fail(ctx, CFMM_E_STATE, "oneshot_attach: the RCCL communicator has %d ranks", ctx->n_ranks);
     for (int r = 0; r < n_ranks; ++r) {
@@ -4227,6 +4308,7 @@
     if (on && !ctx->os_peers[ctx->rank]) return fail(ctx, CFMM_E_STATE, "oneshot_enable: no mailboxes attached (cfmm_oneshot_import / _attach first)");
     if (!on && !ctx->comm && ctx->os_ready) return fail(ctx, CFMM_E_STATE, "oneshot_enable(0): no RCCL communicator to fall back on");
     HIP_TRY(ctx, hipSetDevice(ctx->device));
+    { int rc_ = settle(ctx); if (rc_) return rc_; }
     HIP_TRY(ctx, hipStreamSynchronize(ctx->stream));
     if ((on != 0) != ctx->os_ready) drop_graph(ctx);
     ctx->os_ready = on != 0; ctx->g_counts_valid = false;
@@ -4237,6 +4319,7 @@
 {
     if (!ctx) return CFMM_E_ARG;
     HIP_TRY(ctx, hipSetDevice(ctx->device));
+    { int rc_ = settle(ctx); if (rc_) return rc_; }
     int *d = nullptr, h = -1;
     HIP_TRY(ctx, hipMalloc((void **)&d, sizeof(int)));
     HIP_TRY(ctx, hipMemsetAsync(d, 0, sizeof(int), ctx->stream));
@@ -4257,6 +4340,7 @@
 {
     if (!ctx || !out64) return CFMM_E_ARG;
     HIP_TRY(ctx, hipSetDevice(ctx->device));
+    { int rc_ = settle(ctx); if (rc_) return rc_; }
     HIP_TRY(ctx, hipStreamSynchronize(ctx->stream));
     HIP_TRY(ctx, hipMemcpy(out64, ctx->ts, (64 + 8 * 4096 + 2048) * sizeof(int64_t), hipMemcpyDeviceToHost));
     HIP_TRY(ctx, hipMemset(ctx->ts, 0, (64 + 8 * 4096 + 2048) * sizeof(int64_t)));
@@ -4268,6 +4352,7 @@
 {
     if (!ctx || !(period_us >= 1.0) || !(max_ms > 0.0) || max_ms > 60000.0) return CFMM_E_ARG;
     HIP_TRY(ctx, hipSetDevice(ctx->device));
+    { int rc_ = settle(ctx); if (rc_) return rc_; }
     if (ctx->probe_running) return fail(ctx, CFMM_E_STATE, "clock probe: already running (cfmm_clock_probe_stop first)");
     if (!ctx->probe_stream) HIP_TRY(ctx, hipStreamCreateWithFlags(&ctx->probe_stream, hipStreamNonBlocking));
     if (!ctx->probe_ring) {
@@ -4316,6 +4401,7 @@
     double *out6 = out7;
     if (!ctx || !out6 || np < 1 || np > 8192 || reps < 1) return CFMM_E_ARG;
     HIP_TRY(ctx, hipSetDevice(ctx->device));
+    { int rc_ = settle(ctx); if (rc_) return rc_; }
     const int grid = ctx->cus;
     double *pub = nullptr; unsigned long long *flag = nullptr; long long *stamps = nullptr;
     HIP_TRY(ctx, hipMalloc(&pub, (size_t)16 * np * sizeof(double)));
@@ -4454,6 +4540,7 @@
 {
     if (!ctx || reps < 1) return CFMM_E_ARG;
     HIP_TRY(ctx, hipSetDevice(ctx->device));
+    { int rc_ = settle(ctx); if (rc_) return rc_; }
     const int n = ctx->n, len = acc_arb(n) + 1;
     float ms = 0.f;
     HIP_TRY(ctx, hipMemsetAsync(ctx->acc, 0, (size_t)ctx->nslices * acc_stride(n) * sizeof(double), ctx->stream));
diff --git a/cfmm-routing-code_amd/csrc/iterate.hpp b/cfmm-routing-code_amd/csrc/iterate.hpp
--- a/cfmm-routing-code_amd/csrc/iterate.hpp
+++ b/cfmm-routing-code_amd/csrc/iterate.hpp
@@ -22,6 +22,10 @@
 {
     return (unsigned long long)((unsigned)evals & 0xffffffu) | ((unsigned long long)((unsigned)status & 0xffu) << 24) | ((unsigned long long)(unsigned)launch << 32);
 }
+struct EnvRec {
+    unsigned long long prog, seal;
+    long long t0, t1;
+};
 struct IterArgs {
     EvalArgs ev;
     int n, M, nread, phase;
@@ -40,6 +44,8 @@
     int launch;
     double *h_nu_acc, *h_psi_acc;
     DevState *h_final;
+    EnvRec *env;
+    unsigned epoch;
 };
 
 template <int E> __device__ __forceinline__ void ldE(const double *p, int first, double (&v)[E]);
@@ -275,6 +281,10 @@
         if (blockIdx.x == 0 && tid == 0) {
             a.st3[p] = st;
             if (a.hring) __hip_atomic_store(a.hring + (a.launch & (ITER_HRING - 1)), iter_hring_word(st.evals, st.status, a.launch), __ATOMIC_RELAXED, __HIP_MEMORY_SCOPE_SYSTEM);
+            if (a.env) {
+                if (a.launch == st.evals + 1) a.env->t1 = wall_clock64();
+                __hip_atomic_store(&a.env->seal, iter_hring_word(st.evals, st.status, (int)a.epoch), __ATOMIC_RELEASE, __HIP_MEMORY_SCOPE_SYSTEM);
+            }
         }
         return;
     }
@@ -556,7 +566,8 @@
             if (tid == 0) {
                 a.st3[p] = st; a.nu[n] = st.status != 0 ? 1.0 : 0.0;
                 if (st.status != 0 && a.h_final) *a.h_final = st;
-                if (a.hstat) __hip_atomic_store(a.hstat, (unsigned long long)(unsigned)st.evals | ((unsigned long long)(unsigned)st.status << 32),
+                if (a.env) __hip_atomic_store(&a.env->prog, iter_hring_word(st.evals, st.status, (int)a.epoch), __ATOMIC_RELAXED, __HIP_MEMORY_SCOPE_SYSTEM);
+                else if (a.hstat) __hip_atomic_store(a.hstat, (unsigned long long)(unsigned)st.evals | ((unsigned long long)(unsigned)st.status << 32),
                                                 __ATOMIC_RELAXED, __HIP_MEMORY_SCOPE_SYSTEM);
                 if (a.hring) __hip_atomic_store(a.hring + (a.launch & (ITER_HRING - 1)), iter_hring_word(st.evals, st.status, a.launch), __ATOMIC_RELAXED, __HIP_MEMORY_SCOPE_SYSTEM);
             }
diff --git a/cfmm-routing-code_amd/csrc/kernels.hpp b/cfmm-routing-code_amd/csrc/kernels.hpp
--- a/cfmm-routing-code_amd/csrc/kernels.hpp
+++ b/cfmm-routing-code_amd/csrc/kernels.hpp
@@ -2050,8 +2050,9 @@
 
 template <bool BATCH = false>
 __global__ void __launch_bounds__(UPD_THREADS)
-start_kernel(UpdArgs a0, const double *nu0_, double *zero, long long nzero, DevState *st_clear, int n_clear)
-{
+start_kernel(UpdArgs a0, const double *nu0_, double *zero, long long nzero, DevState *st_clear, int n_clear, long long *t0_stamp = nullptr)
+{
+    if (t0_stamp && blockIdx.x == 0 && threadIdx.x == 0) *t0_stamp = wall_clock64();
     const UpdArgs &a = upd_args<BATCH>(a0);
     const double *nu0 = BATCH ? a.nu_acc : nu0_;
     if (BATCH) { zero = a.acc; }
```
